# nju-websoft/OpenEA

Measured on AMD Instinct MI355X. Metric: training triples/sec (k=10 truncated negatives + limited loss + Adagrad), higher is better.
Workload: dtype f32; 1 GPU; BootEA/AlignE translational step, EN-FR-100K-V1 shape (synthetic), dim=100, GLOBAL batch=20000 positives (weak scaling: 20000 per GPU x 1 GPU), k=10, truncated eps=0.98; the same workload at every N (; global_batch=20000, entities=200000, parallelism=single

## Files before the change

### include/openea_hip.h

```cpp
#ifndef OPENEA_HIP_H
#define OPENEA_HIP_H

#include <stddef.h>
#include <stdint.h>

#ifdef __cplusplus
extern "C" {
#endif

#define OEA_OK 0
#define OEA_EINVAL (-1)
#define OEA_EHIP (-2)
#define OEA_ENOMEM (-3)
#define OEA_EUNSUPPORTED (-4)

int oea_version(void);
const char *oea_last_error(void);
int oea_device_count(void);

int oea_profile_begin(int32_t stride);
int oea_profile_end(int32_t group, double *out_ms_host, int32_t *n_calls_host);

typedef struct oea_store *oea_store_t;
int oea_store_create(int64_t rows, int32_t dim, oea_store_t *out);
// ... 230 lines not shown
                     const int32_t *pos, int64_t n_pos, const int32_t *neg, int64_t n_neg, const int32_t *paths,
                     const int32_t *neg_rel, const float *weight, int64_t n_paths, float path_parm, const oea_step_cfg *cfg,
                     void *step_workspace, void *path_workspace, double *loss_accum, int32_t *err_flag, void *stream);
int oea_path_sample_epoch(const int32_t *paths1, const float *weight1, int64_t n1, const int32_t *paths2, const float *weight2,
                          int64_t n2, const int32_t *rels1, int32_t n_rels1, const int32_t *rels2, int32_t n_rels2, int32_t steps,
                          uint64_t seed, uint32_t epoch, int32_t *out_paths, int32_t *out_neg_rel, float *out_weight, void *stream);
int oea_ptranse_epoch(float *ent, float *ent_acc, int64_t n_ent, float *rel, float *rel_acc, int64_t n_rel, int32_t dim, int32_t ld,
                      const int32_t *pos_all, const int64_t *offsets_host, int32_t steps, const int32_t *neg_buf,
                      const int32_t *path_buf, const int32_t *neg_rel_buf, const float *weight_buf, int64_t P, float path_parm,
                      const oea_step_cfg *cfg, void *step_workspace, void *path_workspace, double *loss_accum, int32_t *err_flag,
                      void *stream);
int oea_weighted_pair_step(float *ent, float *ent_acc, int64_t n_ent, float *rel, float *rel_acc, int64_t n_rel, int32_t dim,
                           int32_t ld, const int32_t *pos, const int32_t *neg, const float *weight, int64_t n,
                           const oea_step_cfg *cfg, void *step_workspace, double *loss_accum, void *stream);

uint64_t oea_tripleset_capacity(int64_t n);
int oea_tripleset_build(const int32_t *triples, int64_t n, uint64_t *table, uint64_t capacity,
                        void *stream);
int oea_sample_negatives(const int32_t *pos, int64_t n_pos, int32_t k, const uint64_t *table,
                         uint64_t capacity, const int32_t *entity_list, int32_t n_ent_list,
                         const int32_t *ent_pos, const int32_t *nbr, int32_t nbr_k, uint64_t seed,
                         uint32_t step, uint32_t pos_offset, int32_t max_try, int32_t *out,
                         int32_t *err_flag, void *stream);

int oea_sample_negatives_replay(const int32_t *pos, int64_t n_pos, int32_t k, const uint64_t *table, uint64_t capacity,
                                const int32_t *entity_list, int32_t n_ent_list, const int32_t *ent_pos, const int32_t *nbr,
                                int32_t nbr_k, int32_t max_try, const int32_t *replay, int32_t *out, int32_t *err_flag, void *stream);

typedef struct oea_sampler_side {
    const uint64_t *table;
    uint64_t capacity;
    const int32_t *entity_list;
    const int32_t *ent_pos;
    const int32_t *nbr;
    int32_t n_ent_list;
    int32_t nbr_k;
    const uint32_t *filter;
    uint64_t filter_bits;
} oea_sampler_side;
uint64_t oea_tripleset_filter_bits(uint64_t capacity);
int oea_tripleset_filter_build(const int32_t *triples, int64_t n, uint32_t *filter, uint64_t filter_bits, void *stream);
int oea_sample_negatives_pair(const int32_t *pos, int64_t n_pos, int64_t n_split, int32_t k,
                              const oea_sampler_side *side0, const oea_sampler_side *side1, uint64_t seed,
                              uint32_t step, uint32_t pos_offset, int32_t max_try, int32_t *out,
                              int32_t *err_flag, void *stream);

int oea_sample_negatives_epoch(const int32_t *pos_all, int64_t n_rows, const int64_t *offsets_dev,
                               const int64_t *splits_dev, int32_t steps, int32_t k, const oea_sampler_side *side0,
                               const oea_sampler_side *side1, uint64_t seed, uint32_t step_base, int32_t max_try,
                               int32_t *out_all, int32_t *err_flag, void *stream);

typedef struct oea_epoch {
    float *ent, *ent_acc;
    int64_t n_ent;
    float *rel, *rel_acc;
    int64_t n_rel;
    int32_t dim, ld;
    const int32_t *pos_all;
    const int64_t *offsets_host, *splits_host;
    int32_t steps;
    const int64_t *offsets_dev, *splits_dev;
    int32_t k;
    const oea_sampler_side *side0, *side1;
    uint64_t seed;
    uint32_t step_base;
    int32_t *neg_buf, *err_flag;
    const oea_step_cfg *cfg;
    void *workspace;
    double *loss_accum;
} oea_epoch;
int oea_triple_epoch_range(const oea_epoch *e, int32_t step_begin, int32_t step_end, int32_t rank, int32_t world, void *plan,
                           size_t plan_bytes, int32_t plan_built, void *stream);

size_t oea_epoch_layout_bytes(int64_t n);
int oea_epoch_layout(const int32_t *triples, int64_t n1, int64_t n2, const int64_t *slot, int64_t n_slots, uint64_t seed, uint32_t epoch,
                     int32_t *dall, void *workspace, size_t ws_bytes, void *stream);

int32_t oea_step_plan_supported(const oea_step_cfg *cfg, int64_t n_ent, int64_t n_rel, int32_t ld, int32_t k);
size_t oea_step_plan_bytes(int64_t n_total, int32_t steps, int64_t max_batch, int64_t n_ent, int32_t ld);
int oea_step_plan_build(const int32_t *pos_all, const int32_t *neg_all, int32_t k, const int64_t *offsets_dev, int64_t n_total,
                        int32_t steps, int64_t max_batch, int64_t n_ent, int32_t ld, void *plan, size_t plan_bytes, void *stream);
int oea_step_plan_offsets(int64_t n_total, int32_t steps, int64_t max_batch, int64_t n_ent, int32_t ld, int64_t *out);
int oea_step_plan_rel_order_offset(int64_t n_total, int32_t steps, int64_t max_batch, int64_t n_ent, int32_t ld, int64_t *out);

struct oea_comm;
int oea_triple_epoch_range_comm(struct oea_comm *comm, const oea_epoch *e, int32_t step_begin, int32_t step_end, void *send, void *own,
                                void *rel_x, float *upd, float *all, void *stream);


uint32_t oea_perm_index(uint32_t i, uint32_t n, uint32_t key);
int oea_sample_link_negatives(const int32_t *pos_links, int64_t n_pos, int32_t k, const int32_t *ents1, int32_t n1,
                              const int32_t *ents2, int32_t n2, const int32_t *nbr1, const int32_t *row1,
                              const int32_t *nbr2, const int32_t *row2, int32_t nbr_k, const uint64_t *exclude,
                              uint64_t exclude_cap, uint64_t seed, uint32_t step, int32_t *out_pairs, float *out_valid,
                              uint64_t *scratch_keys, int32_t *scratch_vals, uint64_t scratch_cap, void *stream);

int oea_greedy_matching(const int32_t *left, const int32_t *right, const float *weight, int64_t n_edges,
                        uint8_t *selected);
int oea_pair_dots(const float *e1, int32_t ld1, const float *e2, int32_t ld2, int32_t dim, const int32_t *ii,
                  const int32_t *jj, int64_t n, float *out, void *stream);

int oea_row_rank_select_f32(const float *vals, int64_t n_rows, int32_t nc, int64_t ld, int32_t k, int32_t largest, const int32_t *ids,
                            int64_t ld_ids, int32_t *out_sel, float *out_kth, void *stream);
int oea_row_rank_select_f64(const double *vals, int64_t n_rows, int32_t nc, int64_t ld, int32_t k, int32_t largest, const int32_t *ids,
                            int64_t ld_ids, int32_t *out_sel, double *out_kth, void *stream);

size_t oea_topk_workspace_bytes(int64_t nq, int64_t nc);
size_t oea_topk_sym_workspace_bytes(int64_t n, int32_t k);
int oea_topk_inner(const float *q, int64_t nq, int32_t ldq, const float *c, int64_t nc, int32_t ldc,
                   int32_t dim, int32_t k, const int32_t *id_map, int32_t *out_idx, void *workspace,
                   size_t ws_bytes, void *stream);

int oea_topk_rows(const float *s, int64_t n_rows, int64_t nc, int64_t ld, int32_t k, const int32_t *id_map,
                  int32_t *out_idx, void *stream);

enum { OEA_METRIC_INNER = 0, OEA_METRIC_MANHATTAN = 1, OEA_METRIC_EUCLIDEAN = 2,
       OEA_METRIC_MANHATTAN_F32 = 3  };
size_t oea_rank_workspace_bytes(int64_t n1);
int oea_rank_eval(const float *e1, int64_t n1, int32_t ld1, const float *e2, int64_t n2, int32_t ld2,
                  int32_t dim, int32_t metric, const float *csls_r, const float *csls_c, int64_t gold_offset,
                  int32_t *rank, int32_t *argmax, void *workspace, void *stream);
size_t oea_rank_eval_bf16_workspace_bytes(int64_t n1, int32_t dim);
int oea_rank_eval_bf16(const float *e1, int64_t n1, int32_t ld1, const float *e2, int64_t n2, int32_t ld2, int32_t dim,
                       int64_t gold_offset, int32_t *rank, int32_t *argmax, int32_t *status, void *workspace, void *stream);
int oea_rank_eval_bf16_csls(const float *e1, int64_t n1, int32_t ld1, const float *e2, int64_t n2, int32_t ld2, int32_t dim,
                            const float *csls_r, const float *csls_c, int64_t gold_offset, int32_t *rank, int32_t *argmax,
                            int32_t *status, void *workspace, void *stream);
int oea_rank_eval_metrics_bf16(const float *e1, int64_t n1, int32_t ld1, const float *e2, int64_t n2, int32_t ld2, int32_t dim,
                               const float *csls_r, const float *csls_c, int64_t gold_offset, const int32_t *top_k_host, int32_t nk,
                               int32_t *rank, int32_t *argmax, int64_t *out_dev, void *workspace, void *stream);
int oea_sim_bf16_matrix(const float *e1, int64_t n1, int32_t ld1, const float *e2, int64_t n2, int32_t ld2, int32_t dim, float *out,
                        int64_t ld_out, void *stream);
size_t oea_rank_eval_metrics_workspace_bytes(int64_t n1);
int oea_rank_eval_metrics(const float *e1, int64_t n1, int32_t ld1, const float *e2, int64_t n2, int32_t ld2, int32_t dim,
                          const float *csls_r, const float *csls_c, int64_t gold_offset, const int32_t *top_k_host, int32_t nk,
                          int32_t *rank, int32_t *argmax, int64_t *hits_and_rank_sum_dev, double *rr_sum_dev, void *workspace,
                          void *stream);
int oea_rank_metrics(const int32_t *rank, int64_t n, const int32_t *top_k_host, int32_t nk,
                     int64_t *hits_dev, int64_t *rank_sum_dev, double *rr_sum_dev, void *stream);

int oea_rank_rows(const float *s, int64_t n_rows, int64_t nc, int64_t ld, const int32_t *gold_idx,
                  int32_t *rank, int32_t *argmax, void *stream);

int oea_sim_matrix(const float *e1, int64_t n1, int32_t ld1, const float *e2, int64_t n2,
                   int32_t ld2, int32_t dim, int32_t metric, float *out, int64_t ld_out,
                   void *stream);
int oea_quantize_rows_u16(const float *src, int64_t n, int32_t ld, int32_t dim, float lo, float inv_step, uint16_t *dst,
                          int32_t ldq, void *stream);
int oea_l1_u16_strip(const uint16_t *q, int64_t nq, const uint16_t *c, int64_t nc, int32_t ldq, float *out, int64_t ld_out,
                     void *stream);
int oea_rank_l1_grid_rows(const float *strip, int64_t rows, int64_t row0, int64_t nc, int64_t ld, const float *e1, int32_t ld1,
                          const float *e2, int32_t ld2, int32_t dim, int64_t gold_offset, float step, float err, int32_t *rank,
                          int32_t *argmax, int32_t *n_exact_rows, void *stream);
int oea_rank_l1_grid_rows_csls(const float *strip, int64_t rows, int64_t row0, int64_t nc, int64_t ld, const float *e1, int32_t ld1,
                               const float *e2, int32_t ld2, int32_t dim, int64_t gold_offset, float step, float err,
                               const float *csls_r, const float *csls_c, int32_t *rank, int32_t *argmax, int32_t *n_exact_rows,
                               void *stream);
int oea_pair_l1_sim(const float *q, int64_t nq, int32_t ldq, const float *table, int64_t n, int32_t ldt, int32_t dim,
                    const int32_t *cand, int32_t c, float *out, void *stream);
int oea_pair_l1_f64(const float *q, int64_t nq, int32_t ldq, const float *table, int64_t n, int32_t ldt, int32_t dim,
                    const int32_t *cand, int32_t c, double *out, void *stream);

int oea_row_topk_mean(const float *s, int64_t n1, int64_t n2, int64_t ld, int32_t k, float *out,
                      void *stream);
size_t oea_csls_means_workspace_bytes(int64_t n1, int64_t n2, int32_t k);
int oea_csls_means(const float *e1, int64_t n1, int32_t ld1, const float *e2, int64_t n2, int32_t ld2, int32_t dim, int32_t k,
// ... 175 lines not shown
```

### openea_amd/_lib.py

```python
import ctypes as C
import os

_HERE = os.path.dirname(os.path.abspath(__file__))
DETERMINISTIC = os.environ.get("OEA_STEP_DETERMINISTIC", "0")[:1] == "1"
LIB_PATH = os.environ.get("OPENEA_HIP_LIB") or os.path.join(_HERE, "csrc",
                                                            "libopenea_hip_det.so" if DETERMINISTIC else "libopenea_hip.so")


class OpenEAHipError(RuntimeError):
    pass


class StepCfg(C.Structure):
    _fields_ = [("loss_kind", C.c_int32), ("l1", C.c_int32), ("margin", C.c_float),
                ("pos_margin", C.c_float), ("neg_margin", C.c_float), ("balance", C.c_float),
                ("ent_l2_norm", C.c_int32), ("rel_l2_norm", C.c_int32), ("opt_kind", C.c_int32),
                ("lr", C.c_float), ("neg_group_k", C.c_int32), ("score_kind", C.c_int32),
                ("normal", C.c_void_p), ("normal_acc", C.c_void_p),
                ("ent_transfer_base", C.c_int32), ("rel_transfer_base", C.c_int32),
                ("beta1", C.c_float), ("beta2", C.c_float), ("eps", C.c_float), ("opt_t", C.c_int32)]


class SamplerSide(C.Structure):
    _fields_ = [("table", C.c_void_p), ("capacity", C.c_uint64), ("entity_list", C.c_void_p),
# ... 50 lines not shown

class ProjEVars(C.Structure):
    _fields_ = [("p", C.c_void_p * 8), ("m", C.c_void_p * 8), ("v", C.c_void_p * 8)]


class Attr2VecVars(C.Structure):
    _fields_ = [(n, C.c_void_p) for n in ("embeds", "embeds_acc", "nce_weights", "nce_weights_acc", "nce_biases", "nce_biases_acc")]


class ConvEVars(C.Structure):
    _fields_ = [("p", C.c_void_p * 14), ("m", C.c_void_p * 14), ("v", C.c_void_p * 14)]


class ConvECfg(C.Structure):
    _fields_ = [("filter_num", C.c_int32), ("keep_prob", C.c_float), ("seed", C.c_uint64)]


class MultiKENet(C.Structure):
    _fields_ = [("p", C.c_void_p * 8), ("ent", C.c_void_p), ("step_workspace", C.c_void_p), ("n_rel_ws", C.c_int64),
                ("weighted", C.c_int32), ("ent_l2_norm", C.c_int32), ("factor", C.c_float)]


LOSS_KIND = {"margin-based": 0, "limited": 1, "logistic": 2, "positive": 3, "align": 4}
OPT_KIND = {"SGD": 0, "Adagrad": 1, "Adam": 2, "Adadelta": 3}
METRIC = {"inner": 0, "manhattan": 1, "euclidean": 2, "manhattan_f32": 3}

_vp, _i32, _i64, _u32, _u64, _f32, _sz = (C.c_void_p, C.c_int32, C.c_int64, C.c_uint32, C.c_uint64,
                                          C.c_float, C.c_size_t)

PROTOTYPES = {
    "oea_version": (C.c_int, []),
    "oea_last_error": (C.c_char_p, []),
    "oea_device_count": (C.c_int, []),
    "oea_profile_begin": (C.c_int, [_i32]),
    "oea_profile_end": (C.c_int, [_i32, C.POINTER(C.c_double), C.POINTER(_i32)]),
    "oea_store_create": (C.c_int, [_i64, _i32, C.POINTER(_vp)]),
    "oea_store_destroy": (C.c_int, [_vp]),
    "oea_store_rows": (_i64, [_vp]),
    "oea_store_dim": (_i32, [_vp]),
    "oea_store_ld": (_i32, [_vp]),
    "oea_store_rows_ptr": (_vp, [_vp]),
    "oea_store_load_host": (C.c_int, [_vp, _vp, _vp]),
    "oea_store_save_host": (C.c_int, [_vp, _vp, _vp]),
    "oea_gather_rows": (C.c_int, [_vp, _i32, _i32, _vp, _i64, _i32, _vp, _i32, _vp]),
    "oea_normalize_rows": (C.c_int, [_vp, _i64, _i32, _i32, _i32, _vp]),
    "oea_fill_f32": (C.c_int, [_vp, _i64, _f32, _vp]),
    "oea_copy_to_host": (C.c_int, [_vp, _vp, _sz, _vp]),
    "oea_copy_from_host": (C.c_int, [_vp, _vp, _sz, _vp]),
    "oea_step_workspace_bytes": (_sz, [_i64, _i64, _i32]),
    "oea_triple_step": (C.c_int, [_vp, _vp, _i64, _vp, _vp, _i64, _i32, _i32, _vp, _i64, _vp, _i64,
                                  C.POINTER(StepCfg), _vp, _vp, _vp]),
    "oea_step_exchange_floats": (_sz, [_i64, _i64, _i32]),
    "oea_step_scratch_elem_bytes": (_i32, []),
    "oea_triple_step_phase": (C.c_int, [_vp, _vp, _i64, _vp, _vp, _i64, _i32, _i32, _vp, _i64, _vp, _i64,
                                        C.POINTER(StepCfg), _vp, _vp, _i32, _vp]),
    "oea_part_rows_per_rank": (_i64, [_i64, _i32]),
    "oea_part_send_floats": (_sz, [_i64, _i32, _i32]),
    "oea_part_pack": (C.c_int, [_vp, _i64, _i64, _i32, _i32, _vp, _vp, _vp]),
    "oea_part_apply": (C.c_int, [_vp, _vp, _i64, _vp, _vp, _i64, _i32, _i32, _i32, _vp, _vp, _vp, C.POINTER(StepCfg), _vp, _i64,
                                 _vp, _vp]),
    "oea_step_normal_scratch": (C.c_int, [_i64, _i64, _i32, _vp, _vp]),
    "oea_step_apply_normals": (C.c_int, [_i64, _i64, _i32, _vp, _vp, _vp]),
    "oea_part_unpack": (C.c_int, [_vp, _i64, _i32, _i32, _i32, _vp, _vp]),
    "oea_step_scatter_ent_rows": (C.c_int, [_vp, _i64, _i64, _i32, _vp, _i64, _vp, _i32, _vp]),
    "oea_tripleset_capacity": (_u64, [_i64]),
    "oea_tripleset_build": (C.c_int, [_vp, _i64, _vp, _u64, _vp]),
    "oea_sample_negatives": (C.c_int, [_vp, _i64, _i32, _vp, _u64, _vp, _i32, _vp, _vp, _i32, _u64,
                                       _u32, _u32, _i32, _vp, _vp, _vp]),
    "oea_sample_negatives_replay": (C.c_int, [_vp, _i64, _i32, _vp, _u64, _vp, _i32, _vp, _vp, _i32, _i32, _vp, _vp, _vp, _vp]),
    "oea_tripleset_filter_bits": (C.c_uint64, [_u64]),
    "oea_tripleset_filter_build": (C.c_int, [_vp, _i64, _vp, _u64, _vp]),
    "oea_sample_negatives_pair": (C.c_int, [_vp, _i64, _i64, _i32, C.POINTER(SamplerSide), C.POINTER(SamplerSide),
                                            _u64, _u32, _u32, _i32, _vp, _vp, _vp]),
    "oea_sample_negatives_epoch": (C.c_int, [_vp, _i64, _vp, _vp, _i32, _i32, C.POINTER(SamplerSide),
                                             C.POINTER(SamplerSide), _u64, _u32, _i32, _vp, _vp, _vp]),
    "oea_triple_epoch_range": (C.c_int, [C.POINTER(Epoch), _i32, _i32, _i32, _i32, _vp, _sz, _i32, _vp]),
    "oea_epoch_layout_bytes": (_sz, [_i64]),
    "oea_epoch_layout": (C.c_int, [_vp, _i64, _i64, _vp, _i64, _u64, _u32, _vp, _vp, _sz, _vp]),
    "oea_step_plan_supported": (_i32, [C.POINTER(StepCfg), _i64, _i64, _i32, _i32]),
    "oea_step_plan_bytes": (_sz, [_i64, _i32, _i64, _i64, _i32]),
    "oea_step_plan_offsets": (C.c_int, [_i64, _i32, _i64, _i64, _i32, _vp]),
    "oea_step_plan_rel_order_offset": (C.c_int, [_i64, _i32, _i64, _i64, _i32, _vp]),
    "oea_step_plan_build": (C.c_int, [_vp, _vp, _i32, _vp, _i64, _i32, _i64, _i64, _i32, _vp, _sz, _vp]),
    "oea_triple_epoch_range_comm": (C.c_int, [_vp, C.POINTER(Epoch), _i32, _i32, _vp, _vp, _vp, _vp, _vp, _vp]),
    "oea_rotate_workspace_bytes": (_sz, [_i64, _i64, _i32]),
    "oea_rotate_exchange_doubles": (_sz, [_i64, _i64, _i32]),
    "oea_rotate_step": (C.c_int, [_vp, _vp, _i64, _vp, _vp, _i64, _i32, _i32, _vp, _i64, _vp, _i64, _i32,
                                  C.POINTER(RotateCfg), _vp, _vp, _i32, _vp]),
    "oea_rotate_lookup": (C.c_int, [_vp, _i64, _i32, _i32, _vp, _i64, _i32, _i32, _vp, _i32, _vp]),
    "oea_mapping_workspace_floats": (_sz, [_i64, _i32, _i32]),
    "oea_mapping_step": (C.c_int, [_vp, _i32, _i32, _i32, _vp, _vp, _i64, _vp, _vp, C.c_float, C.c_float, _i32, _vp, _vp,
                                   _vp, _vp, _vp]),
    "oea_mapping_epoch": (C.c_int, [_vp, _vp, _i64, _vp, _vp, _i64, _i32, _i32, _i32, _vp, _i32, _i64, _vp, _vp, _f32, _f32, _i32,
                                    C.POINTER(StepCfg), _vp, _vp, _vp, _vp, _vp]),
    "oea_sea_mapping_workspace_floats": (_sz, [_i64, _i64, _i32, _i32]),
    "oea_sea_mapping_step": (C.c_int, [_vp, _i32, _i32, _vp, _vp, _i64, _vp, _vp, _i64, _vp, _vp, _vp, _f32, _f32, C.POINTER(StepCfg),
                                       _vp, _vp, _vp, _vp, _vp]),
    "oea_sea_mapping_epoch": (C.c_int, [_vp, _vp, _i64, _vp, _vp, _i64, _i32, _i32, _vp, _i32, _i64, _i64, _vp, _vp, _vp, _f32, _f32,
                                        C.POINTER(StepCfg), _vp, _vp, _vp, _vp, _vp]),
    "oea_step_entity_scratch": (C.c_int, [_vp, _i64, _i64, _i32, C.POINTER(C.c_void_p), C.POINTER(C.c_void_p)]),
    "oea_transr_workspace_bytes": (_sz, [_i64, _i64, _i32, _i64]),
    "oea_transr_step": (C.c_int, [_vp, _vp, _i64, _vp, _vp, _i64, _vp, _vp, _i32, _i32, _vp, _i64, _vp, _i64, C.POINTER(StepCfg),
                                  _vp, _vp, _vp, _vp]),
    "oea_semantic_step": (C.c_int, [_i32, _vp, _vp, _i64, _vp, _vp, _i64, _i32, _i32, _vp, _i64, _vp, _i64, C.POINTER(StepCfg),
                                    _vp, _vp, _vp]),
    "oea_jape_step": (C.c_int, [_vp, _vp, _i64, _vp, _vp, _i64, _i32, _i32, _vp, _i64, _vp, _i64, _f32, C.POINTER(StepCfg), _vp, _vp, _vp]),
    "oea_multike_cnn_workspace_bytes": (_sz, [_i32, _i32, _i64]),
    "oea_multike_cnn_grads": (C.c_int, [_vp, _i32, _i32, _i64, _i32, C.POINTER(C.c_void_p)]),
    "oea_multike_cnn_step": (C.c_int, [C.POINTER(MultiKENet), _i32, _i64, _vp, _i64, _vp, _i64, _i32, _i32, _vp, _i64, _vp, _f32, _vp,
                                       _i64, _vp, _i32, _vp]),
    "oea_multike_rows": (C.c_int, [_i32, _vp, _vp, _i64, _i32, _vp, _vp, _i64, _i32, _vp, _i32, _i64, _i32, _i32, _i32, _vp, _i64, _vp,
                                   _f32, _vp, _vp]),
    "oea_attre_lds_chars": (_i64, [_i32]),
    "oea_attre_char_workspace_bytes": (_sz, [_i64, _i32, _i64]),
    "oea_attre_char_step": (C.c_int, [_vp, _vp, _i64, _vp, _vp, _i64, _vp, _vp, _i64, _i32, _i32, _vp, _i64, _i32, _vp, _i64, _vp, _i64,
                                      _i32, _i32, _i32, C.POINTER(StepCfg), _vp, _vp, _sz, _vp, _vp, _vp]),
    "oea_attre_sample_heads": (C.c_int, [_vp, _i64, _i64, _i32, _vp, _i32, _vp, _vp, _i32, _vp, _i64, _u64, _u32, _u32, _vp, _vp]),
    "oea_attre_joint_epoch": (C.c_int, [_vp, _vp, _vp, _vp, _vp, _i64, _i32, _i32, _i32, _i32, _f32, _i32, _vp, _vp]),
    "oea_sample_distinct": (C.c_int, [_i64, _i64, _u64, _u64, _vp, _vp]),
    "oea_sim_csr_count": (C.c_int, [_vp, _i64, _i32, _vp, _i64, _i32, _i32, _f32, _i64, _vp, _vp, _vp]),
    "oea_sim_csr_fill": (C.c_int, [_vp, _i64, _i32, _vp, _i64, _i32, _i32, _f32, _i64, _vp, _vp, _vp, _vp, _vp, _vp]),
    "oea_jape_sim_loss": (C.c_int, [_vp, _i64, _i32, _i32, _vp, _i64, _vp, _i64, _vp, _vp, _vp, _vp, _i64, _f32, _vp, _vp]),
    "oea_lcs_workspace_ints": (_sz, [_i64]),
    "oea_lcs_ratio_pairs": (C.c_int, [_vp, _vp, _i64, _i64, _vp, _vp, _i64, _i64, _i64, _vp, _i64, _vp, _vp, _vp, _vp, _vp]),
    "oea_attr_sim_records": (C.c_int, [_vp, _vp, _i64, _i64, _vp, _vp, _i64, _i64, _i64, _i32, _vp, _i64, _vp, _i64, C.c_double, _vp, _i64,
                                       _i32, _vp, _vp, _vp, _vp, _vp, _vp, _vp]),
    "oea_log_uniform_sample_steps": (C.c_int, [_i64, _i64, _u64, _u64, _i64, _vp, _vp, _vp, _vp, _vp, _vp]),
    "oea_attr2vec_workspace_bytes": (_sz, [_i64, _i32, _i64]),
    "oea_attr2vec_grads": (C.c_int, [_vp, _i64, _i32, _i64, C.POINTER(C.c_void_p)]),
    "oea_attr2vec_step": (C.c_int, [C.POINTER(Attr2VecVars), _i64, _i32, _i32, _vp, _i64, _vp, _i64, _vp, _vp, _f32, _vp, _i64, _vp, _i32,
                                    _vp]),
    "oea_attr2vec_epoch": (C.c_int, [C.POINTER(Attr2VecVars), _i64, _i32, _i32, _vp, _i64, _i64, _i32, _u64, _u64, _vp, _i64, _vp, _vp, _vp,
                                     _vp, _vp, _f32, _vp, _i64, _vp, _vp]),
    "oea_log_uniform_workspace_bytes": (_sz, [_i64, _i64]),
    "oea_log_uniform_sample": (C.c_int, [_i64, _i64, _u64, _u64, _vp, _vp, _vp, _vp, _vp, _vp]),
    "oea_proje_workspace_floats": (_sz, [_i64, _i64, _i32, _i32, _i64, _i64]),
    "oea_proje_grads": (C.c_int, [_vp, _i64, _i64, _i32, _i32, _i64, _i64, C.POINTER(C.c_void_p)]),
    "oea_proje_step": (C.c_int, [C.POINTER(ProjEVars), _i64, _i64, _i32, _i32, _vp, _i64, _vp, _vp, _i64, _vp, _i64, _f32, _vp, _i64,
                                 _i64, _vp, _i32, _vp]),
    "oea_conve_workspace_floats": (_sz, [_i64, _i64, _i32, _i32, _i32, _i64, _i64]),
    "oea_conve_grads": (C.c_int, [_vp, _i64, _i64, _i32, _i32, _i32, _i64, _i64, C.POINTER(C.c_void_p)]),
    "oea_conve_step": (C.c_int, [C.POINTER(ConvEVars), C.POINTER(ConvECfg), _i64, _i64, _i32, _i32, _vp, _i64, _vp, _vp, _i64, _vp,
                                 _u64, _i64, _f32, _vp, _i64, _i64, _vp, _i32, _vp]),
    "oea_path_workspace_bytes": (_sz, [_i64, _i32]),
    "oea_path_grad": (C.c_int, [_vp, _i64, _i32, _i32, _vp, _vp, _vp, _i64, _f32, _f32, _i32, _vp, _i64, _vp, _vp, _vp, _vp]),
    "oea_ptranse_step": (C.c_int, [_vp, _vp, _i64, _vp, _vp, _i64, _i32, _i32, _vp, _i64, _vp, _i64, _vp, _vp, _vp, _i64, _f32,
                                   C.POINTER(StepCfg), _vp, _vp, _vp, _vp, _vp]),
    "oea_path_sample_epoch": (C.c_int, [_vp, _vp, _i64, _vp, _vp, _i64, _vp, _i32, _vp, _i32, _i32, _u64, _u32, _vp, _vp, _vp, _vp]),
    "oea_ptranse_epoch": (C.c_int, [_vp, _vp, _i64, _vp, _vp, _i64, _i32, _i32, _vp, _vp, _i32, _vp, _vp, _vp, _vp, _i64, _f32,
                                    C.POINTER(StepCfg), _vp, _vp, _vp, _vp, _vp]),
    "oea_weighted_pair_step": (C.c_int, [_vp, _vp, _i64, _vp, _vp, _i64, _i32, _i32, _vp, _vp, _vp, _i64, C.POINTER(StepCfg), _vp,
                                         _vp, _vp]),
    "oea_greedy_matching": (C.c_int, [_vp, _vp, _vp, _i64, _vp]),
    "oea_pair_dots": (C.c_int, [_vp, _i32, _vp, _i32, _i32, _vp, _vp, _i64, _vp, _vp]),
    "oea_perm_index": (_u32, [_u32, _u32, _u32]),
    "oea_sample_link_negatives": (C.c_int, [_vp, _i64, _i32, _vp, _i32, _vp, _i32, _vp, _vp, _vp, _vp, _i32, _vp, _u64,
                                            _u64, _u32, _vp, _vp, _vp, _vp, _u64, _vp]),
    "oea_topk_sym_workspace_bytes": (_sz, [_i64, _i32]),
    "oea_topk_workspace_bytes": (_sz, [_i64, _i64]),
    "oea_topk_inner": (C.c_int, [_vp, _i64, _i32, _vp, _i64, _i32, _i32, _i32, _vp, _vp, _vp, _sz, _vp]),
    "oea_row_rank_select_f32": (C.c_int, [_vp, _i64, _i32, _i64, _i32, _i32, _vp, _i64, _vp, _vp, _vp]),
    "oea_row_rank_select_f64": (C.c_int, [_vp, _i64, _i32, _i64, _i32, _i32, _vp, _i64, _vp, _vp, _vp]),
    "oea_topk_rows": (C.c_int, [_vp, _i64, _i64, _i64, _i32, _vp, _vp, _vp]),
    "oea_rank_rows": (C.c_int, [_vp, _i64, _i64, _i64, _vp, _vp, _vp, _vp]),
    "oea_rank_workspace_bytes": (_sz, [_i64]),
    "oea_rank_eval": (C.c_int, [_vp, _i64, _i32, _vp, _i64, _i32, _i32, _i32, _vp, _vp, _i64, _vp, _vp, _vp, _vp]),
# ... 118 lines not shown
```

### openea_amd/csrc/common.h

```cpp
#pragma once
#include <hip/hip_runtime.h>
#include <hip/hip_ext.h>
#include <stdint.h>
#include <stdio.h>

#include "../../include/openea_hip.h"

namespace oea {

void set_error(const char *fmt, ...);

bool prof_enabled();
void prof_call();
void prof_mark(hipStream_t st);
bool prof_pair(hipEvent_t *start, hipEvent_t *stop);

#define OEA_CHECK_HIP(expr)                                                                   \
    do {                                                                                      \
        hipError_t _e = (expr);                                                               \
        if (_e != hipSuccess) {                                                               \
            oea::set_error("%s:%d: %s -> %s", __FILE__, __LINE__, #expr, hipGetErrorString(_e)); \
            return OEA_EHIP;                                                                  \
        }                                                                                     \
    } while (0)
// ... 58 lines not shown
    return __builtin_bit_cast(float, __builtin_amdgcn_update_dpp(0, __builtin_bit_cast(int, v), CTRL, 0xf, 0xf, false));
}
template <int G>
__device__ __forceinline__ float group_sum(float v) {
    static_assert(G == 2 || G == 4 || G == 8 || G == 16 || G == 32 || G == 64, "group width");
    if (G >= 2) v += dpp_f32<0xB1>(v);
    if (G >= 4) v += dpp_f32<0x4E>(v);
    if (G >= 8) v += dpp_f32<0x141>(v);
    if (G >= 16) v += dpp_f32<0x140>(v);
    if (G >= 32) {
        const unsigned u = __builtin_bit_cast(unsigned, v);
        const auto r = __builtin_amdgcn_permlane16_swap(u, u, false, false);
        v = __builtin_bit_cast(float, (unsigned)r[0]) + __builtin_bit_cast(float, (unsigned)r[1]);
    }
    if (G >= 64) {
        const unsigned u = __builtin_bit_cast(unsigned, v);
        const auto r = __builtin_amdgcn_permlane32_swap(u, u, false, false);
        v = __builtin_bit_cast(float, (unsigned)r[0]) + __builtin_bit_cast(float, (unsigned)r[1]);
    }
    return v;
}
__device__ __forceinline__ float wave_sum_uniform(float v) {
    v += dpp_f32<0xB1>(v);
    v += dpp_f32<0x4E>(v);
    v += dpp_f32<0x141>(v);
    v += dpp_f32<0x140>(v);
    v += dpp_f32<0x142>(v);
    v += dpp_f32<0x143>(v);
    return __builtin_bit_cast(float, __builtin_amdgcn_readlane(__builtin_bit_cast(int, v), 63));
}
template <int G>
__device__ __forceinline__ double group_sum_d(double v) {
#pragma unroll
    for (int off = G / 2; off > 0; off >>= 1) v += __shfl_xor(v, off, 64);
    return v;
}
__device__ __forceinline__ double wave_sum_d(double v) { return group_sum_d<64>(v); }

template <int WAVES>
__device__ __forceinline__ void block_loss_add(double v, int lane, int wave, double *loss_accum, double scale = 1.0) {
    __shared__ double wave_loss[WAVES];
    if (lane == 0) wave_loss[wave] = v;
    __syncthreads();
    if (threadIdx.x == 0) {
        double s = 0.0;
        for (int w = 0; w < WAVES; ++w) s += wave_loss[w];
        if (s != 0.0) atomicAdd(loss_accum, scale * s);
    }
}

__device__ __forceinline__ void atomic_add_f32(float *p, float v) { unsafeAtomicAdd(p, v); }

#ifdef OEA_DET_SCRATCH
typedef long long grad_t;
typedef long long flag_t;
constexpr int kDetScratch = 1;
__device__ __forceinline__ long long to_fixed(float v) {
    const float c = __builtin_amdgcn_fmed3f(v, -524287.f, 524287.f);
    const double d = (double)c + 1572864.0;
    return __double_as_longlong(d) - 0x4138000000000000LL;
}
__device__ __forceinline__ float grad_val(long long q) { return (float)((double)q * 2.3283064365386963e-10); }
__device__ __forceinline__ void grad_add(long long *p, float v) {
    __hip_atomic_fetch_add(reinterpret_cast<unsigned long long *>(p), (unsigned long long)to_fixed(v), __ATOMIC_RELAXED,
                           __HIP_MEMORY_SCOPE_AGENT);
}
__device__ __forceinline__ void grad_add_raw(long long *p, long long q) {
    __hip_atomic_fetch_add(reinterpret_cast<unsigned long long *>(p), (unsigned long long)q, __ATOMIC_RELAXED, __HIP_MEMORY_SCOPE_AGENT);
}
#else
typedef float grad_t;
typedef float flag_t;
constexpr int kDetScratch = 0;
__device__ __forceinline__ float grad_val(float q) { return q; }
__device__ __forceinline__ void grad_add(float *p, float v) { unsafeAtomicAdd(p, v); }
__device__ __forceinline__ void grad_add_raw(float *p, float q) { unsafeAtomicAdd(p, q); }
#endif

void step_scratch_rows(void *workspace, int64_t n_ent, int64_t n_rel, int32_t ld, grad_t **ent_grad, flag_t **ent_touched,
                       grad_t **rel_grad, flag_t **rel_touched);

__device__ __forceinline__ float4 ld4(const float *p) { return *reinterpret_cast<const float4 *>(p); }
__device__ __forceinline__ void st4(float *p, float4 v) { *reinterpret_cast<float4 *>(p) = v; }

__device__ __forceinline__ uint4 philox4x32_10(uint32_t c0, uint32_t c1, uint32_t c2, uint32_t c3,
                                               uint32_t k0, uint32_t k1) {
    const uint32_t M0 = 0xD2511F53u, M1 = 0xCD9E8D57u, W0 = 0x9E3779B9u, W1 = 0xBB67AE85u;
#pragma unroll
    for (int r = 0; r < 10; ++r) {
        const uint32_t hi0 = __umulhi(M0, c0), lo0 = M0 * c0;
        const uint32_t hi1 = __umulhi(M1, c2), lo1 = M1 * c2;
        const uint32_t n0 = hi1 ^ c1 ^ k0, n1 = lo1, n2 = hi0 ^ c3 ^ k1, n3 = lo0;
        c0 = n0; c1 = n1; c2 = n2; c3 = n3;
        k0 += W0; k1 += W1;
    }
    return make_uint4(c0, c1, c2, c3);
}

__host__ __device__ __forceinline__ uint32_t feistel_f(uint32_t r, uint32_t key, uint32_t round) {
    uint32_t v = r * 0x9E3779B1u + key + round * 0x85EBCA6Bu;
    v ^= v >> 15; v *= 0x2C1B3C6Du;
    v ^= v >> 12; v *= 0x297A2D39u;
    v ^= v >> 15;
    return v;
}
__host__ __device__ __forceinline__ uint32_t perm_index(uint32_t i, uint32_t n, uint32_t key) {
    uint32_t bits = 2;
    while ((1u << bits) < n) bits += 2;
    const uint32_t half = bits >> 1, mask = (1u << half) - 1u;
    uint32_t x = i;
    do {
        uint32_t l = x >> half, r = x & mask;
#pragma unroll
        for (uint32_t round = 0; round < 4; ++round) {
            const uint32_t t = l ^ (feistel_f(r, key, round) & mask);
            l = r;
            r = t;
        }
        x = (l << half) | r;
    } while (x >= n);
    return x;
}

#define OEA_EMPTY_KEY 0xFFFFFFFFFFFFFFFFull
__host__ __device__ __forceinline__ uint64_t pack_triple(uint32_t h, uint32_t r, uint32_t t) {
    return ((uint64_t)h << 40) | ((uint64_t)(r & 0xFFFFu) << 24) | (uint64_t)(t & 0xFFFFFFu);
}
__host__ __device__ __forceinline__ uint64_t mix64(uint64_t x) {
    x ^= x >> 30; x *= 0xBF58476D1CE4E5B9ull;
    x ^= x >> 27; x *= 0x94D049BB133111EBull;
    x ^= x >> 31;
    return x;
}

}
```

### openea_amd/csrc/step_plan.h

```cpp
#pragma once
#include <hip/hip_runtime.h>
#include <stddef.h>
#include <stdint.h>

namespace oea {

struct StepPlanView {
    uint64_t *keys_a, *keys_b;
    uint32_t *vals_a, *vals_b;
    uint64_t *ukeys;
    uint32_t *ucount;
    uint32_t *uoff;
    int32_t *n_unique;
    int32_t *step_first;
    uint32_t *pflags;
    uint4 *recs;
    uint8_t *inplan;
    float *contrib;
    void *temp;
    size_t temp_bytes;
    uint32_t *rel_order;
    int row_bits;
};

constexpr uint32_t kPlanHubEntries = 8;

size_t step_plan_layout(int64_t n_total, int32_t steps, int64_t max_batch, int64_t n_ent, int32_t ld, void *base, StepPlanView *v);

}
```

### openea_amd/csrc/step_plan.hip

```cpp
#include <string.h>

#include <rocprim/rocprim.hpp>

#include <algorithm>

#include "common.h"
#include "step_plan.h"

namespace oea {

static size_t al256(size_t x) { return (x + 255) / 256 * 256; }
static int bits_for(uint64_t max_value) { int b = 1; while (b < 64 && (max_value >> b) != 0) ++b; return b; }

size_t step_plan_layout(int64_t n_total, int32_t steps, int64_t max_batch, int64_t n_ent, int32_t ld, void *base, StepPlanView *v) {
    const size_t m = (size_t)std::max<int64_t>(2 * n_total, 1);
    size_t off = 0;
    char *b = static_cast<char *>(base);
    auto take = [&](size_t bytes) { size_t o = off; off += al256(bytes); return b ? b + o : nullptr; };
    StepPlanView w{};
    w.keys_a = (uint64_t *)take(8 * m);
    w.keys_b = (uint64_t *)take(8 * m);
    w.vals_a = (uint32_t *)take(4 * m);
    w.vals_b = (uint32_t *)take(4 * m);
    w.ukeys = (uint64_t *)take(8 * m);
    w.ucount = (uint32_t *)take(4 * (m + 1));
    w.uoff = (uint32_t *)take(4 * (m + 1));
    w.n_unique = (int32_t *)take(4);
    w.step_first = (int32_t *)take(4 * ((size_t)steps + 1));
    w.pflags = (uint32_t *)take(4 * (size_t)std::max<int64_t>(n_total, 1));
    w.recs = (uint4 *)take(16 * m);
    w.inplan = (uint8_t *)take((size_t)std::max<int32_t>(steps, 1) * (size_t)n_ent);
    w.contrib = (float *)take(sizeof(float) * 2 * (size_t)std::max<int64_t>(max_batch, 1) * (size_t)ld);
    size_t t1 = 0, t2 = 0, t3 = 0;
    (void)rocprim::radix_sort_pairs(nullptr, t1, (const uint64_t *)nullptr, (uint64_t *)nullptr, (const uint32_t *)nullptr,
                                    (uint32_t *)nullptr, m, 0, 64, (hipStream_t)0);
    (void)rocprim::run_length_encode(nullptr, t2, (const uint64_t *)nullptr, m, (uint64_t *)nullptr, (uint32_t *)nullptr,
                                     (int32_t *)nullptr, (hipStream_t)0);
    (void)rocprim::exclusive_scan(nullptr, t3, (const uint32_t *)nullptr, (uint32_t *)nullptr, 0u, m + 1, rocprim::plus<uint32_t>(),
                                  (hipStream_t)0);
    const size_t n1 = (size_t)std::max<int64_t>(n_total, 1);
    w.temp_bytes = std::max(std::max(t1, std::max(t2, t3)), al256(4 * n1)) + 256;
    w.temp = take(w.temp_bytes);
    w.rel_order = (uint32_t *)take(4 * n1);
    w.row_bits = bits_for((uint64_t)std::max<int64_t>(n_ent - 1, 1));
    if (v) *v = w;
    return off;
}

namespace {

__global__ void plan_emit_kernel(const int32_t *__restrict__ pos_all, const int32_t *__restrict__ neg_all, int k,
                                 const int64_t *__restrict__ offsets, int steps, int64_t n_total, int row_bits,
                                 uint64_t *__restrict__ keys, uint32_t *__restrict__ vals) {
    const int64_t p = (int64_t)blockIdx.x * blockDim.x + threadIdx.x;
    if (p >= n_total) return;
    int lo = 0, hi = steps;
    while (hi - lo > 1) {
        const int mid = (lo + hi) >> 1;
        if (offsets[mid] <= p) lo = mid; else hi = mid;
    }
    const uint32_t pl = (uint32_t)(p - offsets[lo]);
    const int h = pos_all[3 * p], r = pos_all[3 * p + 1], t = pos_all[3 * p + 2];
    unsigned bad = 0, xh = 0, xt = 0;
    const int32_t *ng = neg_all + p * k * 3;
    for (int j = 0; j < k; ++j) {
        const unsigned a = (unsigned)(ng[3 * j] ^ h), b = (unsigned)(ng[3 * j + 2] ^ t), c = (unsigned)(ng[3 * j + 1] ^ r);
        bad |= c | min(a, b);
        xh |= a;
        xt |= b;
    }
    if (bad | min(xh, xt)) {
        keys[2 * p] = keys[2 * p + 1] = (uint64_t)steps << row_bits;
        vals[2 * p] = vals[2 * p + 1] = 0u;
        return;
    }
    const bool tails = xh == 0;
    const uint64_t sk = (uint64_t)lo << row_bits;
    keys[2 * p] = sk | (uint64_t)(uint32_t)h;
    vals[2 * p] = 2u * pl + (tails ? 0u : 1u);
    keys[2 * p + 1] = sk | (uint64_t)(uint32_t)t;
    vals[2 * p + 1] = 0x80000000u | (2u * pl + (tails ? 1u : 0u));
}

constexpr int kRelSortWaves = 8, kRelDigitBits = 10, kRelBins = 1 << kRelDigitBits, kRelAhead = 8;
__global__ __launch_bounds__(kRelSortWaves * 64) void plan_rel_order_kernel(const int32_t *__restrict__ pos_all, const int64_t *__restrict__ offsets,
                                                                            uint32_t *__restrict__ tmp, uint32_t *__restrict__ rel_order) {
    __shared__ uint32_t hist[kRelSortWaves][kRelBins];
    __shared__ uint32_t dbase[kRelBins];
    __shared__ uint32_t wsum[kRelSortWaves];
    __shared__ uint32_t rmax;
    const int64_t first = offsets[blockIdx.x];
    const uint32_t n = (uint32_t)(offsets[blockIdx.x + 1] - first);
    if (n == 0) return;
    const int32_t *rel = pos_all + 3 * first + 1;
    const uint32_t t = threadIdx.x, lane = t & 63u, w = t >> 6;
    const uint32_t slice = (n + kRelSortWaves - 1) / kRelSortWaves, c0 = min(w * slice, n), c1 = min(c0 + slice, n);
    const uint32_t groups = (c1 - c0 + 63u) / 64u;
    if (t == 0) rmax = 0u;
    int passes = 1;
    uint32_t *src = nullptr, *dst = nullptr;
    for (int pass = 0; pass < passes; ++pass) {
        const int shift = pass * kRelDigitBits;
        for (uint32_t i = t; i < kRelSortWaves * kRelBins; i += blockDim.x) (&hist[0][0])[i] = 0u;
        __syncthreads();
        uint32_t m = 0u;
        for (uint32_t g0 = 0; g0 < groups; g0 += kRelAhead) {
            uint32_t r[kRelAhead];
#pragma unroll
            for (int u = 0; u < kRelAhead; ++u) {
                const uint32_t i = c0 + (g0 + u) * 64u + lane;
                r[u] = i < c1 ? (uint32_t)rel[3 * (int64_t)(src ? src[i] : i)] : 0xffffffffu;
            }
#pragma unroll
            for (int u = 0; u < kRelAhead; ++u)
                if (c0 + (g0 + u) * 64u + lane < c1) {
                    m = max(m, r[u]);
                    atomicAdd(&hist[w][(r[u] >> shift) & (kRelBins - 1)], 1u);
                }
        }
        if (pass == 0) {
            for (int o = 32; o > 0; o >>= 1) m = max(m, (uint32_t)__shfl_xor((int)m, o));
            if (lane == 0) atomicMax(&rmax, m);
        }
        __syncthreads();
        if (pass == 0) {
            while (passes * kRelDigitBits < 32 && (rmax >> (passes * kRelDigitBits)) != 0u) ++passes;
// ... 78 lines not shown
    }
}

__global__ void plan_hub_kernel(const uint64_t *__restrict__ keys, const uint32_t *__restrict__ vals, int64_t m,
                                const int64_t *__restrict__ offsets, int steps, int row_bits, uint32_t *__restrict__ pflags) {
    const int64_t e = (int64_t)blockIdx.x * blockDim.x + threadIdx.x;
    if (e >= m) return;
    const uint64_t key = keys[e];
    const int64_t step = (int64_t)(key >> row_bits);
    if (step >= steps) return;
    int left = 0, right = 0;
    while (left < (int)kPlanHubEntries && e - left - 1 >= 0 && keys[e - left - 1] == key) ++left;
    while (left + right < (int)kPlanHubEntries && e + right + 1 < m && keys[e + right + 1] == key) ++right;
    if (left + right < (int)kPlanHubEntries) return;
    const uint32_t v = vals[e];
    atomicOr(&pflags[offsets[step] + ((v & 0x7fffffffu) >> 1)], (v >> 31) ? 2u : 1u);
}

__device__ __forceinline__ uint32_t mix32(uint32_t x) {
    x ^= x >> 16; x *= 0x7feb352du; x ^= x >> 15; x *= 0x846ca68bu; x ^= x >> 16;
    return x;
}
__device__ __forceinline__ uint32_t feistel_perm(uint32_t i, uint32_t n, int lbits, int rbits, const uint32_t (&key)[6]) {
    const uint32_t lmask = (1u << lbits) - 1u, rmask = (1u << rbits) - 1u;
    uint32_t x = i;
    do {
        uint32_t l = x >> rbits, r = x & rmask;
#pragma unroll
        for (int q = 0; q < 6; q += 2) {
            l = (l ^ mix32(r ^ key[q])) & lmask;
            r = (r ^ mix32(l ^ key[q + 1])) & rmask;
        }
        x = (l << rbits) | r;
    } while (x >= n);
    return x;
}
__global__ void layout_perm_kernel(const int32_t *__restrict__ triples, int64_t n1, int64_t n2, const int64_t *__restrict__ slot, int64_t n_slots,
                                   uint32_t k0, uint32_t k1, uint32_t epoch, int32_t *__restrict__ dall) {
    const int64_t j = (int64_t)blockIdx.x * blockDim.x + threadIdx.x;
    if (j >= n_slots) return;
    const int64_t sj = slot[j];
    const bool second = sj >= n1;
    const uint32_t n = (uint32_t)(second ? n2 : n1), i = (uint32_t)(second ? sj - n1 : sj);
    int bits = 1;
    while (bits < 32 && (1ull << bits) < (unsigned long long)n) ++bits;
    if (bits < 2) bits = 2;
    const int rbits = bits / 2, lbits = bits - rbits;
    const uint4 wa = philox4x32_10(epoch, second ? 1u : 0u, 0x5eedu, 0u, k0, k1), wb = philox4x32_10(epoch, second ? 1u : 0u, 0x5eedu, 1u, k0, k1);
    const uint32_t key[6] = {wa.x, wa.y, wa.z, wa.w, wb.x, wb.y};
    const int64_t src = (int64_t)feistel_perm(i, n, lbits, rbits, key) + (second ? n1 : 0);
    dall[3 * j] = triples[3 * src]; dall[3 * j + 1] = triples[3 * src + 1]; dall[3 * j + 2] = triples[3 * src + 2];
}

}
}

extern "C" {

size_t oea_step_plan_bytes(int64_t n_total, int32_t steps, int64_t max_batch, int64_t n_ent, int32_t ld) {
    if (n_total < 0 || steps < 0 || max_batch < 0 || n_ent <= 0 || ld <= 0) return 0;
    return oea::step_plan_layout(n_total, steps, max_batch, n_ent, ld, nullptr, nullptr);
}

int oea_step_plan_offsets(int64_t n_total, int32_t steps, int64_t max_batch, int64_t n_ent, int32_t ld, int64_t *out) {
    OEA_REQUIRE(out && n_total >= 0 && steps >= 0 && n_ent > 0 && ld > 0, "arguments");
    oea::StepPlanView v;
    char *base = reinterpret_cast<char *>(4096);
    const size_t total = oea::step_plan_layout(n_total, steps, max_batch, n_ent, ld, base, &v);
    out[0] = (char *)v.vals_b - base; out[1] = (char *)v.ukeys - base; out[2] = (char *)v.uoff - base;
    out[3] = (char *)v.n_unique - base; out[4] = (char *)v.step_first - base; out[5] = (char *)v.contrib - base;
    out[6] = v.row_bits; out[7] = (int64_t)total; out[8] = (char *)v.pflags - base;
    return OEA_OK;
}

int oea_step_plan_rel_order_offset(int64_t n_total, int32_t steps, int64_t max_batch, int64_t n_ent, int32_t ld, int64_t *out) {
    OEA_REQUIRE(out && n_total >= 0 && steps >= 0 && n_ent > 0 && ld > 0, "arguments");
    oea::StepPlanView v;
    char *base = reinterpret_cast<char *>(4096);
    (void)oea::step_plan_layout(n_total, steps, max_batch, n_ent, ld, base, &v);
    *out = (char *)v.rel_order - base;
    return OEA_OK;
}

size_t oea_epoch_layout_bytes(int64_t n) {
    return n < 0 ? 0 : 256;
}

int oea_epoch_layout(const int32_t *triples, int64_t n1, int64_t n2, const int64_t *slot, int64_t n_slots, uint64_t seed, uint32_t epoch,
                     int32_t *dall, void *workspace, size_t ws_bytes, void *stream) {
    OEA_REQUIRE(triples && (slot || n_slots == 0) && (dall || n_slots == 0), "null pointer");
    OEA_REQUIRE(n1 >= 0 && n2 >= 0 && n_slots >= 0 && n1 < ((int64_t)1 << 32) && n2 < ((int64_t)1 << 32), "sizes");
    (void)workspace; (void)ws_bytes;
    if (n1 + n2 == 0 || n_slots == 0) return OEA_OK;
    hipStream_t st = oea::as_stream(stream);
    oea::layout_perm_kernel<<<(unsigned)oea::ceil_div(n_slots, 256), 256, 0, st>>>(triples, n1, n2, slot, n_slots, (uint32_t)seed,
                                                                                   (uint32_t)(seed >> 32), epoch, dall);
    OEA_CHECK_HIP(hipGetLastError());
    return OEA_OK;
}

int oea_step_plan_build(const int32_t *pos_all, const int32_t *neg_all, int32_t k, const int64_t *offsets_dev, int64_t n_total,
                        int32_t steps, int64_t max_batch, int64_t n_ent, int32_t ld, void *plan, size_t plan_bytes, void *stream) {
    OEA_REQUIRE(pos_all && offsets_dev && plan && (neg_all || k == 0), "null pointer");
    OEA_REQUIRE(n_total >= 0 && steps >= 1 && k >= 0 && n_ent > 0 && ld > 0, "sizes");
    OEA_REQUIRE(2 * n_total < ((int64_t)1 << 31) && 2 * max_batch < ((int64_t)1 << 31), "entries and slots are 31-bit");
    oea::StepPlanView v;
    const size_t need = oea::step_plan_layout(n_total, steps, max_batch, n_ent, ld, plan, &v);
    OEA_REQUIRE(plan_bytes >= need, "plan workspace smaller than oea_step_plan_bytes");
    hipStream_t st = oea::as_stream(stream);
    const size_t m = (size_t)(2 * n_total);
    if (m == 0) {
        OEA_CHECK_HIP(hipMemsetAsync(v.n_unique, 0, sizeof(int32_t), st));
        OEA_CHECK_HIP(hipMemsetAsync(v.step_first, 0, sizeof(int32_t) * ((size_t)steps + 1), st));
        return OEA_OK;
    }
    oea::plan_rel_order_kernel<<<(unsigned)steps, oea::kRelSortWaves * 64, 0, st>>>(pos_all, offsets_dev, (uint32_t *)v.temp, v.rel_order);
    oea::plan_emit_kernel<<<(unsigned)oea::ceil_div(n_total, 256), 256, 0, st>>>(pos_all, neg_all, k, offsets_dev, steps, n_total, v.row_bits,
                                                                                 v.keys_a, v.vals_a);
    const int end_bit = std::min(64, v.row_bits + oea::bits_for((uint64_t)steps));
    size_t tb = v.temp_bytes;
    OEA_CHECK_HIP(rocprim::radix_sort_pairs(v.temp, tb, (const uint64_t *)v.keys_a, v.keys_b, (const uint32_t *)v.vals_a, v.vals_b, m, 0,
                                            (unsigned)end_bit, st));
    OEA_CHECK_HIP(hipMemsetAsync(v.ucount, 0, sizeof(uint32_t) * (m + 1), st));
    tb = v.temp_bytes;
    OEA_CHECK_HIP(rocprim::run_length_encode(v.temp, tb, (const uint64_t *)v.keys_b, m, v.ukeys, v.ucount, v.n_unique, st));
    tb = v.temp_bytes;
    OEA_CHECK_HIP(rocprim::exclusive_scan(v.temp, tb, (const uint32_t *)v.ucount, v.uoff, 0u, m + 1, rocprim::plus<uint32_t>(), st));
    oea::plan_step_first_kernel<<<(unsigned)oea::ceil_div(steps + 1, 256), 256, 0, st>>>(v.ukeys, v.n_unique, steps, v.row_bits, v.step_first);
    OEA_CHECK_HIP(hipMemsetAsync(v.pflags, 0, sizeof(uint32_t) * (size_t)n_total, st));
    OEA_CHECK_HIP(hipMemsetAsync(v.inplan, 0, (size_t)steps * (size_t)n_ent, st));
    oea::plan_records_kernel<<<(unsigned)std::min<int64_t>(oea::ceil_div((int64_t)m, 256), 4096), 256, 0, st>>>(
        v.ukeys, v.uoff, v.vals_b, v.n_unique, steps, v.row_bits, n_ent, v.recs, v.inplan);
    oea::plan_hub_kernel<<<(unsigned)oea::ceil_div((int64_t)m, 256), 256, 0, st>>>(v.keys_b, v.vals_b, (int64_t)m, offsets_dev, steps, v.row_bits,
                                                                                   v.pflags);
    OEA_CHECK_HIP(hipGetLastError());
    return OEA_OK;
}

}
```

### openea_amd/csrc/triple_step.hip

```cpp
#include <stdlib.h>

#include <algorithm>
#include <type_traits>
#include <vector>

#include "common.h"
#include "step_plan.h"

namespace {

using oea::align256;
using oea::group_sum;

using oea::flag_t;
using oea::grad_t;

struct StepWs {
    grad_t *ent_grad, *rel_grad;
    grad_t *rel_extra;
    int64_t rel_copy_stride;
    flag_t *ent_touched, *rel_touched;
    grad_t *nrm_grad, *nrm_extra;
    flag_t *nrm_touched;
    double *partials;
// ... 327 lines not shown
            any = coef != 0.f;
        }
        if (any) {
            atomic_row<G, IT>(ws.ent_grad + (int64_t)h * ld, ld, lane, gh, 1.f);
            atomic_row<G, IT>(ws.rel_copy(p % kRelCopies) + (int64_t)r * ld, ld, lane, gr, 1.f);
            atomic_row<G, IT>(ws.ent_grad + (int64_t)t * ld, ld, lane, gt, 1.f);
            if (lane == 0) { ws.ent_touched[h] = 1.f; ws.ent_touched[t] = 1.f; ws.rel_touched[r] = 1.f; }
        }
        if (lane == 0) loss_local += lsum;
    }
    block_loss_partial(loss_local, ws.partials);
}

#ifdef OEA_DET_SCRATCH
constexpr int kGradShift = 3;
#else
constexpr int kGradShift = 2;
#endif
constexpr unsigned kBufFlags = 0x00020000u;
constexpr int kBufRecords = (int)0x80000000u;
constexpr int kBufOob = (int)0xC0000000u;

__device__ __forceinline__ void buf_grad_add(__amdgpu_buffer_rsrc_t rs, float v, int voff, int soff, int imm) {
#ifdef OEA_DET_SCRATCH
    const long long q = oea::to_fixed(v);
    const int vo = voff + imm;
    asm volatile("s_nop 4\n\tbuffer_atomic_add_x2 %0, %1, %2, %3 offen" ::"v"(q), "v"(vo), "s"(rs), "s"(soff) : "memory");
#else
    __builtin_amdgcn_raw_ptr_buffer_atomic_fadd_f32(v, rs, voff + imm, soff, 0);
#endif
}
__device__ __forceinline__ void buf_flag_set(__amdgpu_buffer_rsrc_t rs, int row) {
#ifdef OEA_DET_SCRATCH
    typedef unsigned int u32x2 __attribute__((ext_vector_type(2)));
    const u32x2 one = {1u, 0u};
    __builtin_amdgcn_raw_buffer_store_b64(one, rs, 0, row * 8, 0);
#else
    __builtin_amdgcn_raw_buffer_store_b32(0x3f800000u, rs, 0, row * 4, 0);
#endif
}
template <int IT>
__device__ __forceinline__ void wave_load_row(__amdgpu_buffer_rsrc_t rs, int soff, int v4, int vt, Row<64, IT> &r) {
#pragma unroll
    for (int it = 0; it < IT; ++it)
        r.v[it] = __builtin_bit_cast(float, __builtin_amdgcn_raw_buffer_load_b32(rs, it < IT - 1 ? v4 + it * 256 : vt, soff, 0));
}
template <int IT>
__device__ __forceinline__ void wave_atomic_row(__amdgpu_buffer_rsrc_t rs, int soff, int vg, int vgt, const Row<64, IT> &g, float sign) {
#pragma unroll
    for (int it = 0; it < IT; ++it) {
        if (it < IT - 1) buf_grad_add(rs, sign * g.v[it], vg, soff, it * (64 << kGradShift));
        else buf_grad_add(rs, sign * g.v[it], vgt, soff, 0);
    }
}
template <int IT>
__device__ __forceinline__ void wave_rel_row(const StepWs &ws, int dbg, int64_t p, int r, int row_g, int vg, int vgt, const Row<64, IT> &g) {
    const int copy = (int)(p % kRelCopies);
    grad_t *rgb = copy == 0 ? ws.rel_grad : ws.rel_extra + (copy - 1) * ws.rel_copy_stride;
    const __amdgpu_buffer_rsrc_t rs_rg = __builtin_amdgcn_make_buffer_rsrc(rgb, 0, (dbg & 1) ? 0 : kBufRecords, kBufFlags);
    const __amdgpu_buffer_rsrc_t rs_rt = __builtin_amdgcn_make_buffer_rsrc(ws.rel_touched, 0, (dbg & 4) ? 0 : kBufRecords, kBufFlags);
    wave_atomic_row<IT>(rs_rg, r * row_g, vg, vgt, g, 1.f);
    buf_flag_set(rs_rt, r);
}
__device__ __forceinline__ float uniform_f(float x) {
    return __builtin_bit_cast(float, __builtin_amdgcn_readfirstlane(__builtin_bit_cast(int, x)));
}

__device__ __forceinline__ double uniform_d(double x) {
    const unsigned long long b = __builtin_bit_cast(unsigned long long, x);
    const unsigned lo = (unsigned)__builtin_amdgcn_readfirstlane((int)(unsigned)b), hi = (unsigned)__builtin_amdgcn_readfirstlane((int)(unsigned)(b >> 32));
    return __builtin_bit_cast(double, ((unsigned long long)hi << 32) | lo);
}

template <int IT>
__device__ __forceinline__ void wave_normalize(Row<64, IT> &r) {
    float s = 0.f;
#pragma unroll
    for (int it = 0; it < IT; ++it) s += r.v[it] * r.v[it];
    const float inv = rsqrtf(fmaxf(oea::wave_sum_uniform(s), 1e-12f));
#pragma unroll
    for (int it = 0; it < IT; ++it) r.v[it] *= inv;
}

template <int IT, int L1, int KT, bool PLAN>
__global__ __launch_bounds__(512, (IT <= 2 ? (KT == 10 ? 8 : 7) : 4)) void triple_wave(
    const float *__restrict__ ent, const float *__restrict__ rel, int ld, const int32_t *__restrict__ pos,
    int64_t n_pos, const int32_t *__restrict__ neg, int k, oea_step_cfg cfg, StepWs ws, int dbg, float *__restrict__ contrib,
    const uint32_t *__restrict__ pflags, const uint32_t *__restrict__ order) {
    constexpr int G = 64, KC = 10;
    if (KT > 0) k = KT;
    const int lane = threadIdx.x & 63;
    const int wv = __builtin_amdgcn_readfirstlane((int)(threadIdx.x >> 6));
    const int wpb = blockDim.x >> 6;
    const int64_t nw = (int64_t)gridDim.x * wpb;
    const int row_b = ld * 4, row_g = ld << kGradShift;
    const __amdgpu_buffer_rsrc_t rs_ent = __builtin_amdgcn_make_buffer_rsrc(const_cast<float *>(ent), 0, (dbg & 2) ? 0 : kBufRecords, kBufFlags);
    const __amdgpu_buffer_rsrc_t rs_rel = __builtin_amdgcn_make_buffer_rsrc(const_cast<float *>(rel), 0, (dbg & 2) ? 0 : kBufRecords, kBufFlags);
    const __amdgpu_buffer_rsrc_t rs_eg = __builtin_amdgcn_make_buffer_rsrc(ws.ent_grad, 0, (dbg & 1) ? 0 : kBufRecords, kBufFlags);
    const __amdgpu_buffer_rsrc_t rs_et = __builtin_amdgcn_make_buffer_rsrc(ws.ent_touched, 0, (dbg & 4) ? 0 : kBufRecords, kBufFlags);
    const int v4 = lane * 4, vg = lane << kGradShift;
    const int c_last = (IT - 1) * 64 + lane;
    const int vt = c_last < ld ? c_last * 4 : kBufOob, vgt = c_last < ld ? c_last << kGradShift : kBufOob;
    const float c_neg = L1 ? -cfg.balance : -2.f * cfg.balance;
    double loss_local = 0.0;
    auto score_positive = [&](int64_t p, Row<G, IT> &gacc) -> int {
        const int32_t *pp = pos + 3 * p;
        const int32_t *ng = neg + p * k * 3;
        const int h = pp[0], r = pp[1], t = pp[2];
        Row<G, IT> yh, yr, yt;
        wave_load_row<IT>(rs_ent, h * row_b, v4, vt, yh);
        wave_load_row<IT>(rs_rel, r * row_b, v4, vt, yr);
        wave_load_row<IT>(rs_ent, t * row_b, v4, vt, yt);
        int ids[3 * KC];
        if (KT == KC || k == KC) {
#pragma unroll
            for (int q = 0; q < 3 * KC; ++q) ids[q] = ng[q];
        } else {
#pragma unroll
            for (int q = 0; q < 3 * KC; ++q) ids[q] = q < 3 * k ? ng[q] : 0;
        }
        unsigned bad = 0, xh = 0, xt = 0;
#pragma unroll
        for (int j = 0; j < KC; ++j)
            if (KT == KC || j < k) {
                const unsigned a = (unsigned)(ids[3 * j] ^ h), b = (unsigned)(ids[3 * j + 2] ^ t), c = (unsigned)(ids[3 * j + 1] ^ r);
                bad |= c | min(a, b);
                xh |= a;
                xt |= b;
            }
        if (bad) {
            double ls = score_independent<G, IT>(ent, rel, ld, lane, p, h, r, t, true, cfg, ws, OEA_LOSS_LIMITED, L1);
#pragma unroll 1
            for (int j = 0; j < k; ++j)
                ls += score_independent<G, IT>(ent, rel, ld, lane, p, ng[3 * j], ng[3 * j + 1], ng[3 * j + 2], false, cfg, ws, OEA_LOSS_LIMITED, L1);
            loss_local = uniform_d(loss_local + ls);
            return -1;
        }
        if (min(xh, xt)) {
            unsigned tmask = 0;
            int ce[KC];
            Row<G, IT> yc[KC];
#pragma unroll
            for (int j = 0; j < KC; ++j)
                if (KT == KC || j < k) {
                    const int nh = ids[3 * j], nt = ids[3 * j + 2];
                    const bool tl = nh == h;
                    tmask |= tl ? 1u << j : 0u;
                    ce[j] = tl ? nt : nh;
                    wave_load_row<IT>(rs_ent, ce[j] * row_b, v4, vt, yc[j]);
                }
            asm volatile("" : "+s"(tmask));
#pragma unroll
            for (int it = 0; it < IT; ++it)
                asm volatile("" : "+v"(yh.v[it]), "+v"(yr.v[it]), "+v"(yt.v[it]));
            wave_normalize<IT>(yh);
            wave_normalize<IT>(yr);
            wave_normalize<IT>(yt);
            Row<G, IT> u, gpos;
            float sp = 0.f;
#pragma unroll
            for (int it = 0; it < IT; ++it) {
                u.v[it] = yh.v[it] + yr.v[it];
                const float d = u.v[it] - yt.v[it];
                gpos.v[it] = d;
                sp += L1 ? fabsf(d) : d * d;
            }
            const float xp = oea::wave_sum_uniform(sp) - cfg.pos_margin;
            const bool cpos = xp > 0.f;
            float lsum = cpos ? xp : 0.f;
#pragma unroll
            for (int it = 0; it < IT; ++it) {
                gpos.v[it] = cpos ? (L1 ? sgn(gpos.v[it]) : 2.f * gpos.v[it]) : 0.f;
                gacc.v[it] = gpos.v[it];
            }
            bool anyneg = false;
#pragma unroll
            for (int j = 0; j < KC; ++j)
                if (KT == KC || j < k) {
                    const bool tl = (tmask >> j) & 1u;
                    wave_normalize<IT>(yc[j]);
                    float s = 0.f;
                    if (tl) {
#pragma unroll
                        for (int it = 0; it < IT; ++it) {
                            const float d = u.v[it] - yc[j].v[it];
                            yc[j].v[it] = d;
                            s += L1 ? fabsf(d) : d * d;
                        }
                    } else {
#pragma unroll
                        for (int it = 0; it < IT; ++it) {
                            const float d = yc[j].v[it] + yr.v[it] - yt.v[it];
                            yc[j].v[it] = d;
                            s += L1 ? fabsf(d) : d * d;
                        }
                    }
                    const float xn = cfg.neg_margin - oea::wave_sum_uniform(s);
                    if (xn > 0.f) {
                        lsum += cfg.balance * xn;
                        anyneg = true;
                        Row<G, IT> g;
#pragma unroll
                        for (int it = 0; it < IT; ++it) {
                            g.v[it] = L1 ? c_neg * sgn(yc[j].v[it]) : c_neg * yc[j].v[it];
                            gacc.v[it] += g.v[it];
                        }
                        const int pe = tl ? h : t;
                        const float sign_c = tl ? -1.f : 1.f;
                        wave_atomic_row<IT>(rs_eg, ce[j] * row_g, vg, vgt, g, sign_c);
                        buf_flag_set(rs_et, ce[j]);
                        wave_atomic_row<IT>(rs_eg, pe * row_g, vg, vgt, g, -sign_c);
                        buf_flag_set(rs_et, pe);
                    }
                }
            if (cpos) {
                wave_atomic_row<IT>(rs_eg, h * row_g, vg, vgt, gpos, 1.f);
                buf_flag_set(rs_et, h);
                wave_atomic_row<IT>(rs_eg, t * row_g, vg, vgt, gpos, -1.f);
                buf_flag_set(rs_et, t);
            }
            loss_local = uniform_d(loss_local + (double)lsum);
            if (!(cpos | anyneg)) return -1;
            if (PLAN && order) return r;
            wave_rel_row<IT>(ws, dbg, p, r, row_g, vg, vgt, gacc);
            return -1;
        }
        auto one_sided = [&](auto side) -> int {
            constexpr bool tails = decltype(side)::value;
            int ce[KC];
            Row<G, IT> yc[KC];
#pragma unroll
            for (int j = 0; j < KC; ++j)
                if (KT == KC || j < k) {
                    ce[j] = tails ? ids[3 * j + 2] : ids[3 * j];
                    wave_load_row<IT>(rs_ent, ce[j] * row_b, v4, vt, yc[j]);
                }
            wave_normalize<IT>(yh);
            wave_normalize<IT>(yr);
            wave_normalize<IT>(yt);
            Row<G, IT> u, gpos;
            int r_sum = -1;
            float sp = 0.f;
#pragma unroll
            for (int it = 0; it < IT; ++it) {
                u.v[it] = yh.v[it] + yr.v[it];
                const float d = u.v[it] - yt.v[it];
                gpos.v[it] = d;
                sp += L1 ? fabsf(d) : d * d;
            }
            const float xp = oea::wave_sum_uniform(sp) - cfg.pos_margin;
            const bool cpos = xp > 0.f;
            float lsum = cpos ? xp : 0.f;
#pragma unroll
            for (int it = 0; it < IT; ++it) {
                gpos.v[it] = cpos ? (L1 ? sgn(gpos.v[it]) : 2.f * gpos.v[it]) : 0.f;
                gacc.v[it] = gpos.v[it];
            }
            float sc[KC];
            if (tails) {
#pragma unroll
                for (int j = 0; j < KC; ++j)
                    if (KT == KC || j < k) {
                        wave_normalize<IT>(yc[j]);
                        float s = 0.f;
#pragma unroll
                        for (int it = 0; it < IT; ++it) {
                            const float d = u.v[it] - yc[j].v[it];
                            yc[j].v[it] = d;
                            s += L1 ? fabsf(d) : d * d;
                        }
                        sc[j] = oea::wave_sum_uniform(s);
                    }
            } else {
#pragma unroll
                for (int j = 0; j < KC; ++j)
                    if (KT == KC || j < k) {
                        wave_normalize<IT>(yc[j]);
                        float s = 0.f;
#pragma unroll
                        for (int it = 0; it < IT; ++it) {
                            const float d = yc[j].v[it] + yr.v[it] - yt.v[it];
                            yc[j].v[it] = d;
                            s += L1 ? fabsf(d) : d * d;
                        }
                        sc[j] = oea::wave_sum_uniform(s);
                    }
            }
            bool anyneg = false;
            const float sign_c = tails ? -1.f : 1.f;
#pragma unroll
            for (int j = 0; j < KC; ++j)
                if (KT == KC || j < k) {
                    const float xn = cfg.neg_margin - sc[j];
                    if (xn > 0.f) {
                        lsum += cfg.balance * xn;
                        anyneg = true;
                        Row<G, IT> g;
#pragma unroll
                        for (int it = 0; it < IT; ++it) {
                            g.v[it] = L1 ? c_neg * sgn(yc[j].v[it]) : c_neg * yc[j].v[it];
                            gacc.v[it] += g.v[it];
                        }
                        wave_atomic_row<IT>(rs_eg, ce[j] * row_g, vg, vgt, g, sign_c);
                        buf_flag_set(rs_et, ce[j]);
                    }
                }
            if (PLAN) {
                const __amdgpu_buffer_rsrc_t rs_cb = __builtin_amdgcn_make_buffer_rsrc(contrib, 0, kBufRecords, kBufFlags);
                const int so = (int)p * 2 * row_b;
#pragma unroll
                for (int it = 0; it < IT; ++it) {
                    const int vo = it < IT - 1 ? v4 + it * 256 : vt;
                    __builtin_amdgcn_raw_buffer_store_b32(__builtin_bit_cast(unsigned, gacc.v[it]), rs_cb, vo, so, 0);
                    __builtin_amdgcn_raw_buffer_store_b32(__builtin_bit_cast(unsigned, gpos.v[it]), rs_cb, vo, so + row_b, 0);
                }
            }
            if (cpos | anyneg) {
                if (PLAN && order) r_sum = r;
                else wave_rel_row<IT>(ws, dbg, p, r, row_g, vg, vgt, gacc);
                const unsigned via_atomics = PLAN ? pflags[p] : 3u;
                const bool h_full = tails, t_full = !tails;
                if ((via_atomics & 1u) && (h_full || cpos)) {
                    wave_atomic_row<IT>(rs_eg, h * row_g, vg, vgt, h_full ? gacc : gpos, 1.f);
                    buf_flag_set(rs_et, h);
                }
                if ((via_atomics & 2u) && (t_full || cpos)) {
                    wave_atomic_row<IT>(rs_eg, t * row_g, vg, vgt, t_full ? gacc : gpos, -1.f);
                    buf_flag_set(rs_et, t);
                }
            }
            loss_local = uniform_d(loss_local + (double)lsum);
            return r_sum;
        };
        return xh == 0 ? one_sided(std::true_type{}) : one_sided(std::false_type{});
    };
    if constexpr (!PLAN) {
        for (int64_t p = (int64_t)blockIdx.x * wpb + wv; p < n_pos; p += nw) {
            Row<G, IT> gacc;
            (void)score_positive(p, gacc);
        }
    } else {
        for (int64_t q0 = (int64_t)blockIdx.x * wpb; q0 < n_pos; q0 += nw) {
            const int64_t q = q0 + wv;
            Row<G, IT> gacc;
            const int r_sum = q < n_pos ? score_positive(order ? (int64_t)order[q] : q, gacc) : -1;
            if (!order) continue;
            __shared__ float s_row[8][IT][64];
            __shared__ int s_rel[8];
            int lb = v4;
            asm volatile("" : "+v"(lb));
            const auto at = [lb](auto *base) { return (decltype(base))((char *)base + lb); };
            if (lb == 0) s_rel[wv] = r_sum;
            if (r_sum >= 0) {
#pragma unroll
                for (int it = 0; it < IT; ++it) *at(&s_row[wv][it][0]) = gacc.v[it];
            }
            __syncthreads();
            if (r_sum >= 0) {
                const int held = lb < wpb * 4 ? *at(&s_rel[0]) : -1;
                bool first = true;
#pragma unroll
                for (int w = 0; w < 8; ++w) first = first && !(w < wv && __builtin_amdgcn_readlane(held, w) == r_sum);
                if (first) {
#pragma unroll
                    for (int w = 1; w < 8; ++w)
                        if (w > wv && __builtin_amdgcn_readlane(held, w) == r_sum) {
#pragma unroll
                            for (int it = 0; it < IT; ++it) gacc.v[it] += *at(&s_row[w][it][0]);
                        }
                    wave_rel_row<IT>(ws, dbg, order[q], r_sum, row_g, vg, vgt, gacc);
                }
            }
            if (q0 + nw < n_pos) __syncthreads();
        }
    }
    __shared__ double sred[8];
    int lz = v4;
    if constexpr (PLAN) asm volatile("" : "+v"(lz));
    if (lz == 0) sred[wv] = loss_local;
    __syncthreads();
    if (wv == 0 && lz == 0) {
        double s = 0.0;
        for (int w = 0; w < wpb; ++w) s += sred[w];
        ws.partials[blockIdx.x] = s;
    }
}

template <int G, int IT>
__device__ __forceinline__ float dot(const Row<G, IT> &a, const Row<G, IT> &b) {
// ... 293 lines not shown
        if (KIND == OEA_SCORE_TRANSD)
            return transd_triple<G, IT>(ent, rel, ld, lane, item, tr[0], tr[1], tr[2], is_pos, cfg, ws, mode, coef, l);
        return transh_triple<G, IT>(ent, rel, ld, lane, item, tr[0], tr[1], tr[2], is_pos, cfg, ws, mode, coef, l);
    };
    for (int64_t item = grp; item < items; item += ngrp) {
        float l;
        if (!margin) {
            const bool is_pos = item < n_pos;
            one(item, is_pos ? pos + 3 * item : neg + 3 * (item - n_pos), is_pos, 2, 0.f, l);
            if (lane == 0) loss_local += (double)l;
            continue;
        }
        float sc[2];
#pragma unroll 1
        for (int u = 0; u < 2; ++u) sc[u] = one(item, (u ? neg : pos) + 3 * item, u == 0, 0, 0.f, l);
        const float x = cfg.margin + sc[0] - sc[1];
        if (x <= 0.f) continue;
        if (lane == 0) loss_local += (double)x;
#pragma unroll 1
        for (int u = 0; u < 2; ++u) one(item, (u ? neg : pos) + 3 * item, u == 0, 1, u ? -1.f : 1.f, l);
    }
    block_loss_partial(loss_local, ws.partials);
}

template <int G, int IT>
__global__ __launch_bounds__(256) void apply_normal_rows(int64_t n_rel, int ld, oea_step_cfg cfg, StepWs ws, int copies_folded) {
    const int lane = threadIdx.x % G;
    const int64_t grp = ((int64_t)blockIdx.x * blockDim.x + threadIdx.x) / G;
    const int64_t ngrp = (int64_t)gridDim.x * blockDim.x / G;
    for (int64_t row = grp; row < n_rel; row += ngrp) {
        if (ws.nrm_touched[row] == 0) continue;
        float *v = cfg.normal + row * ld;
        Row<G, IT> rv, rg, y1, y2;
        grad_t q[IT];
        load_row<G, IT>(v, ld, lane, rv);
        load_grad_raw<G, IT>(ws.nrm_grad + row * ld, ld, lane, q);
        for (int cp = 1; cp < kRelCopies && !copies_folded; ++cp) {
#pragma unroll
            for (int it = 0; it < IT; ++it) {
                const int c = it * G + lane;
                if (c < ld) {
                    const grad_t x = ws.nrm_copy(cp)[row * ld + c];
                    if (x != 0) { q[it] += x; ws.nrm_copy(cp)[row * ld + c] = 0; }
                }
            }
        }
#pragma unroll
        for (int it = 0; it < IT; ++it) rg.v[it] = oea::grad_val(q[it]);
        const float ss1 = sumsq<G, IT>(rv);
        const float inv1 = rsqrtf(fmaxf(ss1, 1e-12f));
#pragma unroll
        for (int it = 0; it < IT; ++it) y1.v[it] = rv.v[it] * inv1;
        const float ss2 = sumsq<G, IT>(y1);
        const float inv2 = rsqrtf(fmaxf(ss2, 1e-12f));
#pragma unroll
        for (int it = 0; it < IT; ++it) y2.v[it] = y1.v[it] * inv2;
        const float d2 = dot<G, IT>(y2, rg);
#pragma unroll
        for (int it = 0; it < IT; ++it) rg.v[it] = (rg.v[it] - y2.v[it] * d2) * inv2;
        const float d1 = ss1 > 1e-12f ? dot<G, IT>(y1, rg) : 0.f;
#pragma unroll
        for (int it = 0; it < IT; ++it) {
            const int c = it * G + lane;
            if (c < ld) {
                const float gv = (rg.v[it] - y1.v[it] * d1) * inv1;
                if (cfg.opt_kind == OEA_OPT_ADAGRAD) {
                    const float a = cfg.normal_acc[row * ld + c] + gv * gv;
                    cfg.normal_acc[row * ld + c] = a;
                    v[c] = rv.v[it] - cfg.lr * gv / sqrtf(a);
                } else {
                    v[c] = rv.v[it] - cfg.lr * gv;
                }
                ws.nrm_grad[row * ld + c] = 0;
            }
        }
        if (lane == 0) ws.nrm_touched[row] = 0;
    }
}

template <int G, int IT, bool CLEAR = true>
__device__ __forceinline__ void apply_one_row(float *__restrict__ v, float *__restrict__ acc, grad_t *__restrict__ g,
                                              flag_t *__restrict__ touched_flag, int ld, int lane, int on,
                                              const oea_step_cfg &cfg, const Row<G, IT> &rv, Row<G, IT> &rg,
                                              const Row<G, IT> &ra) {
    float inv = 1.f, ydg = 0.f;
    if (on) {
        const float ss = sumsq<G, IT>(rv);
        inv = rsqrtf(fmaxf(ss, 1e-12f));
        float dot = 0.f;
#pragma unroll
        for (int it = 0; it < IT; ++it) dot += rv.v[it] * rg.v[it];
        dot = group_sum<G>(dot) * inv;
        ydg = ss > 1e-12f ? dot : 0.f;
    }
#pragma unroll
    for (int it = 0; it < IT; ++it) {
        const int c = it * G + lane;
        if (c < ld) {
            const float gv = on ? (rg.v[it] - rv.v[it] * inv * ydg) * inv : rg.v[it];
            if (cfg.opt_kind == OEA_OPT_ADAGRAD) {
                const float a = ra.v[it] + gv * gv;
                acc[c] = a;
                v[c] = rv.v[it] - cfg.lr * gv / sqrtf(a);
            } else {
                v[c] = rv.v[it] - cfg.lr * gv;
            }
            if (CLEAR) g[c] = 0;
        }
    }
    if (CLEAR && lane == 0) *touched_flag = 0;
}

template <int G, int IT>
__device__ __forceinline__ void apply_relation_row(int64_t row, float *__restrict__ rel, float *__restrict__ rel_acc, int ld, int lane,
                                                   const oea_step_cfg &cfg, const StepWs &ws, int copies_folded) {
    float *v = rel + row * ld;
    float *acc = rel_acc + row * ld;
    grad_t *g = ws.rel_grad + row * ld;
    const float flag = (float)ws.rel_touched[row];
    Row<G, IT> rv, rg, ra;
    grad_t q[IT];
    load_row<G, IT>(v, ld, lane, rv);
    load_grad_raw<G, IT>(g, ld, lane, q);
    if (cfg.opt_kind == OEA_OPT_ADAGRAD) load_row<G, IT>(acc, ld, lane, ra);
    if (flag == 0.f) return;
    if (!copies_folded) {
        constexpr int CB = IT <= 4 ? 5 : 1;
#ifdef OEA_DET_SCRATCH
#pragma unroll 1
#endif
        for (int cp0 = 1; cp0 < kRelCopies; cp0 += CB) {
            grad_t tmp[CB][IT];
#pragma unroll
            for (int u = 0; u < CB; ++u)
#pragma unroll
                for (int it = 0; it < IT; ++it) {
                    const int c = it * G + lane;
                    tmp[u][it] = (cp0 + u < kRelCopies && c < ld) ? ws.rel_copy(cp0 + u)[row * ld + c] : (grad_t)0;
                }
#pragma unroll
            for (int u = 0; u < CB; ++u)
#pragma unroll
                for (int it = 0; it < IT; ++it) {
                    const int c = it * G + lane;
                    q[it] += tmp[u][it];
                    if (cp0 + u < kRelCopies && c < ld && tmp[u][it] != 0) ws.rel_copy(cp0 + u)[row * ld + c] = 0;
                }
        }
    }
#pragma unroll
    for (int it = 0; it < IT; ++it) rg.v[it] = oea::grad_val(q[it]);
    apply_one_row<G, IT>(v, acc, g, ws.rel_touched + row, ld, lane, cfg.rel_l2_norm, cfg, rv, rg, ra);
}

template <int G, int IT, int R>
__global__ __launch_bounds__(256) void apply_rows(float *__restrict__ ent, float *__restrict__ ent_acc,
                                                  int64_t n_ent, float *__restrict__ rel,
                                                  float *__restrict__ rel_acc, int64_t n_rel, int ld,
                                                  oea_step_cfg cfg, StepWs ws, int n_partials,
                                                  double *__restrict__ loss_accum, int copies_folded, int flag_first) {
    const int lane = threadIdx.x % G;
    const int64_t grp = ((int64_t)blockIdx.x * blockDim.x + threadIdx.x) / G;
    const int64_t ngrp = (int64_t)gridDim.x * blockDim.x / G;
    const int64_t n_items = n_rel + (n_ent + R - 1) / R;
    for (int64_t w = grp; w < n_items; w += ngrp) {
        if (w >= n_rel) {
            const int64_t row0 = (w - n_rel) * R;
            float flag[R];
            Row<G, IT> rv[R], rg[R], ra[R];
            if (flag_first) {
                bool any = false;
#pragma unroll
                for (int r = 0; r < R; ++r) any |= row0 + r < n_ent && ws.ent_touched[row0 + r] != 0;
                if (!any) continue;
            }
#pragma unroll
            for (int r = 0; r < R; ++r) {
                const int64_t row = row0 + r < n_ent ? row0 + r : n_ent - 1;
                flag[r] = row0 + r < n_ent ? (float)ws.ent_touched[row] : 0.f;
                load_row<G, IT>(ent + row * ld, ld, lane, rv[r]);
                load_grad_row<G, IT>(ws.ent_grad + row * ld, ld, lane, rg[r]);
                if (cfg.opt_kind == OEA_OPT_ADAGRAD) load_row<G, IT>(ent_acc + row * ld, ld, lane, ra[r]);
            }
#pragma unroll
            for (int r = 0; r < R; ++r) {
                if (flag[r] == 0.f) continue;
                const int64_t row = row0 + r;
                apply_one_row<G, IT>(ent + row * ld, ent_acc + row * ld, ws.ent_grad + row * ld, ws.ent_touched + row, ld,
                                     lane, cfg.ent_l2_norm, cfg, rv[r], rg[r], ra[r]);
            }
            continue;
        }
        apply_relation_row<G, IT>(w, rel, rel_acc, ld, lane, cfg, ws, copies_folded);
    }
    if (blockIdx.x == 0 && threadIdx.x < 64) {
        double s = 0.0;
        for (int i = threadIdx.x; i < n_partials; i += 64) s += ws.partials[i];
        s = oea::wave_sum_d(s);
        if (threadIdx.x == 0) *loss_accum += s;
    }
}

template <int G, int IT>
__global__ __launch_bounds__(256) void apply_step_plan(float *__restrict__ ent, float *__restrict__ ent_acc, int64_t n_ent,
                                                       float *__restrict__ rel, float *__restrict__ rel_acc, int64_t n_rel, int ld,
                                                       oea_step_cfg cfg, StepWs ws, int n_partials, double *__restrict__ loss_accum,
                                                       int copies_folded, int rel_blocks, int scan_blocks,
                                                       const uint4 *__restrict__ recs, const uint32_t *__restrict__ vals,
                                                       const int32_t *__restrict__ step_first, int s, const uint8_t *__restrict__ inplan,
                                                       const float *__restrict__ contrib) {
    constexpr int GPB = 256 / G, GPW = 64 / G;
    const int lane = threadIdx.x % G;
    const int b = (int)blockIdx.x, nb = (int)gridDim.x;
    if (b < rel_blocks) {
        for (int64_t row = (int64_t)b * GPB + threadIdx.x / G; row < n_rel; row += (int64_t)rel_blocks * GPB)
            apply_relation_row<G, IT>(row, rel, rel_acc, ld, lane, cfg, ws, copies_folded);
    } else if (b >= rel_blocks + scan_blocks && b < nb - 1) {
        const int plan_blocks = nb - 1 - rel_blocks - scan_blocks;
        const int64_t grp = (int64_t)(b - rel_blocks - scan_blocks) * GPB + threadIdx.x / G, ngrp = (int64_t)plan_blocks * GPB;
        const int64_t i1 = step_first[s + 1];
        for (int64_t i = step_first[s] + grp; i < i1; i += ngrp) {
            const uint4 rec = recs[i];
            if (rec.z > oea::kPlanHubEntries) continue;
            const int64_t row = rec.x;
            const uint32_t e0 = rec.y, e1 = rec.y + rec.z, v0 = rec.w;
            const float flag = (float)ws.ent_touched[row];
            Row<G, IT> rv, ra, rg, rc;
            load_row<G, IT>(ent + row * ld, ld, lane, rv);
            if (cfg.opt_kind == OEA_OPT_ADAGRAD) load_row<G, IT>(ent_acc + row * ld, ld, lane, ra);
            load_row<G, IT>(contrib + (int64_t)(v0 & 0x7fffffffu) * ld, ld, lane, rc);
#pragma unroll
            for (int it = 0; it < IT; ++it) rg.v[it] = (v0 >> 31) ? -rc.v[it] : rc.v[it];
            for (uint32_t e = e0 + 1; e < e1; e += 3) {
                uint32_t ve[3];
                Row<G, IT> r3[3];
#pragma unroll
                for (int u = 0; u < 3; ++u) ve[u] = vals[min(e + u, e1 - 1)];
#pragma unroll
                for (int u = 0; u < 3; ++u) load_row<G, IT>(contrib + (int64_t)(ve[u] & 0x7fffffffu) * ld, ld, lane, r3[u]);
#pragma unroll
                for (int u = 0; u < 3; ++u)
                    if (e + u < e1) {
#pragma unroll
                        for (int it = 0; it < IT; ++it) rg.v[it] += (ve[u] >> 31) ? -r3[u].v[it] : r3[u].v[it];
                    }
            }
            if (flag != 0.f) {
                grad_t *g = ws.ent_grad + row * ld;
                Row<G, IT> rs;
                load_grad_row<G, IT>(g, ld, lane, rs);
#pragma unroll
                for (int it = 0; it < IT; ++it) {
                    rg.v[it] += rs.v[it];
                    const int c = it * G + lane;
                    if (c < ld) g[c] = 0;
                }
                if (lane == 0) ws.ent_touched[row] = 0;
            }
            apply_one_row<G, IT, false>(ent + row * ld, ent_acc + row * ld, nullptr, nullptr, ld, lane, cfg.ent_l2_norm, cfg, rv, rg, ra);
        }
    } else if (b < nb - 1) {
        const int first = rel_blocks;
        const int wl = threadIdx.x & 63, gw = wl / G;
        const int64_t wave = (int64_t)(b - first) * 4 + (threadIdx.x >> 6), nwave = (int64_t)scan_blocks * 4;
        const int64_t n_chunk = (n_ent + 63) / 64;
        const uint8_t *mine = inplan + (int64_t)s * n_ent;
        for (int64_t chunk = wave; chunk < n_chunk; chunk += nwave) {
            const int64_t r = (int64_t)wl * n_chunk + chunk;
            const bool todo = r < n_ent && (float)ws.ent_touched[r] != 0.f && mine[r] == 0;
            unsigned long long mask = __ballot(todo);
            while (mask) {
                int64_t row = -1;
#pragma unroll
                for (int q = 0; q < GPW; ++q)
                    if (mask) {
                        const int bit = __builtin_ctzll(mask);
                        mask &= mask - 1;
                        if (gw == q) row = (int64_t)bit * n_chunk + chunk;
                    }
                if (row >= 0) {
                    Row<G, IT> rv, rg, ra;
                    load_row<G, IT>(ent + row * ld, ld, lane, rv);
                    load_grad_row<G, IT>(ws.ent_grad + row * ld, ld, lane, rg);
                    if (cfg.opt_kind == OEA_OPT_ADAGRAD) load_row<G, IT>(ent_acc + row * ld, ld, lane, ra);
                    apply_one_row<G, IT>(ent + row * ld, ent_acc + row * ld, ws.ent_grad + row * ld, ws.ent_touched + row, ld, lane,
                                         cfg.ent_l2_norm, cfg, rv, rg, ra);
                }
            }
        }
    } else {
        __shared__ double sp[256];
        double v[16];
#pragma unroll
        for (int u = 0; u < 16; ++u) { const int i = u * 256 + (int)threadIdx.x; v[u] = i < n_partials ? ws.partials[i] : 0.0; }
        double acc = 0.0;
#pragma unroll
        for (int u = 0; u < 16; ++u) acc += v[u];
        sp[threadIdx.x] = acc;
        __syncthreads();
        for (int o = 128; o > 0; o >>= 1) {
            if ((int)threadIdx.x < o) sp[threadIdx.x] += sp[threadIdx.x + o];
            __syncthreads();
        }
        if (threadIdx.x == 0) *loss_accum += sp[0];
    }
}

#ifndef OEA_DET_SCRATCH
template <int IT4>
struct Row4 {
    float4 v[IT4];
};
template <int G, int IT4>
__device__ __forceinline__ void load_row4(const float *__restrict__ base, int ld, int lane, Row4<IT4> &r) {
#pragma unroll
    for (int it = 0; it < IT4; ++it) {
        const int c = (it * G + lane) * 4;
        r.v[it] = c < ld ? oea::ld4(base + c) : make_float4(0.f, 0.f, 0.f, 0.f);
    }
}
__device__ __forceinline__ float4 f4_axpy(float a, float4 x, float4 y) { return make_float4(fmaf(a, x.x, y.x), fmaf(a, x.y, y.y), fmaf(a, x.z, y.z), fmaf(a, x.w, y.w)); }
__device__ __forceinline__ float4 f4_add(float4 x, float4 y) { return make_float4(x.x + y.x, x.y + y.y, x.z + y.z, x.w + y.w); }
__device__ __forceinline__ float f4_dot(float4 x, float4 y) { return x.x * y.x + x.y * y.y + x.z * y.z + x.w * y.w; }

template <int G, int IT4, bool CLEAR>
__device__ __forceinline__ void apply_one_row4(float *__restrict__ v, float *__restrict__ acc, float *__restrict__ g, flag_t *__restrict__ touched_flag,
                                               int ld, int lane, int on, const oea_step_cfg &cfg, const Row4<IT4> &rv, const Row4<IT4> &rg,
                                               const Row4<IT4> &ra) {
    float inv = 1.f, ydg = 0.f;
    if (on) {
        float ss = 0.f, dot = 0.f;
#pragma unroll
        for (int it = 0; it < IT4; ++it) { ss += f4_dot(rv.v[it], rv.v[it]); dot += f4_dot(rv.v[it], rg.v[it]); }
        ss = group_sum<G>(ss);
        inv = rsqrtf(fmaxf(ss, 1e-12f));
        dot = group_sum<G>(dot) * inv;
        ydg = ss > 1e-12f ? dot : 0.f;
    }
#pragma unroll
    for (int it = 0; it < IT4; ++it) {
        const int c = (it * G + lane) * 4;
        if (c < ld) {
            float4 gv = rg.v[it];
            const float4 y = rv.v[it];
            if (on)
                gv = make_float4((gv.x - y.x * inv * ydg) * inv, (gv.y - y.y * inv * ydg) * inv, (gv.z - y.z * inv * ydg) * inv,
                                 (gv.w - y.w * inv * ydg) * inv);
            float4 nv;
            if (cfg.opt_kind == OEA_OPT_ADAGRAD) {
                const float4 a = make_float4(ra.v[it].x + gv.x * gv.x, ra.v[it].y + gv.y * gv.y, ra.v[it].z + gv.z * gv.z,
                                             ra.v[it].w + gv.w * gv.w);
                oea::st4(acc + c, a);
                nv = make_float4(rv.v[it].x - cfg.lr * gv.x / sqrtf(a.x), rv.v[it].y - cfg.lr * gv.y / sqrtf(a.y),
                                 rv.v[it].z - cfg.lr * gv.z / sqrtf(a.z), rv.v[it].w - cfg.lr * gv.w / sqrtf(a.w));
            } else {
                nv = make_float4(y.x - cfg.lr * gv.x, y.y - cfg.lr * gv.y, y.z - cfg.lr * gv.z, y.w - cfg.lr * gv.w);
            }
            oea::st4(v + c, nv);
            if (CLEAR) oea::st4(g + c, make_float4(0.f, 0.f, 0.f, 0.f));
        }
    }
    if (CLEAR && lane == 0) *touched_flag = 0;
}

template <int G, int IT>
__global__ __launch_bounds__(256) void apply_step_plan_v4(float *__restrict__ ent, float *__restrict__ ent_acc, int64_t n_ent,
                                                          float *__restrict__ rel, float *__restrict__ rel_acc, int64_t n_rel, int ld,
                                                          oea_step_cfg cfg, StepWs ws, int n_partials, double *__restrict__ loss_accum,
                                                          int copies_folded, int rel_blocks, int scan_blocks,
                                                          const uint4 *__restrict__ recs, const uint32_t *__restrict__ vals,
                                                          const int32_t *__restrict__ step_first, int s, const uint8_t *__restrict__ inplan,
                                                          const float *__restrict__ contrib) {
    constexpr int GPB = 256 / G, GPW = 64 / G, IT4 = (IT + 3) / 4;
    const int lane = threadIdx.x % G;
    const int b = (int)blockIdx.x, nb = (int)gridDim.x;
    if (b < rel_blocks) {
        for (int64_t row = (int64_t)b * GPB + threadIdx.x / G; row < n_rel; row += (int64_t)rel_blocks * GPB)
            apply_relation_row<G, IT>(row, rel, rel_acc, ld, lane, cfg, ws, copies_folded);
    } else if (b >= rel_blocks + scan_blocks && b < nb - 1) {
        const int plan_blocks = nb - 1 - rel_blocks - scan_blocks;
        const int64_t grp = (int64_t)(b - rel_blocks - scan_blocks) * GPB + threadIdx.x / G, ngrp = (int64_t)plan_blocks * GPB;
        const int64_t i1 = step_first[s + 1];
        for (int64_t i = step_first[s] + grp; i < i1; i += ngrp) {
            const uint4 rec = recs[i];
            if (rec.z > oea::kPlanHubEntries) continue;
            const int64_t row = rec.x;
            const uint32_t e0 = rec.y, e1 = rec.y + rec.z, v0 = rec.w;
            const float flag = (float)ws.ent_touched[row];
            Row4<IT4> rv, ra, rg, rc;
            load_row4<G, IT4>(ent + row * ld, ld, lane, rv);
            if (cfg.opt_kind == OEA_OPT_ADAGRAD) load_row4<G, IT4>(ent_acc + row * ld, ld, lane, ra);
            load_row4<G, IT4>(contrib + (int64_t)(v0 & 0x7fffffffu) * ld, ld, lane, rc);
            const float s0 = (v0 >> 31) ? -1.f : 1.f;
#pragma unroll
            for (int it = 0; it < IT4; ++it) rg.v[it] = make_float4(s0 * rc.v[it].x, s0 * rc.v[it].y, s0 * rc.v[it].z, s0 * rc.v[it].w);
            for (uint32_t e = e0 + 1; e < e1; e += 3) {
                uint32_t ve[3];
                Row4<IT4> r3[3];
#pragma unroll
                for (int u = 0; u < 3; ++u) ve[u] = vals[min(e + u, e1 - 1)];
#pragma unroll
                for (int u = 0; u < 3; ++u) load_row4<G, IT4>(contrib + (int64_t)(ve[u] & 0x7fffffffu) * ld, ld, lane, r3[u]);
#pragma unroll
                for (int u = 0; u < 3; ++u)
                    if (e + u < e1) {
                        const float su = (ve[u] >> 31) ? -1.f : 1.f;
#pragma unroll
                        for (int it = 0; it < IT4; ++it) rg.v[it] = f4_axpy(su, r3[u].v[it], rg.v[it]);
                    }
            }
            if (flag != 0.f) {
                float *g = ws.ent_grad + row * ld;
                Row4<IT4> rs;
                load_row4<G, IT4>(g, ld, lane, rs);
#pragma unroll
                for (int it = 0; it < IT4; ++it) {
                    rg.v[it] = f4_add(rg.v[it], rs.v[it]);
                    const int c = (it * G + lane) * 4;
                    if (c < ld) oea::st4(g + c, make_float4(0.f, 0.f, 0.f, 0.f));
                }
                if (lane == 0) ws.ent_touched[row] = 0;
            }
            apply_one_row4<G, IT4, false>(ent + row * ld, ent_acc + row * ld, nullptr, nullptr, ld, lane, cfg.ent_l2_norm, cfg, rv, rg, ra);
        }
    } else if (b < nb - 1) {
        const int first = rel_blocks;
        const int wl = threadIdx.x & 63, gw = wl / G;
        const int64_t wave = (int64_t)(b - first) * 4 + (threadIdx.x >> 6), nwave = (int64_t)scan_blocks * 4;
        const int64_t n_chunk = (n_ent + 63) / 64;
        const uint8_t *mine = inplan + (int64_t)s * n_ent;
        for (int64_t chunk = wave; chunk < n_chunk; chunk += nwave) {
            const int64_t r = (int64_t)wl * n_chunk + chunk;
            const bool todo = r < n_ent && (float)ws.ent_touched[r] != 0.f && mine[r] == 0;
            unsigned long long mask = __ballot(todo);
            while (mask) {
                int64_t row = -1;
#pragma unroll
                for (int q = 0; q < GPW; ++q)
                    if (mask) {
                        const int bit = __builtin_ctzll(mask);
                        mask &= mask - 1;
                        if (gw == q) row = (int64_t)bit * n_chunk + chunk;
                    }
                if (row >= 0) {
                    Row4<IT4> rv, rg, ra;
                    load_row4<G, IT4>(ent + row * ld, ld, lane, rv);
                    load_row4<G, IT4>(ws.ent_grad + row * ld, ld, lane, rg);
                    if (cfg.opt_kind == OEA_OPT_ADAGRAD) load_row4<G, IT4>(ent_acc + row * ld, ld, lane, ra);
                    apply_one_row4<G, IT4, true>(ent + row * ld, ent_acc + row * ld, ws.ent_grad + row * ld, ws.ent_touched + row, ld, lane,
                                                 cfg.ent_l2_norm, cfg, rv, rg, ra);
                }
            }
        }
    } else {
        __shared__ double sp[256];
        double v[16];
#pragma unroll
        for (int u = 0; u < 16; ++u) { const int i = u * 256 + (int)threadIdx.x; v[u] = i < n_partials ? ws.partials[i] : 0.0; }
        double acc = 0.0;
#pragma unroll
        for (int u = 0; u < 16; ++u) acc += v[u];
        sp[threadIdx.x] = acc;
        __syncthreads();
        for (int o = 128; o > 0; o >>= 1) {
            if ((int)threadIdx.x < o) sp[threadIdx.x] += sp[threadIdx.x + o];
            __syncthreads();
        }
        if (threadIdx.x == 0) *loss_accum += sp[0];
    }
}
#endif

template <int G, int IT>
__global__ __launch_bounds__(256) void apply_rows_dense(float *__restrict__ ent, float *__restrict__ ent_state,
                                                        int64_t n_ent, float *__restrict__ rel,
                                                        float *__restrict__ rel_state, int64_t n_rel, int ld,
                                                        oea_step_cfg cfg, StepWs ws, int n_partials,
                                                        double *__restrict__ loss_accum, float lr_t) {
    const int lane = threadIdx.x % G;
    const int64_t grp = ((int64_t)blockIdx.x * blockDim.x + threadIdx.x) / G;
    const int64_t ngrp = (int64_t)gridDim.x * blockDim.x / G;
    for (int64_t row_all = grp; row_all < n_ent + n_rel; row_all += ngrp) {
        const bool is_rel = row_all < n_rel;
        const int64_t row = is_rel ? row_all : row_all - n_rel;
        const int64_t rows = is_rel ? n_rel : n_ent;
        flag_t *touched = is_rel ? ws.rel_touched : ws.ent_touched;
        float *v = (is_rel ? rel : ent) + row * ld;
        float *s0 = (is_rel ? rel_state : ent_state) + row * ld;
        float *s1 = s0 + rows * (int64_t)ld;
        grad_t *g = (is_rel ? ws.rel_grad : ws.ent_grad) + row * ld;
        const int on = is_rel ? cfg.rel_l2_norm : cfg.ent_l2_norm;
        const float flag = (float)touched[row];
        if (cfg.opt_kind == OEA_OPT_ADADELTA && !on && flag == 0.f) continue;
        Row<G, IT> rv, rg, r0, r1;
        load_row<G, IT>(v, ld, lane, rv);
        load_grad_row<G, IT>(g, ld, lane, rg);
        load_row<G, IT>(s0, ld, lane, r0);
        load_row<G, IT>(s1, ld, lane, r1);
        float inv = 1.f, ydg = 0.f;
        if (on) {
            const float ss = sumsq<G, IT>(rv);
            inv = rsqrtf(fmaxf(ss, 1e-12f));
            float dot = 0.f;
#pragma unroll
            for (int it = 0; it < IT; ++it) dot += rv.v[it] * rg.v[it];
            dot = group_sum<G>(dot) * inv;
            ydg = ss > 1e-12f ? dot : 0.f;
        }
#pragma unroll
        for (int it = 0; it < IT; ++it) {
            const int c = it * G + lane;
            if (c < ld) {
                const float gv = on ? (rg.v[it] - rv.v[it] * inv * ydg) * inv : rg.v[it];
                if (cfg.opt_kind == OEA_OPT_ADAM) {
                    const float m = r0.v[it] + (gv - r0.v[it]) * (1.f - cfg.beta1);
                    const float vv = r1.v[it] + (gv * gv - r1.v[it]) * (1.f - cfg.beta2);
                    s0[c] = m; s1[c] = vv;
                    v[c] = rv.v[it] - lr_t * m / (sqrtf(vv) + cfg.eps);
                } else {
                    const float acc = r0.v[it] * cfg.beta1 + gv * gv * (1.f - cfg.beta1);
                    const float upd = sqrtf(r1.v[it] + cfg.eps) * rsqrtf(acc + cfg.eps) * gv;
                    s0[c] = acc;
                    s1[c] = r1.v[it] * cfg.beta1 + upd * upd * (1.f - cfg.beta1);
                    v[c] = rv.v[it] - cfg.lr * upd;
                }
                if (flag != 0.f) g[c] = 0;
            }
        }
        if (flag != 0.f && lane == 0) touched[row] = 0;
    }
    if (blockIdx.x == 0 && threadIdx.x < 64) {
        double s = 0.0;
        for (int i = threadIdx.x; i < n_partials; i += 64) s += ws.partials[i];
// ... 273 lines not shown
    const int64_t grp = ((int64_t)blockIdx.x * blockDim.x + threadIdx.x) / G;
    const int64_t ngrp = (int64_t)gridDim.x * blockDim.x / G;
    for (int64_t w = grp; w < rpr + n_rel; w += ngrp) {
        Row<G, IT> rv, rg, ra;
        if (w >= rpr) {
            const int64_t r = w - rpr;
            if (rel_x[n_rel * ld + r] == 0) continue;
            load_row<G, IT>(rel + r * ld, ld, lane, rv);
            load_grad_row<G, IT>(rel_x + r * ld, ld, lane, rg);
            if (cfg.opt_kind == OEA_OPT_ADAGRAD) load_row<G, IT>(rel_acc + r * ld, ld, lane, ra);
            flag_t dummy;
            apply_one_row<G, IT>(rel + r * ld, rel_acc + r * ld, rel_x + r * ld, &dummy, ld, lane, cfg.rel_l2_norm, cfg, rv, rg, ra);
            continue;
        }
        const int64_t j = w, id = j * world + rank;
        if (id >= n_ent || ws.ent_touched[id] == 0) continue;
        float *v = ent + id * ld;
        load_row<G, IT>(v, ld, lane, rv);
        load_grad_row<G, IT>(ws.ent_grad + id * ld, ld, lane, rg);
        if (cfg.opt_kind == OEA_OPT_ADAGRAD) load_row<G, IT>(acc_own + j * ld, ld, lane, ra);
        apply_one_row<G, IT>(v, acc_own + j * ld, ws.ent_grad + id * ld, ws.ent_touched + id, ld, lane, cfg.ent_l2_norm, cfg, rv, rg, ra);
    }
    if (blockIdx.x == 0 && threadIdx.x < 64) {
        double s = 0.0;
        for (int i = threadIdx.x; i < n_partials; i += 64) s += ws.partials[i];
        s = oea::wave_sum_d(s);
        if (threadIdx.x == 0) *loss_accum += s;
    }
}

__global__ void halo_rel_pack_kernel(StepWs ws, int64_t n_rel, int ld, grad_t *__restrict__ rel_x) {
    const int64_t total = n_rel * ld;
    for (int64_t i = (int64_t)blockIdx.x * blockDim.x + threadIdx.x; i < total; i += (int64_t)gridDim.x * blockDim.x) {
        const int64_t r = i / ld;
        const flag_t f = ws.rel_touched[r];
        rel_x[i] = f != 0 ? ws.rel_grad[i] : (grad_t)0;
        if (f != 0) ws.rel_grad[i] = 0;
    }
}
__global__ void halo_rel_flags_kernel(StepWs ws, int64_t n_rel, int ld, grad_t *__restrict__ rel_x) {
    const int64_t r = (int64_t)blockIdx.x * blockDim.x + threadIdx.x;
    if (r < n_rel) { rel_x[n_rel * ld + r] = ws.rel_touched[r]; ws.rel_touched[r] = 0; }
}

template <bool PACK>
__global__ void halo_pull_kernel(float *__restrict__ ent, int ld, HaloGeom g, const int32_t *__restrict__ lists_s ,
                                 const int32_t *__restrict__ own_off, const int32_t *__restrict__ pfx, float *__restrict__ buf) {
    const int cpr = ld / 4;
    const int64_t total = (int64_t)pfx[g.world] * cpr;
    for (int64_t i = (int64_t)blockIdx.x * blockDim.x + threadIdx.x; i < total; i += (int64_t)gridDim.x * blockDim.x) {
        const int64_t q = i / cpr;
        const int c = (int)(i - q * cpr);
        const int peer = halo_peer_of(pfx, g.world, q);
        if (peer == g.rank) continue;
        if (PACK) {
            const int64_t j = lists_s[(int64_t)peer * g.cap + own_off[peer] + (q - pfx[peer])];
            oea::st4(buf + q * ld + 4 * c, oea::ld4(ent + (j * g.world + g.rank) * ld + 4 * c));
        } else {
            const int64_t j = lists_s[q];
            oea::st4(ent + (j * g.world + peer) * ld + 4 * c, oea::ld4(buf + q * ld + 4 * c));
        }
    }
}

__global__ void halo_owned_rows_kernel(const float *__restrict__ ent, int64_t n_ent, int ld, int world, int rank, int64_t rpr,
                                       float *__restrict__ upd) {
    const int cpr = ld / 4;
    const int64_t total = rpr * cpr;
    for (int64_t i = (int64_t)blockIdx.x * blockDim.x + threadIdx.x; i < total; i += (int64_t)gridDim.x * blockDim.x) {
        const int64_t j = i / cpr, id = j * world + rank;
        const int c = (int)(i - j * cpr);
        oea::st4(upd + j * ld + 4 * c, id < n_ent ? oea::ld4(ent + id * ld + 4 * c) : make_float4(0.f, 0.f, 0.f, 0.f));
    }
}

static bool step_wave_enabled() {
    static const int env = [] { const char *e = getenv("OEA_STEP_WAVE"); return e ? atoi(e) : 1; }();
    return env != 0;
}

template <int IT64>
void launch_wave(int nb, int block, hipStream_t st, const float *ent, const float *rel, int ld, const int32_t *pos,
                 int64_t n_pos, const int32_t *neg, const oea_step_cfg &cfg, const StepWs &ws, float *contrib = nullptr,
                 const uint32_t *pflags = nullptr, const uint32_t *order = nullptr) {
    const int k = cfg.neg_group_k;
    static const int dbg = [] { const char *e = getenv("OEA_STEP_WAVE_DBG"); return e ? atoi(e) : 0; }();
#define OEA_WAVE(L1, KT)                                                                                                               \
    do {                                                                                                                               \
        if (contrib) oea::launch_timed(triple_wave<IT64, L1, KT, true>, nb, block, st, ent, rel, ld, pos, n_pos, neg, k, cfg, ws, dbg, contrib, pflags, order);   \
        else oea::launch_timed(triple_wave<IT64, L1, KT, false>, nb, block, st, ent, rel, ld, pos, n_pos, neg, k, cfg, ws, dbg, contrib, pflags, nullptr);          \
    } while (0)
    if (k == 10) { if (cfg.l1) OEA_WAVE(1, 10); else OEA_WAVE(0, 10); }
    else { if (cfg.l1) OEA_WAVE(1, 0); else OEA_WAVE(0, 0); }
#undef OEA_WAVE
}

static bool step_runtime_kind() {
    static const int env = [] { const char *e = getenv("OEA_STEP_RUNTIME_KIND"); return e ? atoi(e) : 0; }();
    return env != 0;
}

static bool wave_rule(const oea_step_cfg &cfg, int64_t n_ent, int64_t n_rel, int32_t ld) {
    return cfg.score_kind == OEA_SCORE_TRANSE && cfg.loss_kind == OEA_LOSS_LIMITED && cfg.ent_l2_norm && cfg.rel_l2_norm &&
           cfg.neg_group_k >= 1 && cfg.neg_group_k <= 10 && ld <= 256 &&
           std::max(n_ent, n_rel) * (int64_t)ld * (int64_t)sizeof(grad_t) < ((int64_t)1 << 30) && step_wave_enabled() &&
           !step_runtime_kind();
}

template <int G, int IT>
void launch_grouped(int nb, int block, hipStream_t st, const float *ent, const float *rel, int ld, const int32_t *pos,
                    int64_t n_pos, const int32_t *neg, const oea_step_cfg &cfg, const StepWs &ws, bool wave, float *contrib = nullptr,
                    const uint32_t *pflags = nullptr, const uint32_t *order = nullptr) {
    const bool runtime_kind = step_runtime_kind();
    const int k = cfg.neg_group_k;
    if constexpr ((G == 32 && IT <= 4) || (G == 64 && IT == 4)) {
        if (wave) {
            constexpr int IT64 = G == 32 ? (IT + 1) / 2 : 4;
            static const int blk_env = [] { const char *e = getenv("OEA_STEP_WAVE_BLOCK"); return e ? atoi(e) : 0; }();
            const int wblock = G == 32 ? (blk_env == 256 || blk_env == 512 ? blk_env : 512) : (block / G) * 64;
            launch_wave<IT64>(nb, wblock, st, ent, rel, ld, pos, n_pos, neg, cfg, ws, contrib, pflags, order);
            return;
        }
    }
#define OEA_GROUPED(LOSS, L1) oea::launch_timed(triple_grouped<G, IT, LOSS, L1>, nb, block, st, ent, rel, ld, pos, n_pos, neg, k, cfg, ws)
    if (runtime_kind) OEA_GROUPED(-1, -1);
    else if (cfg.loss_kind == OEA_LOSS_LIMITED) { if (cfg.l1) OEA_GROUPED(OEA_LOSS_LIMITED, 1); else OEA_GROUPED(OEA_LOSS_LIMITED, 0); }
    else if (cfg.loss_kind == OEA_LOSS_LOGISTIC) { if (cfg.l1) OEA_GROUPED(OEA_LOSS_LOGISTIC, 1); else OEA_GROUPED(OEA_LOSS_LOGISTIC, 0); }
    else if (cfg.loss_kind == OEA_LOSS_POSITIVE) { if (cfg.l1) OEA_GROUPED(OEA_LOSS_POSITIVE, 1); else OEA_GROUPED(OEA_LOSS_POSITIVE, 0); }
    else OEA_GROUPED(-1, -1);
#undef OEA_GROUPED
}

static bool apply_g16(int64_t n_ent, int64_t n_rel, int32_t ld) {
    static const int env_g16 = [] { const char *e = getenv("OEA_APPLY_G16"); return e ? atoi(e) : -1; }();
    return env_g16 >= 0 ? env_g16 != 0 : (n_ent + n_rel) * (int64_t)ld * 12 > (int64_t)128 << 20;
}

static int64_t step_items(const oea_step_cfg &cfg, int64_t n_pos, int64_t n_neg) {
    const bool transh = cfg.score_kind == OEA_SCORE_TRANSH, transd = cfg.score_kind == OEA_SCORE_TRANSD;
    const bool transh_grouped = transh && cfg.loss_kind != OEA_LOSS_MARGIN && (n_neg == 0 || cfg.neg_group_k > 0);
    const bool projected = transd || (transh && !transh_grouped);
    const bool grouped = transh_grouped || (!projected && cfg.neg_group_k > 0 && cfg.loss_kind != OEA_LOSS_MARGIN);
    return (grouped || cfg.loss_kind == OEA_LOSS_MARGIN) ? n_pos : n_pos + n_neg;
}

static int loss_partials(int32_t ld, int64_t n_items) {
    const int gpb = 256 / (ld <= 128 ? 32 : 64);
    return n_items > 0 ? (int)std::min<int64_t>(std::max<int64_t>(oea::ceil_div(n_items, gpb), 1), kMaxBlocks) : 0;
}

template <int V>
using int_c = std::integral_constant<int, V>;

template <class F>
static int for_row_width(int32_t ld, F &&f) {
    if (ld <= 32) f(int_c<32>{}, int_c<1>{});
    else if (ld <= 64) f(int_c<32>{}, int_c<2>{});
    else if (ld <= 96) f(int_c<32>{}, int_c<3>{});
    else if (ld <= 128) f(int_c<32>{}, int_c<4>{});
    else if (ld <= 256) f(int_c<64>{}, int_c<4>{});
    else if (ld <= 512) f(int_c<64>{}, int_c<8>{});
    else if (ld <= 1280) f(int_c<64>{}, int_c<20>{});
    else { oea::set_error("ld %d > 1280 unsupported", ld); return OEA_EUNSUPPORTED; }
    return OEA_OK;
}

template <class F>
static void for_width16(int32_t ld, F &&f) {
    const int it16 = (ld + 15) / 16;
    if (it16 <= 2) f(int_c<2>{});
    else if (it16 <= 4) f(int_c<4>{});
    else if (it16 == 5) f(int_c<5>{});
    else if (it16 == 6) f(int_c<6>{});
    else if (it16 == 7) f(int_c<7>{});
    else f(int_c<8>{});
}

template <int G, int IT>
int launch_step(float *ent, float *ent_acc, int64_t n_ent, float *rel, float *rel_acc, int64_t n_rel,
                int32_t ld, const int32_t *pos, int64_t n_pos, const int32_t *neg, int64_t n_neg,
                const oea_step_cfg &cfg, const StepWs &ws, double *loss_accum, int phase, hipStream_t st,
                const oea::StepPlanView *plan = nullptr, int plan_step = 0, int64_t plan_first_pos = 0) {
    const int block = 256, gpb = block / G;
    const bool transh = cfg.score_kind == OEA_SCORE_TRANSH, transd = cfg.score_kind == OEA_SCORE_TRANSD;
    const bool dense_opt = cfg.opt_kind == OEA_OPT_ADAM || cfg.opt_kind == OEA_OPT_ADADELTA;
    const bool transh_grouped = transh && cfg.loss_kind != OEA_LOSS_MARGIN && (n_neg == 0 || cfg.neg_group_k > 0);
    const bool projected = transd || (transh && !transh_grouped);
    const bool grouped = transh_grouped || (!projected && cfg.neg_group_k > 0 && cfg.loss_kind != OEA_LOSS_MARGIN);
    const int64_t items = step_items(cfg, n_pos, n_neg);
    const int n_part = loss_partials(ld, items);
    const int nb1 = std::max(n_part, 1);
    if (phase != OEA_PHASE_APPLY) {
        oea::prof_call();
        if (transd)
            oea::launch_timed(triple_projected<G, IT, OEA_SCORE_TRANSD>, nb1, block, st, ent, rel, ld, pos, n_pos, neg, n_neg, cfg, ws);
        else if (projected)
            oea::launch_timed(triple_projected<G, IT, OEA_SCORE_TRANSH>, nb1, block, st, ent, rel, ld, pos, n_pos, neg, n_neg, cfg, ws);
        else if (transh)
            oea::launch_timed(triple_transh_grouped<G, IT>, nb1, block, st, ent, rel, ld, pos, n_pos, neg, n_neg ? cfg.neg_group_k : 0, cfg, ws);
        else if (grouped) {
            static const bool rel_order_on = [] { const char *e = getenv("OEA_STEP_REL_ORDER"); return !(e && e[0] == '0'); }();
            launch_grouped<G, IT>(nb1, block, st, ent, rel, ld, pos, n_pos, neg, cfg, ws, wave_rule(cfg, n_ent, n_rel, ld),
                                  plan ? plan->contrib : nullptr, plan ? plan->pflags + plan_first_pos : nullptr,
                                  plan && rel_order_on ? plan->rel_order + plan_first_pos : nullptr);
        }
        else
            oea::launch_timed(triple_generic<G, IT>, nb1, block, st, ent, rel, ld, pos, n_pos, neg, n_neg, cfg, ws);
        if (phase == OEA_PHASE_GRAD || dense_opt)
            fold_rel_copies_kernel<<<(unsigned)std::min<int64_t>(oea::ceil_div(n_rel * (int64_t)ld, 256), 1024), 256, 0, st>>>(
                ws, n_rel * (int64_t)ld, transh ? 1 : 0);
    }
    const int nb2 = (int)std::min<int64_t>(std::max<int64_t>(oea::ceil_div(n_ent + n_rel, gpb), 1), 16384);
    if (phase != OEA_PHASE_GRAD) {
        hipEvent_t ev0 = nullptr, ev1 = nullptr;
        (void)oea::prof_pair(&ev0, &ev1);
        if (dense_opt) {
            const double t = (double)cfg.opt_t;
            const float lr_t = cfg.opt_kind == OEA_OPT_ADAM
                                   ? (float)((double)cfg.lr * std::sqrt(1.0 - std::pow((double)cfg.beta2, t)) / (1.0 - std::pow((double)cfg.beta1, t)))
                                   : cfg.lr;
            oea::launch_events(apply_rows_dense<G, IT>, nb2, block, st, ev0, ev1, ent, ent_acc, n_ent, rel, rel_acc, n_rel, ld, cfg, ws,
                              n_part, loss_accum, lr_t);
        } else {
            static const int env_r = [] { const char *e = getenv("OEA_APPLY_ROWS"); return e ? atoi(e) : 0; }();
            const int R = env_r ? env_r : 1;
            const int folded = phase == OEA_PHASE_APPLY;
            static const int flag_first_env = [] { const char *e = getenv("OEA_APPLY_FLAG_FIRST"); return e ? atoi(e) : 0; }();
            const int flag_first = plan ? 1 : flag_first_env;
            auto nb = [&](int r) { return (int)std::min<int64_t>(std::max<int64_t>(oea::ceil_div(n_rel + oea::ceil_div(n_ent, r), gpb), 1), 16384); };
            const bool g16 = apply_g16(n_ent, n_rel, ld);
            if (plan) {
                static_assert(kMaxBlocks <= 16 * 256, "the partials block reads 16 per lane");
                const int64_t bound = 2 * n_pos;
                const int pgpb = g16 && G == 32 ? 16 : gpb;
                const int relb = (int)std::max<int64_t>(oea::ceil_div(n_rel, pgpb), 1);
                const int planb = (int)std::min<int64_t>(std::max<int64_t>(oea::ceil_div(bound, pgpb), 1), 8192);
                const int scanb = (int)std::min<int64_t>(std::max<int64_t>(oea::ceil_div(n_ent, 256), 1), 4096);
                auto launch = [&](auto kernel) {
                    oea::launch_events(kernel, relb + planb + scanb + 1, block, st, ev0, ev1, ent, ent_acc, n_ent, rel, rel_acc, n_rel, ld, cfg,
                                       ws, n_part, loss_accum, folded, relb, scanb, plan->recs, plan->vals_b, plan->step_first, plan_step,
                                       plan->inplan, plan->contrib);
                };
                if (g16 && G == 32)
                    for_width16(ld, [&](auto it) {
                        constexpr int IT16 = decltype(it)::value;
#ifndef OEA_DET_SCRATCH
                        static const bool v4 = [] { const char *e = getenv("OEA_APPLY_V4"); return !(e && e[0] == '0'); }();
                        if (v4) return launch(apply_step_plan_v4<16, IT16>);
#endif
                        launch(apply_step_plan<16, IT16>);
                    });
                else
                    launch(apply_step_plan<G, IT>);
            } else
            if (g16 && G == 32 && R == 1) {
                const int nbg = (int)std::min<int64_t>(std::max<int64_t>(oea::ceil_div(n_rel + n_ent, 16), 1), 16384);
                for_width16(ld, [&](auto it) {
                    oea::launch_events(apply_rows<16, decltype(it)::value, 1>, nbg, block, st, ev0, ev1, ent, ent_acc, n_ent, rel, rel_acc, n_rel,
                                       ld, cfg, ws, n_part, loss_accum, folded, flag_first);
                });
            } else
            if (R >= 4 && IT <= 4)
                oea::launch_events(apply_rows<G, IT, 4>, nb(4), block, st, ev0, ev1, ent, ent_acc, n_ent, rel, rel_acc, n_rel, ld, cfg, ws, n_part, loss_accum, folded, flag_first);
            else if (R >= 2 && IT <= 8)
                oea::launch_events(apply_rows<G, IT, 2>, nb(2), block, st, ev0, ev1, ent, ent_acc, n_ent, rel, rel_acc, n_rel, ld, cfg, ws, n_part, loss_accum, folded, flag_first);
            else
                oea::launch_events(apply_rows<G, IT, 1>, nb(1), block, st, ev0, ev1, ent, ent_acc, n_ent, rel, rel_acc, n_rel, ld, cfg, ws, n_part, loss_accum, folded, flag_first);
        }
        if (transh)
            apply_normal_rows<G, IT><<<(unsigned)std::max<int64_t>(oea::ceil_div(n_rel, gpb), 1), block, 0, st>>>(
                n_rel, ld, cfg, ws, phase == OEA_PHASE_APPLY);
    }
    return 0;
}

template <class F>
static int for_apply_width(int64_t n_ent, int64_t n_rel, int32_t ld, F &&f) {
    if (ld > 128 || !apply_g16(n_ent, n_rel, ld)) return for_row_width(ld, f);
    for_width16(ld, [&](auto it) { f(int_c<16>{}, it); });
    return OEA_OK;
}

}

void oea::step_scratch_rows(void *workspace, int64_t n_ent, int64_t n_rel, int32_t ld, grad_t **ent_grad, flag_t **ent_touched,
                            grad_t **rel_grad, flag_t **rel_touched) {
    StepWs ws;
    ws_layout(n_ent, n_rel, ld, workspace, &ws);
    *ent_grad = ws.ent_grad; *ent_touched = ws.ent_touched; *rel_grad = ws.rel_grad; *rel_touched = ws.rel_touched;
}

#define OEA_TRY_RC(...) do { const int _rc = (__VA_ARGS__); if (_rc != OEA_OK) return _rc; } while (0)

extern "C" {

size_t oea_step_workspace_bytes(int64_t n_ent, int64_t n_rel, int32_t ld) {
    return ws_layout(n_ent, n_rel, ld, nullptr, nullptr);
}

size_t oea_step_exchange_floats(int64_t n_ent, int64_t n_rel, int32_t ld) {
    StepWs ws;
    ws_layout(n_ent, n_rel, ld, reinterpret_cast<void *>(256), &ws);
    return (size_t)(reinterpret_cast<char *>(ws.rel_extra) - reinterpret_cast<char *>(256)) / sizeof(grad_t);
}

int32_t oea_step_scratch_elem_bytes(void) { return (int32_t)sizeof(grad_t); }

static int step_phase_impl(float *ent, float *ent_acc, int64_t n_ent, float *rel, float *rel_acc,
                           int64_t n_rel, int32_t dim, int32_t ld, const int32_t *pos, int64_t n_pos,
                           const int32_t *neg, int64_t n_neg, const oea_step_cfg *cfg, void *workspace,
                           double *loss_accum, int32_t phase, void *stream, const oea::StepPlanView *plan, int plan_step,
                           int64_t plan_first_pos) {
    OEA_REQUIRE(phase >= OEA_PHASE_BOTH && phase <= OEA_PHASE_APPLY, "phase");
    OEA_REQUIRE(ent && rel && (pos || n_pos == 0) && cfg && workspace && loss_accum, "null pointer");
    OEA_REQUIRE(ld % 4 == 0 && dim <= ld && dim > 0, "ld % 4 == 0 and dim <= ld");
    OEA_REQUIRE(n_pos >= 0 && n_neg >= 0 && (neg || n_neg == 0), "neg == NULL needs n_neg == 0");
    OEA_REQUIRE(cfg->loss_kind >= OEA_LOSS_MARGIN && cfg->loss_kind <= OEA_LOSS_ALIGN, "loss_kind");
    OEA_REQUIRE(cfg->opt_kind >= OEA_OPT_SGD && cfg->opt_kind <= OEA_OPT_ADADELTA, "opt_kind");
    OEA_REQUIRE(cfg->opt_kind == OEA_OPT_SGD || phase == OEA_PHASE_GRAD || (ent_acc && rel_acc),
                "Adagrad / Adam / Adadelta need their state arrays (the GRAD phase alone does not)");
    if (cfg->opt_kind == OEA_OPT_ADAM || cfg->opt_kind == OEA_OPT_ADADELTA) {
        OEA_REQUIRE(cfg->score_kind != OEA_SCORE_TRANSH, "Adam / Adadelta are not built for the TransH normal-vector table");
        OEA_REQUIRE(cfg->opt_kind != OEA_OPT_ADAM || cfg->opt_t >= 1, "Adam: opt_t = 1-based step count");
        OEA_REQUIRE(cfg->beta1 > 0.f && cfg->beta1 < 1.f && cfg->eps > 0.f, "beta1 / eps");
    }
    if (cfg->loss_kind == OEA_LOSS_MARGIN) OEA_REQUIRE(n_neg == n_pos, "margin loss pairs pos i with neg i");
    if (cfg->loss_kind == OEA_LOSS_POSITIVE || cfg->loss_kind == OEA_LOSS_ALIGN)
        OEA_REQUIRE(n_neg == 0, "positive-only loss takes no negatives");
    OEA_REQUIRE(cfg->neg_group_k >= 0 && (cfg->neg_group_k == 0 || n_neg == n_pos * (int64_t)cfg->neg_group_k),
                "neg_group_k > 0 needs n_neg == n_pos * neg_group_k");
    OEA_REQUIRE(cfg->score_kind >= OEA_SCORE_TRANSE && cfg->score_kind <= OEA_SCORE_TRANSD, "score_kind");
    if (cfg->score_kind == OEA_SCORE_TRANSH)
        OEA_REQUIRE(cfg->normal && (cfg->opt_kind != OEA_OPT_ADAGRAD || cfg->normal_acc), "TransH needs the normal_vector table (+ accumulator)");
    if (cfg->score_kind == OEA_SCORE_TRANSD)
        OEA_REQUIRE(cfg->ent_transfer_base > 0 && cfg->rel_transfer_base > 0 && 2 * (int64_t)cfg->ent_transfer_base == n_ent &&
                        2 * (int64_t)cfg->rel_transfer_base == n_rel,
// ... 58 lines not shown
    OEA_REQUIRE(grad_offset_bytes && touched_offset_bytes, "null pointer");
    StepWs ws;
    ws_layout(n_ent, n_rel, ld, reinterpret_cast<void *>(256), &ws);
    *grad_offset_bytes = reinterpret_cast<char *>(ws.nrm_grad) - reinterpret_cast<char *>(256);
    *touched_offset_bytes = reinterpret_cast<char *>(ws.nrm_touched) - reinterpret_cast<char *>(256);
    return OEA_OK;
}

int oea_step_apply_normals(int64_t n_ent, int64_t n_rel, int32_t ld, const oea_step_cfg *cfg, void *workspace, void *stream) {
    OEA_REQUIRE(cfg && workspace && ld % 4 == 0, "arguments");
    OEA_REQUIRE(cfg->score_kind == OEA_SCORE_TRANSH && cfg->normal, "TransH score with its normal-vector table");
    OEA_REQUIRE(cfg->opt_kind == OEA_OPT_SGD || (cfg->opt_kind == OEA_OPT_ADAGRAD && cfg->normal_acc), "SGD or Adagrad (+ state)");
    if (n_rel == 0) return OEA_OK;
    StepWs ws;
    ws_layout(n_ent, n_rel, ld, workspace, &ws);
    hipStream_t st = oea::as_stream(stream);
    OEA_TRY_RC(for_row_width(ld, [&](auto g, auto it) {
        constexpr int G = decltype(g)::value;
        apply_normal_rows<G, decltype(it)::value><<<(unsigned)std::max<int64_t>(oea::ceil_div(n_rel, 256 / G), 1), 256, 0, st>>>(n_rel, ld, *cfg, ws, 1);
    }));
    OEA_CHECK_HIP(hipGetLastError());
    return OEA_OK;
}

int64_t oea_step_items(const oea_step_cfg *cfg, int64_t n_pos, int64_t n_neg) { return cfg ? step_items(*cfg, n_pos, n_neg) : -1; }

int oea_part_pack(void *workspace, int64_t n_ent, int64_t n_rel, int32_t ld, int32_t world, void *send_, void *rel_x_,
                  void *stream) {
    grad_t *send = static_cast<grad_t *>(send_), *rel_x = static_cast<grad_t *>(rel_x_);
    OEA_REQUIRE(workspace && send && rel_x && world >= 1 && ld % 4 == 0, "arguments");
    StepWs ws;
    ws_layout(n_ent, n_rel, ld, workspace, &ws);
    const int64_t rpr = oea_part_rows_per_rank(n_ent, world);
    hipStream_t st = oea::as_stream(stream);
    OEA_TRY_RC(for_row_width(ld, [&](auto g, auto it) {
        constexpr int G = decltype(g)::value;
        part_pack_kernel<G, decltype(it)::value><<<(unsigned)std::min<int64_t>(oea::ceil_div(world * rpr + n_rel, 256 / G), 16384), 256, 0, st>>>(
            ws, n_ent, n_rel, ld, world, rpr, send, rel_x);
    }));
    OEA_CHECK_HIP(hipGetLastError());
    return OEA_OK;
}

int oea_part_apply(float *ent, float *acc_own, int64_t n_ent, float *rel, float *rel_acc, int64_t n_rel, int32_t ld,
                   int32_t world, int32_t rank, void *own_, void *rel_x_, float *upd, const oea_step_cfg *cfg, void *workspace,
                   int64_t n_items, double *loss_accum, void *stream) {
    grad_t *own = static_cast<grad_t *>(own_), *rel_x = static_cast<grad_t *>(rel_x_);
    OEA_REQUIRE(ent && rel && own && rel_x && upd && cfg && workspace && loss_accum, "null pointer");
    OEA_REQUIRE(world >= 1 && rank >= 0 && rank < world && ld % 4 == 0, "world / rank / ld");
    OEA_REQUIRE(cfg->opt_kind == OEA_OPT_SGD || (cfg->opt_kind == OEA_OPT_ADAGRAD && acc_own && rel_acc), "SGD or Adagrad (+ state)");
    OEA_REQUIRE(cfg->score_kind >= OEA_SCORE_TRANSE && cfg->score_kind <= OEA_SCORE_TRANSD, "score_kind");
    StepWs ws;
    ws_layout(n_ent, n_rel, ld, workspace, &ws);
    const int64_t rpr = oea_part_rows_per_rank(n_ent, world);
    hipStream_t st = oea::as_stream(stream);
    const int n_part = loss_partials(ld, n_items);
    OEA_TRY_RC(for_apply_width(n_ent, n_rel, ld, [&](auto g, auto it) {
        constexpr int G = decltype(g)::value;
        oea::launch_timed(part_apply_kernel<G, decltype(it)::value>,
                          (unsigned)std::min<int64_t>(std::max<int64_t>(oea::ceil_div(rpr + n_rel, 256 / G), 1), 16384), 256, st, ent, acc_own,
                          n_ent, rel, rel_acc, n_rel, ld, world, rank, rpr, own, rel_x, upd, *cfg, ws, n_part, loss_accum);
    }));
    OEA_CHECK_HIP(hipGetLastError());
    return OEA_OK;
}

int oea_part_unpack(float *ent, int64_t n_ent, int32_t ld, int32_t world, int32_t rank, const float *all, void *stream) {
    OEA_REQUIRE(ent && all && world >= 1 && rank >= 0 && rank < world && ld % 4 == 0, "arguments");
    if (world == 1) return OEA_OK;
    const int64_t rpr = oea_part_rows_per_rank(n_ent, world);
    part_unpack_kernel<<<(unsigned)std::min<int64_t>(oea::ceil_div(n_ent * (ld / 4), 256), 16384), 256, 0, oea::as_stream(stream)>>>(
        ent, n_ent, ld, world, rank, rpr, all);
    OEA_CHECK_HIP(hipGetLastError());
    return OEA_OK;
}

int32_t oea_step_plan_supported(const oea_step_cfg *cfg, int64_t n_ent, int64_t n_rel, int32_t ld, int32_t k) {
    static const int env = [] { const char *e = getenv("OEA_STEP_PLAN"); return e ? atoi(e) : 1; }();
    if (!cfg || env == 0 || oea::kDetScratch) return 0;
    if (env != 2 && !apply_g16(n_ent, n_rel, ld)) return 0;
    return wave_rule(*cfg, n_ent, n_rel, ld) && cfg->neg_group_k == k && (cfg->opt_kind == OEA_OPT_SGD || cfg->opt_kind == OEA_OPT_ADAGRAD);
}

}

static_assert(sizeof(oea_epoch) == 184, "oea_epoch: openea_amd/_lib.py:Epoch and tests/test_host_cpu.py hold the same layout");

struct EpochStep {
    int32_t s;
    int64_t lo, n, r_lo, split;
    const int32_t *pos;
    int32_t *negs;
};

struct EpochWalk {
    const oea_epoch *e;
    int32_t step_begin, step_end, rank, world;
    bool presampled, ahead, sample_all;
    int64_t max_batch;
    oea_step_cfg cfg;
    void *stream;
};

static int epoch_walk_begin(const oea_epoch *e, int32_t step_begin, int32_t step_end, int32_t rank, int32_t world, void *stream,
                            EpochWalk *w) {
    OEA_REQUIRE(e && e->pos_all && e->offsets_host && e->splits_host && e->cfg, "null pointer");
    OEA_REQUIRE(e->steps >= 0 && e->k >= 0, "steps, k >= 0");
    OEA_REQUIRE(0 <= step_begin && step_begin <= step_end && step_end <= e->steps, "0 <= step_begin <= step_end <= steps");
    OEA_REQUIRE((e->offsets_dev == nullptr) == (e->splits_dev == nullptr), "offsets_dev and splits_dev go together");
    OEA_REQUIRE(world >= 1 && rank >= 0 && rank < world, "0 <= rank < world");
    const int32_t k = e->k, steps = e->steps;
    const bool presampled = k > 0 && e->side0 == nullptr && e->side1 == nullptr && e->offsets_dev != nullptr;
    OEA_REQUIRE(k == 0 || (e->neg_buf && (presampled || (e->err_flag && e->side0 && e->side1))),
                "sampling needs neg_buf, err_flag and both sides");
    const bool ahead = k > 0 && e->offsets_dev != nullptr && steps > 0;
    const bool sample_all = ahead && !presampled && step_begin == 0;
    if (sample_all)
        OEA_TRY_RC(oea_sample_negatives_epoch(e->pos_all, e->offsets_host[steps], e->offsets_dev, e->splits_dev, steps, k, e->side0, e->side1,
                                              e->seed, e->step_base, 10, e->neg_buf, e->err_flag, stream));
    int64_t max_batch = 0;
    for (int32_t s = 0; s < steps; ++s) max_batch = std::max(max_batch, e->offsets_host[s + 1] - e->offsets_host[s]);
    *w = EpochWalk{e, step_begin, step_end, rank, world, presampled, ahead, sample_all, max_batch, *e->cfg, stream};
    return OEA_OK;
}

template <class F>
static int epoch_walk(EpochWalk &w, F &&step) {
    const oea_epoch &e = *w.e;
    for (int32_t s = w.step_begin; s < w.step_end; ++s) {
        const int64_t b0 = e.offsets_host[s], nb = e.offsets_host[s + 1] - b0;
        if (nb <= 0) continue;
        const int64_t r_lo = nb * w.rank / w.world, r_hi = nb * (w.rank + 1) / w.world;
        const int64_t lo = b0 + r_lo, n = r_hi - r_lo;
        const int64_t split = std::min(std::max<int64_t>(e.splits_host[s] - r_lo, 0), n);
        int32_t *negs = e.k == 0 ? nullptr : w.ahead ? e.neg_buf + 3 * lo * (int64_t)e.k : e.neg_buf;
        const EpochStep t{s, lo, n, r_lo, split, e.pos_all + 3 * lo, negs};
        if (n > 0 && e.k > 0 && !w.presampled && !w.sample_all)
            OEA_TRY_RC(oea_sample_negatives_pair(t.pos, n, split, e.k, e.side0, e.side1, e.seed, e.step_base + (uint32_t)s, (uint32_t)r_lo, 10,
                                                 negs, e.err_flag, w.stream));
        OEA_TRY_RC(step(t));
        ++w.cfg.opt_t;
    }
    return OEA_OK;
}

static HaloGeom halo_geom(int64_t n_ent, int32_t world, int32_t rank, int64_t max_batch, int32_t k) {
    HaloGeom g;
    g.world = world; g.rank = rank;
    g.rpr = oea_part_rows_per_rank(n_ent, world);
    g.rpr32 = (g.rpr + 31) / 32 * 32;
    g.nwords = (int)((int64_t)world * g.rpr32 / 32);
    const int64_t share = oea::ceil_div(max_batch, world) + 1;
    g.cap = std::min<int64_t>(2 * share * (1 + (int64_t)k), (int64_t)world * g.rpr);
    g.cap = (g.cap + 3) / 4 * 4;
    return g;
}
struct HaloWs { uint32_t *bitmaps; int32_t *lists, *counts, *tables, *err; };
static size_t halo_ws_layout(const HaloGeom &g, int32_t steps, void *base, HaloWs *ws) {
    size_t off = 0;
    char *b = static_cast<char *>(base);
    auto take = [&](size_t bytes) { size_t o = off; off += align256(bytes); return b ? b + o : nullptr; };
    uint32_t *bm = (uint32_t *)take(4 * (size_t)steps * g.world * g.nwords);
    int32_t *li = (int32_t *)take(4 * (size_t)steps * g.world * g.cap);
    int32_t *co = (int32_t *)take(4 * (size_t)steps * g.world * g.world);
    int32_t *ta = (int32_t *)take(4 * (size_t)steps * 4 * (g.world + 1));
    int32_t *er = (int32_t *)take(256);
    if (ws) { ws->bitmaps = bm; ws->lists = li; ws->counts = co; ws->tables = ta; ws->err = er; }
    return off;
}

static int halo_build_lists(const int32_t *pos_all, const int32_t *neg_all, int32_t k, const int64_t *offsets_host,
                            const int64_t *offsets_dev, int32_t step_begin, int32_t step_end, const HaloGeom &g, const HaloWs &hw,
                            hipStream_t st) {
    const int32_t nS = step_end - step_begin;
    OEA_CHECK_HIP(hipMemsetAsync(hw.bitmaps, 0, 4 * (size_t)nS * g.world * g.nwords, st));
    OEA_CHECK_HIP(hipMemsetAsync(hw.err, 0, 4, st));
    const int64_t rows = offsets_host[step_end] - offsets_host[step_begin];
    if (rows > 0)
        halo_mark_kernel<<<(unsigned)std::min<int64_t>(oea::ceil_div(rows * (k + 1), 256), 16384), 256, 0, st>>>(
            pos_all, neg_all, k, offsets_dev, step_begin, step_end, g, hw.bitmaps);
    halo_compact_kernel<<<(unsigned)(nS * g.world), 256, 0, st>>>(hw.bitmaps, g, hw.lists, hw.counts, hw.err);
    return OEA_OK;
}

extern "C" {

int oea_triple_epoch_range(const oea_epoch *e, int32_t step_begin, int32_t step_end, int32_t rank, int32_t world, void *plan,
                           size_t plan_bytes, int32_t plan_built, void *stream) {
    EpochWalk w;
    OEA_TRY_RC(epoch_walk_begin(e, step_begin, step_end, rank, world, stream, &w));
    oea::StepPlanView pv;
    const bool use_plan = plan && world == 1 && w.ahead && (w.presampled || w.sample_all) &&
                          oea_step_plan_supported(e->cfg, e->n_ent, e->n_rel, e->ld, e->k);
    if (use_plan) {
        const int64_t n_total = e->offsets_host[e->steps];
        const size_t need = oea::step_plan_layout(n_total, e->steps, w.max_batch, e->n_ent, e->ld, plan, &pv);
        OEA_REQUIRE(plan_bytes >= need, "plan workspace smaller than oea_step_plan_bytes");
        if (!plan_built)
            OEA_TRY_RC(oea_step_plan_build(e->pos_all, e->neg_buf, e->k, e->offsets_dev, n_total, e->steps, w.max_batch, e->n_ent, e->ld, plan,
                                           plan_bytes, stream));
    }
    return epoch_walk(w, [&](const EpochStep &t) -> int {
        if (t.n == 0) return OEA_OK;
        return step_phase_impl(e->ent, e->ent_acc, e->n_ent, e->rel, e->rel_acc, e->n_rel, e->dim, e->ld, t.pos, t.n, t.negs,
                               t.n * (int64_t)e->k, &w.cfg, e->workspace, e->loss_accum, OEA_PHASE_BOTH, stream,
                               use_plan ? &pv : nullptr, t.s, t.lo);
    });
}

int oea_triple_epoch_range_comm(oea_comm_t comm, const oea_epoch *e, int32_t step_begin, int32_t step_end, void *send, void *own,
                                void *rel_x, float *upd, float *all, void *stream) {
    OEA_REQUIRE(comm && e && e->pos_all && e->offsets_host && e->splits_host && e->cfg && send && own && rel_x && upd && all, "null pointer");
    OEA_REQUIRE(e->steps >= 0 && e->k >= 0 && 0 <= step_begin && step_begin <= step_end && step_end <= e->steps, "step range");
    OEA_REQUIRE(e->cfg->opt_kind == OEA_OPT_SGD || e->cfg->opt_kind == OEA_OPT_ADAGRAD, "the partition runs SGD / Adagrad");
    const int32_t world = oea_comm_size(comm), rank = oea_comm_rank(comm);
    EpochWalk w;
    OEA_TRY_RC(epoch_walk_begin(e, step_begin, step_end, rank, world, stream, &w));
    const int64_t n_ent = e->n_ent, n_rel = e->n_rel;
    const int32_t ld = e->ld, k = e->k;
    const int64_t rpr = oea_part_rows_per_rank(n_ent, world);
    const int64_t chunk = rpr * (ld + 1);
    const bool transh = e->cfg->score_kind == OEA_SCORE_TRANSH;
    StepWs ws;
    ws_layout(n_ent, n_rel, ld, e->workspace, &ws);
    const int32_t gdt = oea::kDetScratch ? OEA_COMM_I64 : OEA_COMM_F32;
    hipStream_t st = oea::as_stream(stream);
    return epoch_walk(w, [&](const EpochStep &t) -> int {
        OEA_TRY_RC(oea::comm_phase_mark(comm, st));
        OEA_TRY_RC(oea_triple_step_phase(e->ent, nullptr, n_ent, e->rel, e->rel_acc, n_rel, e->dim, ld, t.pos, t.n, t.negs, t.n * (int64_t)k,
                                         &w.cfg, e->workspace, e->loss_accum, OEA_PHASE_GRAD, stream));
        OEA_TRY_RC(oea::comm_phase_mark(comm, st));
        OEA_TRY_RC(oea_part_pack(e->workspace, n_ent, n_rel, ld, world, send, rel_x, stream));
        OEA_TRY_RC(oea::comm_phase_mark(comm, st));
        OEA_TRY_RC(oea_comm_reduce_scatter(comm, send, own, chunk, gdt, stream));
        OEA_TRY_RC(oea_comm_allreduce(comm, rel_x, n_rel * (int64_t)(ld + 1), gdt, stream));
        if (transh) {
            OEA_TRY_RC(oea_comm_allreduce(comm, ws.nrm_grad, n_rel * (int64_t)ld, gdt, stream));
            OEA_TRY_RC(oea_comm_allreduce(comm, ws.nrm_touched, n_rel, gdt, stream));
        }
        OEA_TRY_RC(oea::comm_phase_mark(comm, st));
        OEA_TRY_RC(oea_part_apply(e->ent, e->ent_acc, n_ent, e->rel, e->rel_acc, n_rel, ld, world, rank, own, rel_x, upd, &w.cfg, e->workspace,
                                  step_items(w.cfg, t.n, t.n * (int64_t)k), e->loss_accum, stream));
        if (transh) OEA_TRY_RC(oea_step_apply_normals(n_ent, n_rel, ld, &w.cfg, e->workspace, stream));
        OEA_TRY_RC(oea::comm_phase_mark(comm, st));
        OEA_TRY_RC(oea_allgather_rows(comm, upd, all, rpr, ld, stream));
        OEA_TRY_RC(oea::comm_phase_mark(comm, st));
        OEA_TRY_RC(oea_part_unpack(e->ent, n_ent, ld, world, rank, all, stream));
        return oea::comm_phase_mark(comm, st);
    });
}

size_t oea_halo_workspace_bytes(int64_t n_ent, int32_t world, int32_t steps, int64_t max_batch, int32_t k) {
    if (world < 1 || steps < 0) return 0;
    return halo_ws_layout(halo_geom(n_ent, world, 0, max_batch, k), steps, nullptr, nullptr);
}

size_t oea_halo_buffer_bytes(int64_t n_ent, int32_t world, int64_t max_batch, int32_t k, int32_t ld) {
    if (world < 1) return 0;
    const HaloGeom g = halo_geom(n_ent, world, 0, max_batch, k);
    const int64_t rows = std::max<int64_t>(g.cap, (int64_t)(world - 1) * std::min<int64_t>(g.cap, g.rpr));
    return align256((size_t)rows * (ld + 1) * sizeof(grad_t));
}

int oea_halo_plan(const int32_t *pos_all, const int32_t *neg_all, int32_t k, const int64_t *offsets_host, const int64_t *offsets_dev,
                  int32_t steps, int32_t step_begin, int32_t step_end, int64_t n_ent, int32_t world, void *halo_ws, size_t halo_ws_bytes,
                  int32_t *counts_host, int32_t *lists_host, int64_t *cap_out, void *stream) {
    OEA_REQUIRE(pos_all && offsets_host && offsets_dev && halo_ws && counts_host, "null pointer");
    OEA_REQUIRE(steps >= 0 && k >= 0 && (k == 0 || neg_all) && 0 <= step_begin && step_begin <= step_end && step_end <= steps && world >= 1, "arguments");
    hipStream_t st = oea::as_stream(stream);
    const int32_t nS = step_end - step_begin;
    int64_t max_batch = 0;
    for (int32_t s = 0; s < steps; ++s) max_batch = std::max(max_batch, offsets_host[s + 1] - offsets_host[s]);
    const HaloGeom g = halo_geom(n_ent, world, 0, max_batch, k);
    if (cap_out) *cap_out = g.cap;
    if (nS == 0) return OEA_OK;
    HaloWs hw;
    OEA_REQUIRE(halo_ws_bytes >= halo_ws_layout(g, nS, halo_ws, &hw), "halo workspace smaller than oea_halo_workspace_bytes");
    OEA_TRY_RC(halo_build_lists(pos_all, neg_all, k, offsets_host, offsets_dev, step_begin, step_end, g, hw, st));
    int32_t err = 0;
    OEA_CHECK_HIP(hipMemcpyAsync(counts_host, hw.counts, 4 * (size_t)nS * world * world, hipMemcpyDeviceToHost, st));
    if (lists_host) OEA_CHECK_HIP(hipMemcpyAsync(lists_host, hw.lists, 4 * (size_t)nS * world * g.cap, hipMemcpyDeviceToHost, st));
    OEA_CHECK_HIP(hipMemcpyAsync(&err, hw.err, 4, hipMemcpyDeviceToHost, st));
    OEA_CHECK_HIP(hipStreamSynchronize(st));
// ... 153 lines not shown
```

### openea_amd/ops.py

```python
import ctypes as C
import math
import os

import numpy as np
import torch

from . import _lib
from ._lib import LOSS_KIND, METRIC, OPT_KIND, OpenEAHipError, RotateCfg, StepCfg, check


def lib():
    return _lib.load(require_device=True)


def _p(t):
    if t is None:
        return None
    assert t.is_cuda and t.is_contiguous(), "device-resident contiguous tensor required"
    return C.c_void_p(t.data_ptr())


def _stream():
    return C.c_void_p(torch.cuda.current_stream().cuda_stream)

# ... 872 lines not shown
                            0 if nbr is None else nbr.shape[1],
                            filt.data_ptr() if filt is not None else None, 0 if filt is None else 32 * filt.numel())
    side._keep = (table, entity_list, ent_pos, nbr, filt)
    return side


def sample_negatives_pair(pos, n_split, k, side0, side1, seed, step, pos_offset, out, err_flag, max_try=10):
    check(lib().oea_sample_negatives_pair(_p(pos), pos.shape[0], int(n_split), k, C.byref(side0), C.byref(side1),
                                          int(seed), int(step), int(pos_offset), int(max_try), _p(out), _p(err_flag),
                                          _stream()))
    return out


def sample_negatives_epoch(pos_all, offsets_dev, splits_dev, steps, k, side0, side1, seed, step_base, out, err_flag, max_try=10):
    check(lib().oea_sample_negatives_epoch(_p(pos_all), pos_all.shape[0], _p(offsets_dev), _p(splits_dev), int(steps), int(k),
                                           C.byref(side0), C.byref(side1), int(seed), int(step_base), int(max_try), _p(out),
                                           _p(err_flag), _stream()))
    return out


def _epoch(ent, ent_acc, rel, rel_acc, dim, pos_all, offsets, splits, k, side0, side1, seed, step_base, neg_buf, err_flag, cfg,
           workspace, loss_accum, offsets_dev, splits_dev, step_range):
    offsets, splits = np.ascontiguousarray(offsets, np.int64), np.ascontiguousarray(splits, np.int64)
    steps = len(splits)
    e = _lib.Epoch(_p(ent), _p(ent_acc), ent.shape[0], _p(rel), _p(rel_acc), rel.shape[0], dim, ent.shape[1],
                   _p(pos_all), offsets.ctypes.data, splits.ctypes.data, steps, _p(offsets_dev), _p(splits_dev),
                   int(k), C.pointer(side0) if side0 is not None else None, C.pointer(side1) if side1 is not None else None,
                   int(seed), int(step_base), _p(neg_buf), _p(err_flag), C.pointer(cfg), _p(workspace), _p(loss_accum))
    e._keep = (offsets, splits)
    lo, hi = (0, steps) if step_range is None else step_range
    return e, int(lo), int(hi)


def triple_epoch(ent, ent_acc, rel, rel_acc, dim, pos_all, offsets, splits, k, side0, side1, seed, step_base,
                 neg_buf, err_flag, cfg, workspace, loss_accum, offsets_dev=None, splits_dev=None, step_range=None, shard=(0, 1),
                 plan=None):
    e, lo, hi = _epoch(ent, ent_acc, rel, rel_acc, dim, pos_all, offsets, splits, k, side0, side1, seed, step_base, neg_buf, err_flag,
                       cfg, workspace, loss_accum, offsets_dev, splits_dev, step_range)
    buf, built = plan if plan is not None else (None, False)
    check(lib().oea_triple_epoch_range(C.byref(e), lo, hi, int(shard[0]), int(shard[1]), _p(buf), buf.numel() if buf is not None else 0,
                                       int(bool(built)), _stream()))


def epoch_layout(triples, n1, n2, slot, seed, epoch, dall, workspace=None):
    n = int(n1) + int(n2)
    if workspace is None:
        workspace = torch.empty(lib().oea_epoch_layout_bytes(n), dtype=torch.uint8, device=triples.device)
    check(lib().oea_epoch_layout(_p(triples), int(n1), int(n2), _p(slot), slot.numel(), int(seed) & 0xFFFFFFFFFFFFFFFF, int(epoch) & 0xFFFFFFFF,
                                 _p(dall), _p(workspace), workspace.numel(), _stream()))
    return workspace


def step_plan_supported(cfg, n_ent, n_rel, ld, k):
    return bool(lib().oea_step_plan_supported(C.byref(cfg), int(n_ent), int(n_rel), int(ld), int(k)))


def step_plan_buffer(n_total, steps, max_batch, n_ent, ld, dev=None):
    nbytes = lib().oea_step_plan_bytes(int(n_total), int(steps), int(max_batch), int(n_ent), int(ld))
    return torch.empty(nbytes, dtype=torch.uint8, device=dev or device())


def step_plan_build(pos_all, neg_all, k, offsets_dev, n_total, steps, max_batch, n_ent, ld, plan):
    check(lib().oea_step_plan_build(_p(pos_all), _p(neg_all), int(k), _p(offsets_dev), int(n_total), int(steps), int(max_batch),
                                    int(n_ent), int(ld), _p(plan), plan.numel(), _stream()))


def step_plan_arrays(plan, n_total, steps, max_batch, n_ent, ld):
    off = (C.c_int64 * 9)()
    check(lib().oea_step_plan_offsets(int(n_total), int(steps), int(max_batch), int(n_ent), int(ld), C.cast(off, C.c_void_p)))
    raw = plan.cpu().numpy()
    m = 2 * int(n_total)
    nu = int(raw[off[3]: off[3] + 4].view(np.int32)[0])
    return dict(vals=raw[off[0]: off[0] + 4 * m].view(np.uint32).copy(), ukeys=raw[off[1]: off[1] + 8 * nu].view(np.uint64).copy(),
                uoff=raw[off[2]: off[2] + 4 * (nu + 1)].view(np.uint32).copy(),
                step_first=raw[off[4]: off[4] + 4 * (steps + 1)].view(np.int32).copy(), row_bits=int(off[6]), n_unique=nu,
                pflags=raw[off[8]: off[8] + 4 * int(n_total)].view(np.uint32).copy())


def step_plan_rel_order(plan, n_total, steps, max_batch, n_ent, ld):
    off = C.c_int64(0)
    check(lib().oea_step_plan_rel_order_offset(int(n_total), int(steps), int(max_batch), int(n_ent), int(ld), C.cast(C.byref(off), C.c_void_p)))
    n = int(n_total)
    return plan[off.value: off.value + 4 * n].cpu().numpy().view(np.uint32).copy()


def step_plan_stats(plan, n_total, steps, max_batch, n_ent, ld):
    a = step_plan_arrays(plan, n_total, steps, max_batch, n_ent, ld)
    last = int(a["step_first"][steps])
    cnt = np.diff(a["uoff"].astype(np.int64))[:last]
    listed = int(a["uoff"][last])
    hub = cnt > 8
    return dict(positives=int(n_total), outside_rule=int(n_total - listed // 2), rows_per_step=float(last) / max(steps, 1),
                refs_per_row_mean=float(cnt.mean()) if last else 0.0, refs_per_row_max=int(cnt.max()) if last else 0,
                hub_rows_per_step=float(hub.sum()) / max(steps, 1), refs_to_hub_rows=int(cnt[hub].sum()),
                refs_listed=listed)


def comm_single_or_none():
    uid = (C.c_char * 128)()
    check(lib().oea_comm_unique_id(uid))
    comm = C.c_void_p()
    check(lib().oea_comm_init(uid, 0, 1, C.byref(comm)))
    return comm


def part_buffers(n_ent, n_rel, ld, world, dev, adagrad=True):
    rpr = lib().oea_part_rows_per_rank(int(n_ent), int(world))
    chunk = rpr * (ld + 1)
    f = dict(dtype=torch.float32, device=dev)
    g = dict(dtype=scratch_dtype(), device=dev)
    return dict(rpr=rpr, chunk=chunk, send=torch.empty(world * chunk, **g), own=torch.empty(chunk, **g),
                rel_x=torch.empty(n_rel * (ld + 1), **g), upd=torch.empty((rpr, ld), **f), all=torch.empty((world, rpr, ld), **f),
                acc_own=torch.full((rpr, ld), 0.1, **f) if adagrad else None)


def triple_epoch_comm(comm, ent, acc_own, rel, rel_acc, dim, pos_all, offsets, splits, k, side0, side1, seed, step_base, neg_buf,
                      err_flag, cfg, workspace, loss_accum, offsets_dev, splits_dev, bufs, step_range=None):
    e, lo, hi = _epoch(ent, acc_own, rel, rel_acc, dim, pos_all, offsets, splits, k, side0, side1, seed, step_base, neg_buf, err_flag,
                       cfg, workspace, loss_accum, offsets_dev, splits_dev, step_range)
    check(lib().oea_triple_epoch_range_comm(comm, C.byref(e), lo, hi, _p(bufs['send']), _p(bufs['own']), _p(bufs['rel_x']),
                                            _p(bufs['upd']), _p(bufs['all']), _stream()))


def halo_buffers(n_ent, ld, world, steps, max_batch, k, dev):
    wsb = lib().oea_halo_workspace_bytes(int(n_ent), int(world), int(steps), int(max_batch), int(k))
    xb = lib().oea_halo_buffer_bytes(int(n_ent), int(world), int(max_batch), int(k), int(ld))
    u8 = dict(dtype=torch.uint8, device=dev)
    return dict(ws=torch.empty(wsb, **u8), a=torch.empty(xb, **u8), b=torch.empty(xb, **u8), key=(int(steps), int(max_batch), int(k)))


def halo_plan(pos_all, neg_all, k, offsets, n_ent, world, step_range=None, with_lists=True):
    offsets = np.ascontiguousarray(offsets, np.int64)
    steps = len(offsets) - 1
    lo, hi = (0, steps) if step_range is None else step_range
    max_batch = int(np.diff(offsets).max()) if steps else 0
    dev = pos_all.device
    ws = torch.empty(lib().oea_halo_workspace_bytes(int(n_ent), int(world), hi - lo, max_batch, int(k)), dtype=torch.uint8, device=dev)
    off_dev = torch.from_numpy(offsets).to(dev)
    counts = np.zeros((hi - lo, world, world), np.int32)
    cap = C.c_int64(0)
    check(lib().oea_halo_plan(_p(pos_all), _p(neg_all), int(k), offsets.ctypes.data_as(C.c_void_p), _p(off_dev), steps, int(lo), int(hi),
                              int(n_ent), int(world), _p(ws), ws.numel(), counts.ctypes.data_as(C.c_void_p), None, C.byref(cap), _stream()))
    lists = None
    if with_lists:
        lists = np.zeros((hi - lo, world, int(cap.value)), np.int32)
        check(lib().oea_halo_plan(_p(pos_all), _p(neg_all), int(k), offsets.ctypes.data_as(C.c_void_p), _p(off_dev), steps, int(lo), int(hi),
                                  int(n_ent), int(world), _p(ws), ws.numel(), counts.ctypes.data_as(C.c_void_p),
                                  lists.ctypes.data_as(C.c_void_p), C.byref(cap), _stream()))
    return counts, lists


def triple_epoch_halo(comm, ent, acc_own, rel, rel_acc, dim, pos_all, offsets, splits, k, side0, side1, seed, step_base, neg_buf,
                      err_flag, cfg, workspace, loss_accum, offsets_dev, splits_dev, bufs, halo, step_range=None):
    e, lo, hi = _epoch(ent, acc_own, rel, rel_acc, dim, pos_all, offsets, splits, k, side0, side1, seed, step_base, neg_buf, err_flag,
                       cfg, workspace, loss_accum, offsets_dev, splits_dev, step_range)
    stats = (C.c_int64 * 4)()
    check(lib().oea_triple_epoch_range_halo(comm, C.byref(e), lo, hi, _p(halo['ws']), halo['ws'].numel(), _p(halo['a']), _p(halo['b']),
                                            halo['a'].numel(), _p(bufs['rel_x']), _p(bufs['upd']), _p(bufs['all']),
                                            C.cast(stats, C.c_void_p), _stream()))
    return tuple(int(x) for x in stats)


def sample_link_negatives(n_pos, k, pos_links=None, ents1=None, ents2=None, nbr1=None, row1=None, nbr2=None, row2=None,
                          exclude=None, seed=0, step=0, scratch=None):
    truncated = nbr1 is not None
    m = (2 if truncated else 1) * k * n_pos
# ... 714 lines not shown
```

Baseline: 292.5 million triples/s.

## Screen truncated negatives with a bf16 normalized row shadow before full loads

After: 282.1 million triples/s. -3.6%, worse.

```diff
diff --git a/include/openea_hip.h b/include/openea_hip.h
--- a/include/openea_hip.h
+++ b/include/openea_hip.h
@@ -336,6 +336,9 @@
                         int32_t steps, int64_t max_batch, int64_t n_ent, int32_t ld, void *plan, size_t plan_bytes, void *stream);
 int oea_step_plan_offsets(int64_t n_total, int32_t steps, int64_t max_batch, int64_t n_ent, int32_t ld, int64_t *out);
 int oea_step_plan_rel_order_offset(int64_t n_total, int32_t steps, int64_t max_batch, int64_t n_ent, int32_t ld, int64_t *out);
+int oea_step_plan_shadow_offset(int64_t n_total, int32_t steps, int64_t max_batch, int64_t n_ent, int32_t ld, int64_t *out);
+int oea_step_shadow_build(const float *ent, int64_t n_ent, int64_t n_rel, int32_t ld, void *plan, size_t plan_bytes, int64_t n_total,
+                          int32_t steps, int64_t max_batch, void *stream);
 
 struct oea_comm;
 int oea_triple_epoch_range_comm(struct oea_comm *comm, const oea_epoch *e, int32_t step_begin, int32_t step_end, void *send, void *own,
diff --git a/openea_amd/_lib.py b/openea_amd/_lib.py
--- a/openea_amd/_lib.py
+++ b/openea_amd/_lib.py
@@ -156,6 +156,8 @@
     "oea_step_plan_offsets": (C.c_int, [_i64, _i32, _i64, _i64, _i32, _vp]),
     "oea_step_plan_rel_order_offset": (C.c_int, [_i64, _i32, _i64, _i64, _i32, _vp]),
     "oea_step_plan_build": (C.c_int, [_vp, _vp, _i32, _vp, _i64, _i32, _i64, _i64, _i32, _vp, _sz, _vp]),
+    "oea_step_plan_shadow_offset": (C.c_int, [_i64, _i32, _i64, _i64, _i32, _vp]),
+    "oea_step_shadow_build": (C.c_int, [_vp, _i64, _i64, _i32, _vp, _sz, _i64, _i32, _i64, _vp]),
     "oea_triple_epoch_range_comm": (C.c_int, [_vp, C.POINTER(Epoch), _i32, _i32, _vp, _vp, _vp, _vp, _vp, _vp]),
     "oea_rotate_workspace_bytes": (_sz, [_i64, _i64, _i32]),
     "oea_rotate_exchange_doubles": (_sz, [_i64, _i64, _i32]),
diff --git a/openea_amd/csrc/common.h b/openea_amd/csrc/common.h
--- a/openea_amd/csrc/common.h
+++ b/openea_amd/csrc/common.h
@@ -164,6 +164,11 @@
 
 __device__ __forceinline__ float4 ld4(const float *p) { return *reinterpret_cast<const float4 *>(p); }
 __device__ __forceinline__ void st4(float *p, float4 v) { *reinterpret_cast<float4 *>(p) = v; }
+
+__device__ __forceinline__ uint32_t bf16_rne(float x) {
+    const uint32_t b = __builtin_bit_cast(uint32_t, x);
+    return x != x ? 0x7fc0u : (b + 0x7fffu + ((b >> 16) & 1u)) >> 16;
+}
 
 __device__ __forceinline__ uint4 philox4x32_10(uint32_t c0, uint32_t c1, uint32_t c2, uint32_t c3,
                                                uint32_t k0, uint32_t k1) {
diff --git a/openea_amd/csrc/step_plan.h b/openea_amd/csrc/step_plan.h
--- a/openea_amd/csrc/step_plan.h
+++ b/openea_amd/csrc/step_plan.h
@@ -20,8 +20,11 @@
     void *temp;
     size_t temp_bytes;
     uint32_t *rel_order;
+    uint32_t *shadow;
     int row_bits;
 };
+
+constexpr int shadow_words(int32_t ld) { return ((ld + 127) / 128) * 64; }
 
 constexpr uint32_t kPlanHubEntries = 8;
 
diff --git a/openea_amd/csrc/step_plan.hip b/openea_amd/csrc/step_plan.hip
--- a/openea_amd/csrc/step_plan.hip
+++ b/openea_amd/csrc/step_plan.hip
@@ -42,6 +42,7 @@
     w.temp_bytes = std::max(std::max(t1, std::max(t2, t3)), al256(4 * n1)) + 256;
     w.temp = take(w.temp_bytes);
     w.rel_order = (uint32_t *)take(4 * n1);
+    w.shadow = (uint32_t *)take(4 * (size_t)shadow_words(ld) * (size_t)n_ent);
     w.row_bits = bits_for((uint64_t)std::max<int64_t>(n_ent - 1, 1));
     if (v) *v = w;
     return off;
@@ -286,6 +287,15 @@
     return OEA_OK;
 }
 
+int oea_step_plan_shadow_offset(int64_t n_total, int32_t steps, int64_t max_batch, int64_t n_ent, int32_t ld, int64_t *out) {
+    OEA_REQUIRE(out && n_total >= 0 && steps >= 0 && n_ent > 0 && ld > 0, "arguments");
+    oea::StepPlanView v;
+    char *base = reinterpret_cast<char *>(4096);
+    (void)oea::step_plan_layout(n_total, steps, max_batch, n_ent, ld, base, &v);
+    *out = (char *)v.shadow - base;
+    return OEA_OK;
+}
+
 size_t oea_epoch_layout_bytes(int64_t n) {
     return n < 0 ? 0 : 256;
 }
diff --git a/openea_amd/csrc/triple_step.hip b/openea_amd/csrc/triple_step.hip
--- a/openea_amd/csrc/triple_step.hip
+++ b/openea_amd/csrc/triple_step.hip
@@ -433,11 +433,13 @@
     for (int it = 0; it < IT; ++it) r.v[it] *= inv;
 }
 
-template <int IT, int L1, int KT, bool PLAN>
+template <int IT, int L1, int KT, bool PLAN, bool SHD>
 __global__ __launch_bounds__(512, (IT <= 2 ? (KT == 10 ? 8 : 7) : 4)) void triple_wave(
     const float *__restrict__ ent, const float *__restrict__ rel, int ld, const int32_t *__restrict__ pos,
     int64_t n_pos, const int32_t *__restrict__ neg, int k, oea_step_cfg cfg, StepWs ws, int dbg, float *__restrict__ contrib,
-    const uint32_t *__restrict__ pflags, const uint32_t *__restrict__ order) {
+    const uint32_t *__restrict__ pflags, const uint32_t *__restrict__ order, const uint32_t *__restrict__ shadow, int shd_row_b,
+    float shd_thr) {
+    static_assert(!SHD || (PLAN && L1 == 0), "the row shadow serves planned L2 steps");
     constexpr int G = 64, KC = 10;
     if (KT > 0) k = KT;
     const int lane = threadIdx.x & 63;
@@ -449,6 +451,7 @@
     const __amdgpu_buffer_rsrc_t rs_rel = __builtin_amdgcn_make_buffer_rsrc(const_cast<float *>(rel), 0, (dbg & 2) ? 0 : kBufRecords, kBufFlags);
     const __amdgpu_buffer_rsrc_t rs_eg = __builtin_amdgcn_make_buffer_rsrc(ws.ent_grad, 0, (dbg & 1) ? 0 : kBufRecords, kBufFlags);
     const __amdgpu_buffer_rsrc_t rs_et = __builtin_amdgcn_make_buffer_rsrc(ws.ent_touched, 0, (dbg & 4) ? 0 : kBufRecords, kBufFlags);
+    const __amdgpu_buffer_rsrc_t rs_shd = __builtin_amdgcn_make_buffer_rsrc(const_cast<uint32_t *>(shadow), 0, (dbg & 2) ? 0 : kBufRecords, kBufFlags);
     const int v4 = lane * 4, vg = lane << kGradShift;
     const int c_last = (IT - 1) * 64 + lane;
     const int vt = c_last < ld ? c_last * 4 : kBufOob, vgt = c_last < ld ? c_last << kGradShift : kBufOob;
@@ -578,13 +581,20 @@
         }
         auto one_sided = [&](auto side) -> int {
             constexpr bool tails = decltype(side)::value;
+            constexpr int SW = (IT + 1) / 2;
             int ce[KC];
             Row<G, IT> yc[KC];
+            unsigned yq[SHD ? KC : 1][SW];
 #pragma unroll
             for (int j = 0; j < KC; ++j)
                 if (KT == KC || j < k) {
                     ce[j] = tails ? ids[3 * j + 2] : ids[3 * j];
-                    wave_load_row<IT>(rs_ent, ce[j] * row_b, v4, vt, yc[j]);
+                    if constexpr (SHD) {
+#pragma unroll
+                        for (int w = 0; w < SW; ++w) yq[j][w] = __builtin_amdgcn_raw_buffer_load_b32(rs_shd, v4 + w * 256, ce[j] * shd_row_b, 0);
+                    } else {
+                        wave_load_row<IT>(rs_ent, ce[j] * row_b, v4, vt, yc[j]);
+                    }
                 }
             wave_normalize<IT>(yh);
             wave_normalize<IT>(yr);
@@ -607,6 +617,62 @@
                 gpos.v[it] = cpos ? (L1 ? sgn(gpos.v[it]) : 2.f * gpos.v[it]) : 0.f;
                 gacc.v[it] = gpos.v[it];
             }
+            bool anyneg = false;
+            const float sign_c = tails ? -1.f : 1.f;
+            if constexpr (SHD) {
+                unsigned unc = 0;
+                {
+                    Row<G, IT> e;
+                    if (!tails) {
+#pragma unroll
+                        for (int it = 0; it < IT; ++it) e.v[it] = yr.v[it] - yt.v[it];
+                    }
+#pragma unroll
+                    for (int j = 0; j < KC; ++j)
+                        if (KT == KC || j < k) {
+                            float s = 0.f;
+#pragma unroll
+                            for (int it = 0; it < IT; ++it) {
+                                const unsigned q = yq[j][it >> 1];
+                                const float y = __builtin_bit_cast(float, (it & 1) ? q & 0xffff0000u : q << 16);
+                                const float d = tails ? u.v[it] - y : y + e.v[it];
+                                s += d * d;
+                            }
+                            unc |= !(oea::wave_sum_uniform(s) > shd_thr) ? 1u << j : 0u;
+                        }
+                }
+                asm volatile("" : "+s"(unc));
+                if (unc) {
+#pragma unroll
+                    for (int j = 0; j < KC; ++j)
+                        if ((KT == KC || j < k) && ((unc >> j) & 1u)) wave_load_row<IT>(rs_ent, ce[j] * row_b, v4, vt, yc[j]);
+#pragma unroll
+                    for (int j = 0; j < KC; ++j)
+                        if ((KT == KC || j < k) && ((unc >> j) & 1u)) {
+                            wave_normalize<IT>(yc[j]);
+                            float s = 0.f;
+#pragma unroll
+                            for (int it = 0; it < IT; ++it) {
+                                const float d = tails ? u.v[it] - yc[j].v[it] : yc[j].v[it] + yr.v[it] - yt.v[it];
+                                yc[j].v[it] = d;
+                                s += d * d;
+                            }
+                            const float xn = cfg.neg_margin - oea::wave_sum_uniform(s);
+                            if (xn > 0.f) {
+                                lsum += cfg.balance * xn;
+                                anyneg = true;
+                                Row<G, IT> g;
+#pragma unroll
+                                for (int it = 0; it < IT; ++it) {
+                                    g.v[it] = c_neg * yc[j].v[it];
+                                    gacc.v[it] += g.v[it];
+                                }
+                                wave_atomic_row<IT>(rs_eg, ce[j] * row_g, vg, vgt, g, sign_c);
+                                buf_flag_set(rs_et, ce[j]);
+                            }
+                        }
+                }
+            } else {
             float sc[KC];
             if (tails) {
 #pragma unroll
@@ -637,8 +703,6 @@
                         sc[j] = oea::wave_sum_uniform(s);
                     }
             }
-            bool anyneg = false;
-            const float sign_c = tails ? -1.f : 1.f;
 #pragma unroll
             for (int j = 0; j < KC; ++j)
                 if (KT == KC || j < k) {
@@ -656,6 +720,7 @@
                         buf_flag_set(rs_et, ce[j]);
                     }
                 }
+            }
             if (PLAN) {
                 const __amdgpu_buffer_rsrc_t rs_cb = __builtin_amdgcn_make_buffer_rsrc(contrib, 0, kBufRecords, kBufFlags);
                 const int so = (int)p * 2 * row_b;
@@ -1115,7 +1180,7 @@
 __device__ __forceinline__ void apply_one_row(float *__restrict__ v, float *__restrict__ acc, grad_t *__restrict__ g,
                                               flag_t *__restrict__ touched_flag, int ld, int lane, int on,
                                               const oea_step_cfg &cfg, const Row<G, IT> &rv, Row<G, IT> &rg,
-                                              const Row<G, IT> &ra) {
+                                              const Row<G, IT> &ra, Row<G, IT> *nv = nullptr) {
     float inv = 1.f, ydg = 0.f;
     if (on) {
         const float ss = sumsq<G, IT>(rv);
@@ -1131,17 +1196,34 @@
         const int c = it * G + lane;
         if (c < ld) {
             const float gv = on ? (rg.v[it] - rv.v[it] * inv * ydg) * inv : rg.v[it];
+            float x;
             if (cfg.opt_kind == OEA_OPT_ADAGRAD) {
                 const float a = ra.v[it] + gv * gv;
                 acc[c] = a;
-                v[c] = rv.v[it] - cfg.lr * gv / sqrtf(a);
+                x = rv.v[it] - cfg.lr * gv / sqrtf(a);
             } else {
-                v[c] = rv.v[it] - cfg.lr * gv;
-            }
+                x = rv.v[it] - cfg.lr * gv;
+            }
+            v[c] = x;
+            if (nv) nv->v[it] = x;
             if (CLEAR) g[c] = 0;
-        }
+        } else if (nv) nv->v[it] = 0.f;
     }
     if (CLEAR && lane == 0) *touched_flag = 0;
+}
+
+template <int G, int IT>
+__device__ __forceinline__ void shadow_store_row(uint32_t *__restrict__ srow, int ld, int lane, const Row<G, IT> &nv) {
+    constexpr int H = 64 / G;
+    constexpr int ITW = (IT * G + 127) / 128 * (128 / G);
+    const float inv = rsqrtf(fmaxf(sumsq<G, IT>(nv), 1e-12f));
+#pragma unroll
+    for (int it = 0; it < ITW; ++it) {
+        if ((it / H) & 1) continue;
+        const int c = it * G + lane;
+        const float lo = it < IT ? nv.v[it < IT ? it : 0] : 0.f, hi = it + H < IT ? nv.v[it + H < IT ? it + H : 0] : 0.f;
+        srow[(c >> 7) * 64 + (c & 63)] = (c < ld ? oea::bf16_rne(lo * inv) : 0u) | (c + 64 < ld ? oea::bf16_rne(hi * inv) << 16 : 0u);
+    }
 }
 
 template <int G, int IT>
@@ -1241,7 +1323,7 @@
                                                        int copies_folded, int rel_blocks, int scan_blocks,
                                                        const uint4 *__restrict__ recs, const uint32_t *__restrict__ vals,
                                                        const int32_t *__restrict__ step_first, int s, const uint8_t *__restrict__ inplan,
-                                                       const float *__restrict__ contrib) {
+                                                       const float *__restrict__ contrib, uint32_t *__restrict__ shadow, int shd_words) {
     constexpr int GPB = 256 / G, GPW = 64 / G;
     const int lane = threadIdx.x % G;
     const int b = (int)blockIdx.x, nb = (int)gridDim.x;
@@ -1290,7 +1372,9 @@
                 }
                 if (lane == 0) ws.ent_touched[row] = 0;
             }
-            apply_one_row<G, IT, false>(ent + row * ld, ent_acc + row * ld, nullptr, nullptr, ld, lane, cfg.ent_l2_norm, cfg, rv, rg, ra);
+            Row<G, IT> nv;
+            apply_one_row<G, IT, false>(ent + row * ld, ent_acc + row * ld, nullptr, nullptr, ld, lane, cfg.ent_l2_norm, cfg, rv, rg, ra, &nv);
+            if (shadow) shadow_store_row<G, IT>(shadow + row * shd_words, ld, lane, nv);
         }
     } else if (b < nb - 1) {
         const int first = rel_blocks;
@@ -1316,8 +1400,10 @@
                     load_row<G, IT>(ent + row * ld, ld, lane, rv);
                     load_grad_row<G, IT>(ws.ent_grad + row * ld, ld, lane, rg);
                     if (cfg.opt_kind == OEA_OPT_ADAGRAD) load_row<G, IT>(ent_acc + row * ld, ld, lane, ra);
+                    Row<G, IT> nv;
                     apply_one_row<G, IT>(ent + row * ld, ent_acc + row * ld, ws.ent_grad + row * ld, ws.ent_touched + row, ld, lane,
-                                         cfg.ent_l2_norm, cfg, rv, rg, ra);
+                                         cfg.ent_l2_norm, cfg, rv, rg, ra, &nv);
+                    if (shadow) shadow_store_row<G, IT>(shadow + row * shd_words, ld, lane, nv);
                 }
             }
         }
@@ -1359,7 +1445,7 @@
 template <int G, int IT4, bool CLEAR>
 __device__ __forceinline__ void apply_one_row4(float *__restrict__ v, float *__restrict__ acc, float *__restrict__ g, flag_t *__restrict__ touched_flag,
                                                int ld, int lane, int on, const oea_step_cfg &cfg, const Row4<IT4> &rv, const Row4<IT4> &rg,
-                                               const Row4<IT4> &ra) {
+                                               const Row4<IT4> &ra, Row4<IT4> *nvo = nullptr) {
     float inv = 1.f, ydg = 0.f;
     if (on) {
         float ss = 0.f, dot = 0.f;
@@ -1390,10 +1476,29 @@
                 nv = make_float4(y.x - cfg.lr * gv.x, y.y - cfg.lr * gv.y, y.z - cfg.lr * gv.z, y.w - cfg.lr * gv.w);
             }
             oea::st4(v + c, nv);
+            if (nvo) nvo->v[it] = nv;
             if (CLEAR) oea::st4(g + c, make_float4(0.f, 0.f, 0.f, 0.f));
-        }
+        } else if (nvo) nvo->v[it] = make_float4(0.f, 0.f, 0.f, 0.f);
     }
     if (CLEAR && lane == 0) *touched_flag = 0;
+}
+
+template <int G, int IT4>
+__device__ __forceinline__ void shadow_store_row4(uint32_t *__restrict__ srow, int ld, int lane, const Row4<IT4> &nv) {
+    static_assert(G == 16 && IT4 <= 2, "columns c and c + 64 in one lane");
+    float ss = 0.f;
+#pragma unroll
+    for (int it = 0; it < IT4; ++it) ss += f4_dot(nv.v[it], nv.v[it]);
+    const float inv = rsqrtf(fmaxf(group_sum<G>(ss), 1e-12f));
+    const int c = 4 * lane;
+    const float4 lo = nv.v[0], hi = nv.v[IT4 - 1];
+    const bool in_lo = c < ld, in_hi = IT4 > 1 && c + 64 < ld;
+    uint4 w;
+    w.x = (in_lo ? oea::bf16_rne(lo.x * inv) : 0u) | (in_hi ? oea::bf16_rne(hi.x * inv) << 16 : 0u);
+    w.y = (in_lo ? oea::bf16_rne(lo.y * inv) : 0u) | (in_hi ? oea::bf16_rne(hi.y * inv) << 16 : 0u);
+    w.z = (in_lo ? oea::bf16_rne(lo.z * inv) : 0u) | (in_hi ? oea::bf16_rne(hi.z * inv) << 16 : 0u);
+    w.w = (in_lo ? oea::bf16_rne(lo.w * inv) : 0u) | (in_hi ? oea::bf16_rne(hi.w * inv) << 16 : 0u);
+    *reinterpret_cast<uint4 *>(srow + c) = w;
 }
 
 template <int G, int IT>
@@ -1403,7 +1508,7 @@
                                                           int copies_folded, int rel_blocks, int scan_blocks,
                                                           const uint4 *__restrict__ recs, const uint32_t *__restrict__ vals,
                                                           const int32_t *__restrict__ step_first, int s, const uint8_t *__restrict__ inplan,
-                                                          const float *__restrict__ contrib) {
+                                                          const float *__restrict__ contrib, uint32_t *__restrict__ shadow, int shd_words) {
     constexpr int GPB = 256 / G, GPW = 64 / G, IT4 = (IT + 3) / 4;
     const int lane = threadIdx.x % G;
     const int b = (int)blockIdx.x, nb = (int)gridDim.x;
@@ -1454,7 +1559,9 @@
                 }
                 if (lane == 0) ws.ent_touched[row] = 0;
             }
-            apply_one_row4<G, IT4, false>(ent + row * ld, ent_acc + row * ld, nullptr, nullptr, ld, lane, cfg.ent_l2_norm, cfg, rv, rg, ra);
+            Row4<IT4> nv;
+            apply_one_row4<G, IT4, false>(ent + row * ld, ent_acc + row * ld, nullptr, nullptr, ld, lane, cfg.ent_l2_norm, cfg, rv, rg, ra, &nv);
+            if (shadow) shadow_store_row4<G, IT4>(shadow + row * shd_words, ld, lane, nv);
         }
     } else if (b < nb - 1) {
         const int first = rel_blocks;
@@ -1480,8 +1587,10 @@
                     load_row4<G, IT4>(ent + row * ld, ld, lane, rv);
                     load_row4<G, IT4>(ws.ent_grad + row * ld, ld, lane, rg);
                     if (cfg.opt_kind == OEA_OPT_ADAGRAD) load_row4<G, IT4>(ent_acc + row * ld, ld, lane, ra);
+                    Row4<IT4> nv;
                     apply_one_row4<G, IT4, true>(ent + row * ld, ent_acc + row * ld, ws.ent_grad + row * ld, ws.ent_touched + row, ld, lane,
-                                                 cfg.ent_l2_norm, cfg, rv, rg, ra);
+                                                 cfg.ent_l2_norm, cfg, rv, rg, ra, &nv);
+                    if (shadow) shadow_store_row4<G, IT4>(shadow + row * shd_words, ld, lane, nv);
                 }
             }
         }
@@ -1921,13 +2030,22 @@
 template <int IT64>
 void launch_wave(int nb, int block, hipStream_t st, const float *ent, const float *rel, int ld, const int32_t *pos,
                  int64_t n_pos, const int32_t *neg, const oea_step_cfg &cfg, const StepWs &ws, float *contrib = nullptr,
-                 const uint32_t *pflags = nullptr, const uint32_t *order = nullptr) {
+                 const uint32_t *pflags = nullptr, const uint32_t *order = nullptr, const uint32_t *shadow = nullptr) {
     const int k = cfg.neg_group_k;
     static const int dbg = [] { const char *e = getenv("OEA_STEP_WAVE_DBG"); return e ? atoi(e) : 0; }();
+    const int shd_row_b = oea::shadow_words(ld) * 4;
+    const double sq = std::sqrt((double)cfg.neg_margin) + (1.0 / 256 + 1.0 / 4096);
+    const float shd_thr = std::nextafter((float)(sq * sq), INFINITY);
 #define OEA_WAVE(L1, KT)                                                                                                               \
     do {                                                                                                                               \
-        if (contrib) oea::launch_timed(triple_wave<IT64, L1, KT, true>, nb, block, st, ent, rel, ld, pos, n_pos, neg, k, cfg, ws, dbg, contrib, pflags, order);   \
-        else oea::launch_timed(triple_wave<IT64, L1, KT, false>, nb, block, st, ent, rel, ld, pos, n_pos, neg, k, cfg, ws, dbg, contrib, pflags, nullptr);          \
+        if constexpr ((L1) == 0 && !oea::kDetScratch) {                                       \
+            if (contrib && shadow) {                                                                                                   \
+                oea::launch_timed(triple_wave<IT64, 0, KT, true, true>, nb, block, st, ent, rel, ld, pos, n_pos, neg, k, cfg, ws, dbg, contrib, pflags, order, shadow, shd_row_b, shd_thr);   \
+                break;                                                                                                                 \
+            }                                                                                                                          \
+        }                                                                                                                              \
+        if (contrib) oea::launch_timed(triple_wave<IT64, L1, KT, true, false>, nb, block, st, ent, rel, ld, pos, n_pos, neg, k, cfg, ws, dbg, contrib, pflags, order, nullptr, 0, 0.f);   \
+        else oea::launch_timed(triple_wave<IT64, L1, KT, false, false>, nb, block, st, ent, rel, ld, pos, n_pos, neg, k, cfg, ws, dbg, contrib, pflags, nullptr, nullptr, 0, 0.f);          \
     } while (0)
     if (k == 10) { if (cfg.l1) OEA_WAVE(1, 10); else OEA_WAVE(0, 10); }
     else { if (cfg.l1) OEA_WAVE(1, 0); else OEA_WAVE(0, 0); }
@@ -1946,10 +2064,15 @@
            !step_runtime_kind();
 }
 
+static bool neg_shadow_applies(const oea_step_cfg &cfg, int64_t n_ent, int32_t ld) {
+    static const bool env_on = [] { const char *e = getenv("OEA_NEG_SHADOW"); return !(e && e[0] == '0'); }();
+    return env_on && !cfg.l1 && cfg.neg_margin > 0.f && n_ent * (int64_t)oea::shadow_words(ld) * 4 < ((int64_t)1 << 30);
+}
+
 template <int G, int IT>
 void launch_grouped(int nb, int block, hipStream_t st, const float *ent, const float *rel, int ld, const int32_t *pos,
                     int64_t n_pos, const int32_t *neg, const oea_step_cfg &cfg, const StepWs &ws, bool wave, float *contrib = nullptr,
-                    const uint32_t *pflags = nullptr, const uint32_t *order = nullptr) {
+                    const uint32_t *pflags = nullptr, const uint32_t *order = nullptr, const uint32_t *shadow = nullptr) {
     const bool runtime_kind = step_runtime_kind();
     const int k = cfg.neg_group_k;
     if constexpr ((G == 32 && IT <= 4) || (G == 64 && IT == 4)) {
@@ -1957,7 +2080,7 @@
             constexpr int IT64 = G == 32 ? (IT + 1) / 2 : 4;
             static const int blk_env = [] { const char *e = getenv("OEA_STEP_WAVE_BLOCK"); return e ? atoi(e) : 0; }();
             const int wblock = G == 32 ? (blk_env == 256 || blk_env == 512 ? blk_env : 512) : (block / G) * 64;
-            launch_wave<IT64>(nb, wblock, st, ent, rel, ld, pos, n_pos, neg, cfg, ws, contrib, pflags, order);
+            launch_wave<IT64>(nb, wblock, st, ent, rel, ld, pos, n_pos, neg, cfg, ws, contrib, pflags, order, shadow);
             return;
         }
     }
@@ -2013,6 +2136,42 @@
     else if (it16 == 6) f(int_c<6>{});
     else if (it16 == 7) f(int_c<7>{});
     else f(int_c<8>{});
+}
+
+template <int G, int IT, class F>
+static void for_plan_apply(int64_t n_ent, int64_t n_rel, int32_t ld, F &&f) {
+    if (G == 32 && apply_g16(n_ent, n_rel, ld)) {
+        for_width16(ld, [&](auto it) {
+#ifndef OEA_DET_SCRATCH
+            static const bool v4 = [] { const char *e = getenv("OEA_APPLY_V4"); return !(e && e[0] == '0'); }();
+            if (v4) return f(int_c<16>{}, it, std::true_type{});
+#endif
+            f(int_c<16>{}, it, std::false_type{});
+        });
+    } else {
+        f(int_c<G>{}, int_c<IT>{}, std::false_type{});
+    }
+}
+
+template <int G, int IT, bool V4>
+__global__ __launch_bounds__(256) void shadow_build_kernel(const float *__restrict__ ent, int64_t n_ent, int ld, uint32_t *__restrict__ shadow,
+                                                           int shd_words) {
+    const int lane = threadIdx.x % G;
+    const int64_t ngrp = (int64_t)gridDim.x * (256 / G);
+    for (int64_t row = (int64_t)blockIdx.x * (256 / G) + threadIdx.x / G; row < n_ent; row += ngrp) {
+#ifndef OEA_DET_SCRATCH
+        if constexpr (V4) {
+            Row4<(IT + 3) / 4> rv;
+            load_row4<G, (IT + 3) / 4>(ent + row * ld, ld, lane, rv);
+            shadow_store_row4<G, (IT + 3) / 4>(shadow + row * shd_words, ld, lane, rv);
+        } else
+#endif
+        {
+            Row<G, IT> rv;
+            load_row<G, IT>(ent + row * ld, ld, lane, rv);
+            shadow_store_row<G, IT>(shadow + row * shd_words, ld, lane, rv);
+        }
+    }
 }
 
 template <int G, int IT>
@@ -2041,7 +2200,7 @@
             static const bool rel_order_on = [] { const char *e = getenv("OEA_STEP_REL_ORDER"); return !(e && e[0] == '0'); }();
             launch_grouped<G, IT>(nb1, block, st, ent, rel, ld, pos, n_pos, neg, cfg, ws, wave_rule(cfg, n_ent, n_rel, ld),
                                   plan ? plan->contrib : nullptr, plan ? plan->pflags + plan_first_pos : nullptr,
-                                  plan && rel_order_on ? plan->rel_order + plan_first_pos : nullptr);
+                                  plan && rel_order_on ? plan->rel_order + plan_first_pos : nullptr, plan ? plan->shadow : nullptr);
         }
         else
             oea::launch_timed(triple_generic<G, IT>, nb1, block, st, ent, rel, ld, pos, n_pos, neg, n_neg, cfg, ws);
@@ -2078,19 +2237,15 @@
                 auto launch = [&](auto kernel) {
                     oea::launch_events(kernel, relb + planb + scanb + 1, block, st, ev0, ev1, ent, ent_acc, n_ent, rel, rel_acc, n_rel, ld, cfg,
                                        ws, n_part, loss_accum, folded, relb, scanb, plan->recs, plan->vals_b, plan->step_first, plan_step,
-                                       plan->inplan, plan->contrib);
+                                       plan->inplan, plan->contrib, plan->shadow, oea::shadow_words(ld));
                 };
-                if (g16 && G == 32)
-                    for_width16(ld, [&](auto it) {
-                        constexpr int IT16 = decltype(it)::value;
+                for_plan_apply<G, IT>(n_ent, n_rel, ld, [&](auto g, auto it, auto v4) {
+                    constexpr int PG = decltype(g)::value, PIT = decltype(it)::value;
 #ifndef OEA_DET_SCRATCH
-                        static const bool v4 = [] { const char *e = getenv("OEA_APPLY_V4"); return !(e && e[0] == '0'); }();
-                        if (v4) return launch(apply_step_plan_v4<16, IT16>);
+                    if constexpr (decltype(v4)::value) return launch(apply_step_plan_v4<PG, PIT>);
 #endif
-                        launch(apply_step_plan<16, IT16>);
-                    });
-                else
-                    launch(apply_step_plan<G, IT>);
+                    launch(apply_step_plan<PG, PIT>);
+                });
             } else
             if (g16 && G == 32 && R == 1) {
                 const int nbg = (int)std::min<int64_t>(std::max<int64_t>(oea::ceil_div(n_rel + n_ent, 16), 1), 16384);
@@ -2315,6 +2470,27 @@
     return wave_rule(*cfg, n_ent, n_rel, ld) && cfg->neg_group_k == k && (cfg->opt_kind == OEA_OPT_SGD || cfg->opt_kind == OEA_OPT_ADAGRAD);
 }
 
+int oea_step_shadow_build(const float *ent, int64_t n_ent, int64_t n_rel, int32_t ld, void *plan, size_t plan_bytes, int64_t n_total,
+                          int32_t steps, int64_t max_batch, void *stream) {
+    OEA_REQUIRE(ent && plan, "null pointer");
+    OEA_REQUIRE(n_ent > 0 && n_rel >= 0 && ld > 0 && ld <= 256 && n_total >= 0 && steps >= 0 && max_batch >= 0, "sizes (ld <= 256)");
+    oea::StepPlanView pv;
+    const size_t need = oea::step_plan_layout(n_total, steps, max_batch, n_ent, ld, plan, &pv);
+    OEA_REQUIRE(plan_bytes >= need, "plan workspace smaller than oea_step_plan_bytes");
+    hipStream_t st = oea::as_stream(stream);
+    const int rc = for_row_width(ld, [&](auto g, auto it) {
+        for_plan_apply<decltype(g)::value, decltype(it)::value>(n_ent, n_rel, ld, [&](auto pg, auto pit, auto v4) {
+            constexpr int PG = decltype(pg)::value;
+            const int nb = (int)std::min<int64_t>(std::max<int64_t>(oea::ceil_div(n_ent, 256 / PG), 1), 8192);
+            shadow_build_kernel<PG, decltype(pit)::value, decltype(v4)::value><<<(unsigned)nb, 256, 0, st>>>(ent, n_ent, ld, pv.shadow,
+                                                                                                               oea::shadow_words(ld));
+        });
+    });
+    if (rc != OEA_OK) return rc;
+    OEA_CHECK_HIP(hipGetLastError());
+    return OEA_OK;
+}
+
 }
 
 static_assert(sizeof(oea_epoch) == 184, "oea_epoch: openea_amd/_lib.py:Epoch and tests/test_host_cpu.py hold the same layout");
@@ -2432,6 +2608,9 @@
         if (!plan_built)
             OEA_TRY_RC(oea_step_plan_build(e->pos_all, e->neg_buf, e->k, e->offsets_dev, n_total, e->steps, w.max_batch, e->n_ent, e->ld, plan,
                                            plan_bytes, stream));
+        if (!neg_shadow_applies(*e->cfg, e->n_ent, e->ld)) pv.shadow = nullptr;
+        else if (step_begin < step_end)
+            OEA_TRY_RC(oea_step_shadow_build(e->ent, e->n_ent, e->n_rel, e->ld, plan, plan_bytes, n_total, e->steps, w.max_batch, stream));
     }
     return epoch_walk(w, [&](const EpochStep &t) -> int {
         if (t.n == 0) return OEA_OK;
diff --git a/openea_amd/ops.py b/openea_amd/ops.py
--- a/openea_amd/ops.py
+++ b/openea_amd/ops.py
@@ -978,6 +978,22 @@
     check(lib().oea_step_plan_rel_order_offset(int(n_total), int(steps), int(max_batch), int(n_ent), int(ld), C.cast(C.byref(off), C.c_void_p)))
     n = int(n_total)
     return plan[off.value: off.value + 4 * n].cpu().numpy().view(np.uint32).copy()
+
+
+def step_shadow_words(ld):
+    return (int(ld) + 127) // 128 * 64
+
+
+def step_shadow_build(ent, n_rel, plan, n_total, steps, max_batch):
+    check(lib().oea_step_shadow_build(_p(ent), ent.shape[0], int(n_rel), ent.shape[1], _p(plan), plan.numel(), int(n_total), int(steps),
+                                      int(max_batch), _stream()))
+
+
+def step_plan_shadow(plan, n_total, steps, max_batch, n_ent, ld):
+    off = C.c_int64(0)
+    check(lib().oea_step_plan_shadow_offset(int(n_total), int(steps), int(max_batch), int(n_ent), int(ld), C.cast(C.byref(off), C.c_void_p)))
+    words = step_shadow_words(ld)
+    return plan[off.value: off.value + 4 * int(n_ent) * words].cpu().numpy().view(np.uint32).reshape(int(n_ent), words).copy()
 
 
 def step_plan_stats(plan, n_total, steps, max_batch, n_ent, ld):
```
